# gooofy/zerovox

Hardware: AMD Instinct MI355X
Metric: audio samples/sec + RTF, 128-phoneme zero-shot synth @22.05kHz, 1/2/4/8 GPU (higher is better)
Workload: dtype f16+bf16

## Files before the change

zerovox_amd/csrc/gemm.hip:

```cpp
#include "mfma_util.h"
#include "zvx_kernels.h"

#include <cstring>
#include <type_traits>

#ifndef ZVX_GEMM_PART
#define ZVX_GEMM_PART 0
#endif
#define ZVX_PART_MAIN (ZVX_GEMM_PART != 2)
#define ZVX_PART_RESFUSE (ZVX_GEMM_PART != 1)
#if ZVX_GEMM_PART == 2
extern thread_local bool zvx_gemm_dry_run;
#else
thread_local hipEvent_t zvx_gemm_ev_start = nullptr, zvx_gemm_ev_stop = nullptr;
thread_local bool zvx_gemm_dry_run = false;
#endif
#define g_dry_run zvx_gemm_dry_run

#define ZVX_LAUNCH(...) do { if (!g_dry_run) ZVX_DISPATCH(__VA_ARGS__); } while (0)

namespace zvx {


#define PITCH 80
#define KBYTES 64

__device__ __forceinline__ float bf16_to_f32(unsigned short h) { return __uint_as_float(((unsigned)h) << 16); }
__device__ __forceinline__ unsigned short f32_to_bf16(float f) {
    unsigned u = __float_as_uint(f);
    u += 0x7fffu + ((u >> 16) & 1u);
    return (unsigned short)(u >> 16);
}

template <int DT>
__device__ __forceinline__ void load4(const void* base, long idx, float v[4]) {
    if (DT == DT_F32) {
        float4 t = *(const float4*)((const float*)base + idx);
        v[0] = t.x; v[1] = t.y; v[2] = t.z; v[3] = t.w;
    } else {
        uint2 t = *(const uint2*)((const unsigned short*)base + idx);
        v[0] = __uint_as_float(t.x << 16); v[1] = __uint_as_float(t.x & 0xffff0000u);
        v[2] = __uint_as_float(t.y << 16); v[3] = __uint_as_float(t.y & 0xffff0000u);
    }
}
__device__ __forceinline__ void load4_dyn(const void* base, int dt, long idx, float v[4]) {
    if (dt == DT_F32) load4<DT_F32>(base, idx, v);
    else if (dt == DT_F16) {
        const uint2 t = *(const uint2*)((const unsigned short*)base + idx);
        const f32x2 a = unpack_f16x2(t.x), b = unpack_f16x2(t.y);
        v[0] = a.x; v[1] = a.y; v[2] = b.x; v[3] = b.y;
    } else load4<DT_BF16>(base, idx, v);
}
__device__ __forceinline__ void store4_dyn(void* base, int dt, long idx, const float v[4]) {
    if (dt == DT_F32) {
        *(float4*)((float*)base + idx) = make_float4(v[0], v[1], v[2], v[3]);
    } else if (dt == DT_F16) {
        uint2 t;
        t.x = pack_f16x2_sat(v[0], v[1]); t.y = pack_f16x2_sat(v[2], v[3]);
        *(uint2*)((unsigned short*)base + idx) = t;
    } else {
        uint2 t;
        t.x = (unsigned)f32_to_bf16(v[0]) | ((unsigned)f32_to_bf16(v[1]) << 16);
        t.y = (unsigned)f32_to_bf16(v[2]) | ((unsigned)f32_to_bf16(v[3]) << 16);
        *(uint2*)((unsigned short*)base + idx) = t;
    }
}

template <int TM, int TN>
__device__ __forceinline__ void epilogue(const GemmArgs& a, f32x16 (&acc)[TN][TM], int b, int h, int row_base, int col_base,
                                         int out_len, bool two_d, int lane) {
    const long ooff = (long)b * a.o_bs + (long)h * a.o_hs;
    const long roff = (long)b * a.r_bs + (long)h * a.r_hs;
    const long aoff = (long)b * a.a_bs;
#pragma unroll
    for (int j = 0; j < TM; j++) {
        const int r = row_base + j * 32 + (lane & 31);
        bool rok = r < a.M;
        if (two_d) rok = rok && (r % a.wout) < out_len; else rok = rok && r < out_len;
        if (!rok) continue;
        const float brow = (a.bias_mode == 2) ? a.bias[r] : 0.f;
#pragma unroll
        for (int i = 0; i < TN; i++) {
#pragma unroll
            for (int g = 0; g < 4; g++) {
                const int n = col_base + i * 32 + 8 * g + 4 * (lane >> 5);
                if (n >= a.N) continue;
                float v[4];
#pragma unroll
                for (int e = 0; e < 4; e++) v[e] = acc[i][j][4 * g + e] * a.alpha + brow;
                if (a.bias_mode == 1) {
                    const float4 bb = *(const float4*)(a.bias + n);
                    v[0] += bb.x; v[1] += bb.y; v[2] += bb.z; v[3] += bb.w;
                }
                if (a.res_mode) {
                    float rr[4];
                    load4_dyn(a.res, a.res_dtype, roff + (long)r * a.ldr + n, rr);
                    if (a.res_mode == 2) {
#pragma unroll
                        for (int e = 0; e < 4; e++) rr[e] = rr[e] >= 0.f ? rr[e] : rr[e] * a.res_inv_slope;
                    }
#pragma unroll
                    for (int e = 0; e < 4; e++) v[e] += rr[e];
                }
                if (a.accum_mode) {
                    const long ai = aoff + (long)r * a.lda + n;
                    if (a.accum_mode & 1) {
                        float t[4];
                        load4_dyn(a.accum, a.accum_dtype, ai, t);
                        v[0] += t[0]; v[1] += t[1]; v[2] += t[2]; v[3] += t[3];
                    }
                    if (a.accum_mode & 2) store4_dyn(a.accum, a.accum_dtype, ai, v);
                }
                if (a.out) {
#pragma unroll
                    for (int e = 0; e < 4; e++) {
                        float t = v[e] * a.out_scale;
                        if (a.act == ACT_RELU) t = fmaxf(t, 0.f);
                        else if (a.act == ACT_LRELU) t = t >= 0.f ? t : t * a.slope;
                        v[e] = t;
                    }
                    if (a.post_scale) {
                        const float4 ps = *(const float4*)(a.post_scale + n), pt = *(const float4*)(a.post_shift + n);
                        v[0] = v[0] * ps.x + pt.x; v[1] = v[1] * ps.y + pt.y;
                        v[2] = v[2] * ps.z + pt.z; v[3] = v[3] * ps.w + pt.w;
                    }
                    store4_dyn(a.out, a.out_dtype, ooff + (long)r * a.ldo + n, v);
                }
            }
        }
    }
}

template <int DT, int BM, int BN, int WM, int WN>
__global__ __launch_bounds__(256) void gemm_kernel(const GemmArgs a) {
    constexpr int ES = (DT == DT_F32) ? 4 : 2;
    constexpr int EPC = 16 / ES;
    constexpr int BKE = KBYTES / ES;
    constexpr int TM = BM / WM / 32, TN = BN / WN / 32;
    constexpr int XCH = BM * 4 / 256;
    constexpr int WCH = (BN * 4 + 255) / 256;
    static_assert(WM * WN == 4, "4 waves");

    __shared__ __attribute__((aligned(16))) unsigned char lds[2][(BM + BN) * PITCH];
// ... 24 lines not shown
    const unsigned char* Wp = (const unsigned char*)a.W + ((long)b * a.w_bs + (long)h * a.w_hs) * ES;

    int xu[XCH], xv[XCH];
    const int kc = tid & 3;
#pragma unroll
    for (int i = 0; i < XCH; i++) {
        const int r = m0 + (tid >> 2) + i * 64;
        if (two_d) { xu[i] = (r / a.wout) * a.stride; xv[i] = (r % a.wout) * a.stride; }
        else { xu[i] = 0; xv[i] = r; }
    }

    const int kchunks = (Kb + BKE - 1) / BKE;
    const int S = a.ntaps * kchunks;

    uint4 xreg[XCH], wreg[WCH];

    auto load_regs = [&](int s) {
        const int tap = s / kchunks;
        const int k = (s - tap * kchunks) * BKE + kc * EPC;
        const bool kok = k < Kb;
        const int du = a.du[tap], dv = a.dv[tap];
#pragma unroll
        for (int i = 0; i < XCH; i++) {
            const int iu = xu[i] + du, iv = xv[i] + dv;
            const bool ok = kok && iu >= 0 && iu < a.hin && iv >= 0 && iv < in_len;
            uint4 v = make_uint4(0, 0, 0, 0);
            if (ok) v = *(const uint4*)(Xp + ((long)(iu * a.win + iv) * a.ldx + k) * ES);
            xreg[i] = v;
        }
#pragma unroll
        for (int i = 0; i < WCH; i++) {
            const int c = tid + i * 256;
            const int n = n0 + (c >> 2);
            uint4 v = make_uint4(0, 0, 0, 0);
            if ((BN * 4 >= 256 * (i + 1) || c < BN * 4) && kok && n < a.N)
                v = *(const uint4*)(Wp + ((long)tap * a.w_ts + (long)n * a.ldw + k) * ES);
            wreg[i] = v;
        }
    };
    auto store_lds = [&](int buf) {
        unsigned char* base = lds[buf];
#pragma unroll
        for (int i = 0; i < XCH; i++)
            *(uint4*)(base + ((tid >> 2) + i * 64) * PITCH + kc * 16) = xreg[i];
#pragma unroll
        for (int i = 0; i < WCH; i++) {
            const int c = tid + i * 256;
            if (BN * 4 >= 256 * (i + 1) || c < BN * 4)
                *(uint4*)(base + (BM + (c >> 2)) * PITCH + kc * 16) = wreg[i];
        }
    };

    f32x16 acc[TN][TM];
#pragma unroll
    for (int i = 0; i < TN; i++)
#pragma unroll
        for (int j = 0; j < TM; j++)
#pragma unroll
            for (int e = 0; e < 16; e++) acc[i][j][e] = 0.f;

    const int xrow = wr * (BM / WM) + (lane & 31);
    const int wrow = BM + wc * (BN / WN) + (lane & 31);
    const int koff = (lane >> 5) * 16;

    if (S > 0) {
        load_regs(0);
        store_lds(0);
    }
    __syncthreads();
    for (int s = 0; s < S; s++) {
        if (s + 1 < S) load_regs(s + 1);
        const unsigned char* base = lds[s & 1];
#pragma unroll
        for (int sub = 0; sub < 2; sub++) {
            uint4 xf[TM], wf[TN];
#pragma unroll
            for (int j = 0; j < TM; j++) xf[j] = *(const uint4*)(base + (xrow + j * 32) * PITCH + sub * 32 + koff);
#pragma unroll
            for (int i = 0; i < TN; i++) wf[i] = *(const uint4*)(base + (wrow + i * 32) * PITCH + sub * 32 + koff);
#pragma unroll
            for (int i = 0; i < TN; i++)
#pragma unroll
                for (int j = 0; j < TM; j++) {
                    if (DT == DT_BF16) {
                        acc[i][j] = __builtin_amdgcn_mfma_f32_32x32x16_bf16(
                            __builtin_bit_cast(bf16x8, wf[i]), __builtin_bit_cast(bf16x8, xf[j]), acc[i][j], 0, 0, 0);
                    } else if (DT == DT_F16) {
                        acc[i][j] = __builtin_amdgcn_mfma_f32_32x32x16_f16(
                            __builtin_bit_cast(f16x8, wf[i]), __builtin_bit_cast(f16x8, xf[j]), acc[i][j], 0, 0, 0);
                    } else {
                        acc[i][j] = __builtin_amdgcn_mfma_f32_32x32x2f32(__uint_as_float(wf[i].x), __uint_as_float(xf[j].x), acc[i][j], 0, 0, 0);
                        acc[i][j] = __builtin_amdgcn_mfma_f32_32x32x2f32(__uint_as_float(wf[i].y), __uint_as_float(xf[j].y), acc[i][j], 0, 0, 0);
                        acc[i][j] = __builtin_amdgcn_mfma_f32_32x32x2f32(__uint_as_float(wf[i].z), __uint_as_float(xf[j].z), acc[i][j], 0, 0, 0);
                        acc[i][j] = __builtin_amdgcn_mfma_f32_32x32x2f32(__uint_as_float(wf[i].w), __uint_as_float(xf[j].w), acc[i][j], 0, 0, 0);
                    }
                }
        }
        if (s + 1 < S) store_lds((s + 1) & 1);
        __syncthreads();
    }

    epilogue<TM, TN>(a, acc, b, h, m0 + wr * (BM / WM), n0 + wc * (BN / WN), out_len, two_d, lane);
}

__device__ __forceinline__ unsigned pack_f16x2(float lo, float hi) { return pack_f16x2_sat(lo, hi); }
__device__ __forceinline__ unsigned pack16x2(float lo, float hi, bool f16) { return f16 ? pack_f16x2_sat(lo, hi) : pack_bf16x2(lo, hi); }
__device__ __forceinline__ f32x2 unpack16x2(unsigned u, bool f16) { return f16 ? unpack_f16x2(u) : unpack_bf16x2(u); }

#define ZVX_EPI(res, am, out) ((res) | ((am) << 1) | ((out) << 3))
#define ZVX_EPI_DEC(res) (16 | 8 | (res))
#define ZVX_EPI_FLIP (ZVX_EPI(0, 0, 1) | 32)

template <int TM, int TN, int RES_LDS = 0, int EPI = -1, bool H16 = false>
__device__ __forceinline__ void epilogue_rows(const GemmArgs& a, f32x16 (&acc)[TN][TM], int b, int row_base, int col_base,
                                              int out_len, int lane, unsigned char* stage ,
                                              const unsigned char* res_lds = nullptr ,
                                              int res_pitch = 0) {
    constexpr int NW = TN * 32;
    constexpr int EP = NW * 4 + 16;
    constexpr int LPR = NW / 8;
    constexpr int RPP = 64 / LPR;
    constexpr int NP = 32 / RPP;
    constexpr bool CT = EPI >= 0;
    constexpr bool DEC = CT && (EPI & 16) != 0;
    constexpr bool BURST = !(CT && !DEC && ((EPI >> 1) & 1));
    const long ooff = (long)b * a.o_bs, roff = (long)b * a.r_bs, aoff = (long)b * a.a_bs;
    const int c8 = lane % LPR;
    const int n = col_base + c8 * 8;
    const bool nok = n < a.N;
    const float alpha = CT ? 1.f : a.alpha, oscale = a.out_scale, rinv = a.res_inv_slope;
    const int act = DEC ? ACT_NONE : (CT ? ACT_LRELU : a.act);
    const float slope = CT ? (a.act == ACT_LRELU ? a.slope : 1.f) : a.slope;
    const int res_mode = RES_LDS ? 2 : (DEC ? (EPI & 1) : (CT ? ((EPI & 1) ? 2 : 0) : a.res_mode));
    const int accum_mode = DEC ? 0 : (CT ? (EPI >> 1) & 3 : a.accum_mode), bias_mode = (CT && !DEC) ? 1 : a.bias_mode;
    const bool has_out = CT ? (EPI >> 3) & 1 : a.out != nullptr, out_bf16 = CT || a.out_dtype != DT_F32, has_post = !CT && a.post_scale != nullptr;
    const bool out_f16 = CT ? H16 : a.out_dtype == DT_F16, res_f16 = (CT || RES_LDS) ? H16 : a.res_dtype == DT_F16, acc_f16 = CT ? H16 : ((TN == 1 || TM <= 2) && a.accum_dtype == DT_F16);
    const bool acc_bf16 = CT || a.accum_dtype == DT_BF16 || acc_f16, res_bf16 = CT || RES_LDS || a.res_dtype != DT_F32;
#define pk2(lo, hi, f16) ((CT && H16) ? pack_f16x2_raw(lo, hi) : pack16x2(lo, hi, f16))
    f32x2 bcol[4];
#pragma unroll
    for (int e = 0; e < 4; e++) bcol[e] = (f32x2){0.f, 0.f};
    if (bias_mode == 1 && nok) {
        const float4 b0 = *(const float4*)(a.bias + n), b1 = *(const float4*)(a.bias + n + 4);
        bcol[0] = (f32x2){b0.x, b0.y}; bcol[1] = (f32x2){b0.z, b0.w}; bcol[2] = (f32x2){b1.x, b1.y}; bcol[3] = (f32x2){b1.z, b1.w};
    }
    u32x4 pk[TM][NP];
    const bool res_glb = !RES_LDS && res_mode && res_bf16;
    uint4 rnext[NP];
    auto res_prefetch = [&](int j) {
#pragma unroll
        for (int p = 0; p < NP; p++) {
            const int r = row_base + j * 32 + p * RPP + lane / LPR;
            const bool okp = r < a.M && r < out_len && nok;
            rnext[p] = *(const uint4*)((const unsigned short*)a.res + (okp ? roff + (long)r * a.ldr + n : 0));
        }
    };
    if (res_glb) res_prefetch(0);
#pragma unroll
    for (int j = 0; j < TM; j++) {
#pragma unroll
        for (int i = 0; i < TN; i++)
#pragma unroll
            for (int g = 0; g < 4; g++)
                *(float4*)(stage + (lane & 31) * EP + (i * 32 + 8 * g + 4 * (lane >> 5)) * 4) =
                    make_float4(acc[i][j][4 * g], acc[i][j][4 * g + 1], acc[i][j][4 * g + 2], acc[i][j][4 * g + 3]);
        f32x2 v[NP][4];
        uint4 rraw[NP];
        float4 aa0[NP], aa1[NP];
        uint4 aab[NP];
        bool ok[NP];
        if (res_glb) {
#pragma unroll
            for (int p = 0; p < NP; p++) rraw[p] = rnext[p];
            if (j + 1 < TM) res_prefetch(j + 1);
        }
#pragma unroll
        for (int p = 0; p < NP; p++) {
            const int rl = p * RPP + lane / LPR;
            const int r = row_base + j * 32 + rl;
            ok[p] = r < a.M && r < out_len && nok;
            const float4 v0 = *(const float4*)(stage + rl * EP + c8 * 32), v1 = *(const float4*)(stage + rl * EP + c8 * 32 + 16);
            v[p][0] = (f32x2){v0.x, v0.y}; v[p][1] = (f32x2){v0.z, v0.w}; v[p][2] = (f32x2){v1.x, v1.y}; v[p][3] = (f32x2){v1.z, v1.w};
            if (RES_LDS == 1) rraw[p] = *(const uint4*)(res_lds + (j * 32 + rl) * res_pitch + (col_base + c8 * 8) * 2);
            if (accum_mode & 1) {
                const long ai = ok[p] ? aoff + (long)r * a.lda + n : 0;
                if (acc_bf16) aab[p] = *(const uint4*)((const unsigned short*)a.accum + ai);
                else { const float* ap = (const float*)a.accum + ai; aa0[p] = *(const float4*)ap; aa1[p] = *(const float4*)(ap + 4); }
// ... 70 lines not shown
                    t[2] = t[2] * (f32x2){s1.x, s1.y} + (f32x2){h1.x, h1.y}; t[3] = t[3] * (f32x2){s1.z, s1.w} + (f32x2){h1.z, h1.w};
                }
                if (out_bf16) {
                    const u32x4 o = (u32x4){pk2(t[0].x, t[0].y, out_f16), pk2(t[1].x, t[1].y, out_f16), pk2(t[2].x, t[2].y, out_f16), pk2(t[3].x, t[3].y, out_f16)};
                    if (BURST) pk[j][p] = o;
                    else if (ok[p]) *(u32x4*)((unsigned short*)a.out + ooff + (long)r * a.ldo + n) = o;
                } else if (ok[p]) {
                    if (!CT && a.out_split3) {
                        unsigned short* op = (unsigned short*)a.out + ooff + (long)r * a.ldo + n;
                        u32x4 hv, lv;
#pragma unroll
                        for (int e = 0; e < 4; e++) {
                            if (a.out_split3 == 2) {
                                const unsigned hp = pack_f16x2(t[e].x, t[e].y);
                                const f32x2 rem = (t[e] - unpack_f16x2(hp)) * 2048.f;
                                hv[e] = hp; lv[e] = pack_f16x2(rem.x, rem.y);
                            } else {
                                const unsigned hp = pack_bf16x2(t[e].x, t[e].y);
                                const f32x2 rem = t[e] - unpack_bf16x2(hp);
                                hv[e] = hp; lv[e] = pack_bf16x2(rem.x, rem.y);
                            }
                        }
                        *(u32x4*)op = hv; *(u32x4*)(op + a.N) = hv; *(u32x4*)(op + 2 * a.N) = lv;
                    } else {
                        float* op = (float*)a.out + ooff + (long)r * a.ldo + n;
                        *(float4*)op = make_float4(t[0].x, t[0].y, t[1].x, t[1].y);
                        *(float4*)(op + 4) = make_float4(t[2].x, t[2].y, t[3].x, t[3].y);
                    }
                }
            }
        }
    }
    if (has_out && out_bf16 && BURST) {
        unsigned short* obase = (unsigned short*)a.out + ooff + n;
        const int ldo = a.ldo;
#pragma unroll
        for (int j = 0; j < TM; j++)
#pragma unroll
            for (int p = 0; p < NP; p++) {
                const int r = row_base + j * 32 + p * RPP + lane / LPR;
                if (r < a.M && r < out_len && nok) *(u32x4*)(obase + (long)r * ldo) = pk[j][p];
            }
    }
#undef pk2
}

template <int TM, int TN, bool F16 = false>
__device__ __forceinline__ void epilogue_direct(const GemmArgs& a, f32x16 (&acc)[TN][TM], int b, int row_base, int col_base,
                                                int out_len, int lane, unsigned char* stage ) {
    constexpr int NW = TN * 32, EP = NW * 2 + 16, LPR = NW / 8, RPP = 64 / LPR, NP = 32 / RPP;
    const float slope = a.act == ACT_LRELU ? a.slope : 1.f;
    const int h4 = 4 * (lane >> 5), c8 = lane % LPR, n = col_base + c8 * 8;
    const bool nok = n < a.N;
    float4 bb[TN][4];
#pragma unroll
    for (int i = 0; i < TN; i++)
#pragma unroll
        for (int g = 0; g < 4; g++) {
            const int co = col_base + i * 32 + 8 * g + h4;
            bb[i][g] = co < a.N ? *(const float4*)(a.bias + co) : make_float4(0.f, 0.f, 0.f, 0.f);
        }
    unsigned short* obase = (unsigned short*)a.out + (long)b * a.o_bs + n;
    u32x4 o[TM][NP];
#pragma unroll
    for (int j = 0; j < TM; j++) {
#pragma unroll
        for (int i = 0; i < TN; i++)
#pragma unroll
            for (int g = 0; g < 4; g++) {
                const f32x2 v01 = lrelu2((f32x2){acc[i][j][4 * g], acc[i][j][4 * g + 1]} + (f32x2){bb[i][g].x, bb[i][g].y}, slope);
                const f32x2 v23 = lrelu2((f32x2){acc[i][j][4 * g + 2], acc[i][j][4 * g + 3]} + (f32x2){bb[i][g].z, bb[i][g].w}, slope);
                uint2 pk;
                pk.x = pack16x2(v01.x, v01.y, F16);
                pk.y = pack16x2(v23.x, v23.y, F16);
                *(uint2*)(stage + (lane & 31) * EP + (i * 32 + 8 * g + h4) * 2) = pk;
            }
#pragma unroll
        for (int p = 0; p < NP; p++) o[j][p] = *(const u32x4*)(stage + (p * RPP + lane / LPR) * EP + c8 * 16);
    }
#pragma unroll
    for (int j = 0; j < TM; j++)
#pragma unroll
        for (int p = 0; p < NP; p++) {
            const int r = row_base + j * 32 + p * RPP + lane / LPR;
            if (r < a.M && r < out_len && nok) *(u32x4*)(obase + (long)r * a.ldo) = o[j][p];
        }
}

#if ZVX_PART_MAIN
#define SLAB_KC 64
#define SLAB_PITCH 144

__global__ void k_pack_w(const unsigned short* w, int ntaps, int N, int K, unsigned short* out, int nkc, long total_frag_lanes) {
    long idx = (long)blockIdx.x * blockDim.x + threadIdx.x;
    if (idx >= total_frag_lanes) return;
    const int lane = idx & 63; long t = idx >> 6;
    const int k16 = t & 3; t >>= 2;
    const int tap = t % ntaps; t /= ntaps;
    const int kc = t % nkc; const int nt = t / nkc;
    const int n = nt * 32 + (lane & 31);
    const int k0 = kc * SLAB_KC + k16 * 16 + 8 * (lane >> 5);
    unsigned short v[8];
#pragma unroll
    for (int e = 0; e < 8; e++) {
        const int k = k0 + e;
        v[e] = (n < N && k < K) ? w[((long)tap * N + n) * K + k] : (unsigned short)0;
    }
    uint4 o;
    o.x = v[0] | ((unsigned)v[1] << 16); o.y = v[2] | ((unsigned)v[3] << 16);
    o.z = v[4] | ((unsigned)v[5] << 16); o.w = v[6] | ((unsigned)v[7] << 16);
    *(uint4*)(out + idx * 8) = o;
}

size_t packed_weight_elems(int ntaps, int N, int K) {
    const int nkc = (K + SLAB_KC - 1) / SLAB_KC, nt = (N + 31) / 32;
    return (size_t)nt * nkc * ntaps * 4 * 64 * 8;
}
void launch_pack_weights(const void* w_bf16, int ntaps, int N, int K, void* out, hipStream_t s) {
    const int nkc = (K + SLAB_KC - 1) / SLAB_KC, nt = (N + 31) / 32;
    const long total = (long)nt * nkc * ntaps * 4 * 64;
    hipLaunchKernelGGL(k_pack_w, dim3((unsigned)((total + 255) / 256)), dim3(256), 0, s, (const unsigned short*)w_bf16, ntaps, N, K,
                       (unsigned short*)out, nkc, total);
}

// ... 10 lines not shown
    constexpr int NIT = ((BM + MAXH) * 8 + 255) / 256;
    static_assert(WM * WN == 4, "4 waves");
    extern __shared__ __attribute__((aligned(16))) unsigned char slab[];
    if (F16 && EPI >= 0 && EPI != ZVX_EPI(0, 0, 1) && EPI != ZVX_EPI_FLIP) f16_saturate_mode();

    const int tid = threadIdx.x, lane = tid & 63, wave = __builtin_amdgcn_readfirstlane(tid >> 6);
    const int wr = wave % WM, wc = wave / WM;
    const int ntn = (a.N + BN - 1) / BN;
    int wg, b;
    if (a.xcd_flat) {
        const int nx = gridDim.x, nwg = nx * gridDim.y, id = blockIdx.y * nx + blockIdx.x, q = nwg >> 3, r = nwg & 7, xcd = id & 7;
        const int w = (xcd < r ? xcd * (q + 1) : r * (q + 1) + (xcd - r) * q) + (id >> 3);
        b = w / nx; wg = w - b * nx;
    } else {
        const int nwg = gridDim.x, id = blockIdx.x, q = nwg >> 3, r = nwg & 7, xcd = id & 7;
        wg = (xcd < r ? xcd * (q + 1) : r * (q + 1) + (xcd - r) * q) + (id >> 3);
        b = blockIdx.y;
    }
    const int nt = wg % ntn, mt = wg / ntn;
    const int m0 = mt * BM, n0 = nt * BN;
    const bool bflat = a.bflat != 0;
    const int out_len = bflat ? a.M : (a.out_len ? a.out_len[b] : a.M);
    const int in_len = bflat ? 0 : (a.in_len ? a.in_len[b] : a.in_len_static);
    if (m0 >= out_len || m0 >= a.M) return;
    if (bflat) {
        const int b0 = m0 / a.bflat, t0 = m0 - b0 * a.bflat;
        if (t0 >= a.out_len[b0] && t0 + BM <= a.bflat) return;
    }

    const int HL = a.halo_l, SR = BM + a.halo_l + a.halo_r;
    const int nkc = (a.K + SLAB_KC - 1) / SLAB_KC, n16 = a.K >> 4, ntaps = a.ntaps;
    const unsigned short* Xp = (const unsigned short*)a.X + (long)b * a.x_bs;
    const int nkc2 = (!FULLK && a.K2 > 0) ? (a.K2 + SLAB_KC - 1) / SLAB_KC : 0, n16_2 = a.K2 >> 4;
    const unsigned short* Xp2 = (const unsigned short*)a.X2 + (long)b * a.x2_bs;
    const int in_rows = ((MAXH > 64 || bflat) && a.flat_win) ? a.flat_rows : in_len;
    unsigned rowmask = 0xffffffffu;
    if (bflat) {
        rowmask = 0;
#pragma unroll
        for (int it = 0; it < NIT; it++) {
            const int g = m0 - HL + ((tid + it * 256) >> 3);
            if (g >= 0 && g < in_rows) { const int bb = g / a.bflat; if (g - bb * a.bflat < a.in_len[bb]) rowmask |= 1u << it; }
        }
    } else if (MAXH > 64 && a.flat_win) {
        rowmask = 0;
#pragma unroll
        for (int it = 0; it < NIT; it++) {
            const int g = m0 - HL + ((tid + it * 256) >> 3);
            if (g >= 0 && g < in_rows && (g % a.flat_win) < in_len) rowmask |= 1u << it;
        }
    }

    f32x16 acc[TN][TM];
#pragma unroll
    for (int i = 0; i < TN; i++)
#pragma unroll
        for (int j = 0; j < TM; j++)
#pragma unroll
            for (int e = 0; e < 16; e++) acc[i][j][e] = 0.f;

    constexpr bool WREG = R == 0;
    constexpr int F = BN / 32, CNT = F >= 4 ? F / 4 : 1, WD = 4, D = WREG ? WD : R - 1, WAITN = WREG ? (WD - 1) * TN : (D - 2) * CNT;
    const int nt32_total = (a.N + 31) >> 5;
    const int nsteps = a.ntaps * 4, gtotal = nkc * nsteps + nkc2 * 4;
    const uint4* wsrc[CNT];
#pragma unroll
    for (int j = 0; j < CNT; j++) {
        const int f = wave * CNT + j, t32 = (n0 >> 5) + f;
        wsrc[j] = (const uint4*)a.Wp + (long)(t32 < nt32_total ? t32 : 0) * gtotal * 64 + lane;
    }
    const int xrow0 = HL + wr * (BM / WM) + (lane & 31);
    const int koff = (lane >> 5) * 16;
    unsigned char* ring = slab + ((SR * SLAB_PITCH + 1023) & ~1023);
    const unsigned lds_base = (unsigned)(size_t)(__attribute__((address_space(3))) unsigned char*)slab;
    const int dvreg = a.dv[lane & (ZVX_MAX_TAPS - 1)];
    const bool loader = wave * CNT < F;
    const unsigned char* wq[TN];
#pragma unroll
    for (int i = 0; i < TN; i++) {
        const int t32 = (n0 >> 5) + wc * TN + i;
        wq[i] = (const unsigned char*)a.Wp + (long)(t32 < nt32_total ? t32 : 0) * gtotal * 1024;
    }
    const bool wave_dead = __builtin_amdgcn_readfirstlane((int)(n0 + wc * TN * 32 >= a.N)) != 0;
    const unsigned lane16 = lane * 16;
    u32x4 wreg[WREG ? WD : 1][TN] = {};
    auto wload = [&](int gs, int slot) {
        const long off = (long)(gs < gtotal ? gs : gtotal - 1) * 1024;
#pragma unroll
        for (int i = 0; i < TN; i++)
            asm volatile("global_load_dwordx4 %0, %1, %2" : "+v"(wreg[WREG ? slot : 0][i]) : "v"(lane16), "s"(wq[i] + off) : "memory");
    };
    auto dma = [&](int gs) {
        if (WREG || !loader) return;
        const int slot = gs & (R - 1);
        const long off = (long)(gs < gtotal ? gs : gtotal - 1) * 64;
#pragma unroll
        for (int j = 0; j < CNT; j++)
            __builtin_amdgcn_global_load_lds((const __attribute__((address_space(1))) void*)(wsrc[j] + off),
                                             (__attribute__((address_space(3))) void*)(ring + (slot * F + wave * CNT + j) * 1024), 16, 0, 0);
    };
    if (WREG) { wload(0, 0); wload(1, 1); wload(2, 2); wload(3, 3); }
    else {
#pragma unroll
        for (int s0 = 0; s0 < D; s0++) dma(s0);
    }

    for (int kc = 0; kc < nkc + nkc2; kc++) {
        const bool src2 = !FULLK && kc >= nkc;
        const unsigned short* const Xs = src2 ? Xp2 : Xp;
        const int ldxs = src2 ? a.ldx2 : a.ldx, Ks = src2 ? a.K2 : a.K, kbase = (src2 ? kc - nkc : kc) * SLAB_KC;
        {
            constexpr int FCH = NIT > 10 ? (NIT + 1) / 2 : NIT;
#pragma unroll
            for (int h0 = 0; h0 < NIT; h0 += FCH) {
                uint4 sv[FCH];
#pragma unroll
                for (int i = 0; i < FCH; i++) {
                    const int it = h0 + i;
                    const int c = tid + it * 256;
                    const int row = c >> 3, q = c & 7;
                    const int g = m0 - HL + row, k = kbase + q * 8;
                    sv[i] = make_uint4(0, 0, 0, 0);
                    if (it < NIT && c < SR * 8 && g >= 0 && g < in_rows && k < Ks && ((rowmask >> it) & 1)) sv[i] = *(const uint4*)(Xs + (long)g * ldxs + k);
                }
                if (kc && h0 == 0) __syncthreads();
#pragma unroll
                for (int i = 0; i < FCH; i++) {
                    const int c = tid + (h0 + i) * 256;
                    if (h0 + i < NIT && c < SR * 8) *(uint4*)(slab + (c >> 3) * SLAB_PITCH + (c & 7) * 16) = sv[i];
                }
            }
        }
        __syncthreads();
        int nk16 = 4;
        if (!FULLK) { nk16 = src2 ? n16_2 - (kc - nkc) * 4 : n16 - kc * 4; if (nk16 > 4) nk16 = 4; if (wave_dead) nk16 = 0; }
        const int ntaps_kc = src2 ? 1 : ntaps;

        uint4 xA[TM], wA[TN], xB[TM], wB[TN];
        const unsigned ring_rd = lds_base + (unsigned)(size_t)(ring - slab) + lane * 16 + wc * TN * 1024;
        const int gs0 = src2 ? nkc * nsteps + (kc - nkc) * 4 : kc * nsteps;
        auto rd = [&](uint4 (&xf)[TM], uint4 (&wf)[TN], int gs, unsigned rowoff, int kk) {
            if (!WREG) {
                const unsigned wa = ring_rd + (gs & ((WREG ? 1 : R) - 1)) * (F * 1024);
#pragma unroll
                for (int i = 0; i < TN; i++)
                    asm volatile("ds_read_b128 %0, %1 offset:%2" : "=v"(wf[i]) : "v"(wa), "n"(i * 1024));
            }
#pragma unroll
            for (int j = 0; j < TM; j++)
                asm volatile("ds_read_b128 %0, %1" : "=v"(xf[j]) : "v"(lds_base + rowoff + j * 32 * SLAB_PITCH + kk * 32));
        };
        auto mma = [&](uint4 (&xf)[TM], uint4 (&wf)[TN]) {
#pragma unroll
            for (int i = 0; i < TN; i++)
#pragma unroll
                for (int j = 0; j < TM; j++)
                    acc[i][j] = F16 ? __builtin_amdgcn_mfma_f32_32x32x16_f16(__builtin_bit_cast(f16x8, wf[i]), __builtin_bit_cast(f16x8, xf[j]), acc[i][j], 0, 0, 0)
                                    : __builtin_amdgcn_mfma_f32_32x32x16_bf16(__builtin_bit_cast(bf16x8, wf[i]),
                                                                       __builtin_bit_cast(bf16x8, xf[j]), acc[i][j], 0, 0, 0);
        };
        auto mma_r = [&](uint4 (&xf)[TM], int slot) {
#pragma unroll
            for (int i = 0; i < TN; i++)
#pragma unroll
                for (int j = 0; j < TM; j++)
                    acc[i][j] = F16 ? __builtin_amdgcn_mfma_f32_32x32x16_f16(__builtin_bit_cast(f16x8, wreg[WREG ? slot : 0][i]), __builtin_bit_cast(f16x8, xf[j]), acc[i][j], 0, 0, 0)
                                    : __builtin_amdgcn_mfma_f32_32x32x16_bf16(__builtin_bit_cast(bf16x8, wreg[WREG ? slot : 0][i]),
                                                                       __builtin_bit_cast(bf16x8, xf[j]), acc[i][j], 0, 0, 0);
        };
        auto rowoff_of = [&](int tap) {
            const int d = src2 ? 0 : __builtin_amdgcn_readlane(dvreg, tap < ntaps ? tap : ntaps - 1);
            return (unsigned)((xrow0 + d) * SLAB_PITCH + koff);
        };
        unsigned rowoff = rowoff_of(0);
        rd(xA, wA, gs0, rowoff, 0);
        for (int tap = 0; tap < ntaps_kc; tap++) {
            const unsigned rowoff_next = rowoff_of(tap + 1);
#pragma unroll
            for (int kk = 0; kk < 4; kk++) {
                const int gs = gs0 + tap * 4 + kk;
                if (WREG) asm volatile("s_waitcnt vmcnt(%0)" :: "n"(WAITN) : "memory");
                else asm volatile("s_waitcnt vmcnt(%0)\n\ts_barrier" :: "n"(WAITN) : "memory");
                dma(gs + D);
                if (kk & 1) rd(xA, wA, gs + 1, kk == 3 ? rowoff_next : rowoff, (kk + 1) & 3);
                else        rd(xB, wB, gs + 1, rowoff, kk + 1);
                asm volatile("s_waitcnt lgkmcnt(%0)" :: "n"(WREG ? TM : TM + TN) : "memory");
// ... 1 lines not shown
                if (FULLK || kk < nk16) {
                    if (WREG) { if (kk & 1) mma_r(xB, kk); else mma_r(xA, kk); }
                    else { if (kk & 1) mma(xB, wB); else mma(xA, wA); }
                }
                __builtin_amdgcn_sched_barrier(0);
                if (WREG) wload(gs + WD, kk);
            }
            rowoff = rowoff_next;
        }
        asm volatile("s_waitcnt lgkmcnt(0)" ::: "memory");
    }
    if (WREG) {
#pragma unroll
        for (int sl = 0; sl < (WREG ? WD : 1); sl++)
#pragma unroll
            for (int i = 0; i < TN; i++) asm volatile("s_waitcnt vmcnt(0)" : "+v"(wreg[sl][i]) :: "memory");
    } else {
        asm volatile("s_waitcnt vmcnt(0)" ::: "memory");
    }
    __syncthreads();
    if (EPI == ZVX_EPI_FLIP)
        epilogue_direct<TM, TN, !F16>(a, acc, b, m0 + wr * (BM / WM), n0 + wc * (BN / WN), out_len, lane, slab + wave * (32 * (TN * 64 + 16)));
    else if (EPI == ZVX_EPI(0, 0, 1))
        epilogue_direct<TM, TN, F16>(a, acc, b, m0 + wr * (BM / WM), n0 + wc * (BN / WN), out_len, lane, slab + wave * (32 * (TN * 64 + 16)));
    else
        epilogue_rows<TM, TN, 0, EPI, (F16 && EPI >= 0)>(a, acc, b, m0 + wr * (BM / WM), n0 + wc * (BN / WN), out_len, lane, slab + wave * (32 * (TN * 32 * 4 + 16)));
}

template <int C, int NT, int BM, int WM, int WN, int MINW, int MAXH = 64, bool F16 = false>
__global__ __launch_bounds__(256, MINW) void convreg_kernel(const GemmArgs a) {
    constexpr int TM = BM / WM / 32;
    constexpr int KS = C / 16;
    constexpr int PITCH_ = C * 2 + 16;
    constexpr int CPR = C / 8;
    constexpr int NIT = ((BM + MAXH) * CPR + 255) / 256;
    constexpr int FCH = NIT > 12 ? 8 : NIT;
    static_assert(WM * WN == 4 && WN * 32 == C, "wave layout");
    extern __shared__ __attribute__((aligned(16))) unsigned char slab[];

    const int tid = threadIdx.x, lane = tid & 63, wave = tid >> 6;
    const int wr = wave % WM, wc = wave / WM;
    int wg;
    {
        const int nwg = gridDim.x, id = blockIdx.x, q = nwg >> 3, r = nwg & 7, xcd = id & 7;
        wg = (xcd < r ? xcd * (q + 1) : r * (q + 1) + (xcd - r) * q) + (id >> 3);
    }
    const int m0 = wg * BM, b = blockIdx.y;
    const int out_len = a.out_len ? a.out_len[b] : a.M;
    const int in_len = a.in_len ? a.in_len[b] : a.in_len_static;
    if (m0 >= out_len || m0 >= a.M) return;
    const int HL = a.halo_l, SR = BM + a.halo_l + a.halo_r;
    const unsigned short* Xp = (const unsigned short*)a.X + (long)b * a.x_bs;

    uint4 w[NT][KS];
    {
        const uint4* Wq = (const uint4*)a.Wp + ((long)wc * NT * 4) * 64 + lane;
#pragma unroll
        for (int t = 0; t < NT; t++)
#pragma unroll
            for (int kk = 0; kk < KS; kk++) w[t][kk] = Wq[(t * 4 + kk) * 64];
    }
    {
        const bool flat = MAXH > 64 && a.flat_win;
        const int in_rows = flat ? a.flat_rows : in_len;
#pragma unroll
        for (int h0 = 0; h0 < NIT; h0 += FCH) {
            uint4 sv[FCH];
#pragma unroll
            for (int i = 0; i < FCH; i++) {
                const int c = tid + (h0 + i) * 256;
                const int row = c / CPR, q = c % CPR;
                const int g = m0 - HL + row;
                sv[i] = make_uint4(0, 0, 0, 0);
                if (h0 + i < NIT && c < SR * CPR && g >= 0 && g < in_rows && (!flat || (g % a.flat_win) < in_len)) sv[i] = *(const uint4*)(Xp + (long)g * a.ldx + q * 8);
            }
#pragma unroll
            for (int i = 0; i < FCH; i++) {
                const int c = tid + (h0 + i) * 256;
                if (h0 + i < NIT && c < SR * CPR) *(uint4*)(slab + (c / CPR) * PITCH_ + (c % CPR) * 16) = sv[i];
            }
        }
    }
    __syncthreads();

    f32x16 acc[1][TM];
#pragma unroll
    for (int j = 0; j < TM; j++)
#pragma unroll
        for (int e = 0; e < 16; e++) acc[0][j][e] = 0.f;
    const int xrow0 = HL + wr * (BM / WM) + (lane & 31);
    const int koff = (lane >> 5) * 16;
#pragma unroll
    for (int t = 0; t < NT; t++) {
        const unsigned char* rowp = slab + (xrow0 + a.dv[t]) * PITCH_ + koff;
#pragma unroll
        for (int kk = 0; kk < KS; kk++)
#pragma unroll
            for (int j = 0; j < TM; j++) {
                const uint4 xf = *(const uint4*)(rowp + j * 32 * PITCH_ + kk * 32);
                acc[0][j] = mfma16<F16>(w[t][kk], xf, acc[0][j]);
            }
    }
    __syncthreads();
    epilogue_rows<TM, 1>(a, acc, b, m0 + wr * (BM / WM), wc * 32, out_len, lane, slab + wave * (32 * (32 * 4 + 16)));
}

typedef __attribute__((ext_vector_type(2))) unsigned u32x2_t;
__device__ __forceinline__ void store_block_mfma_layout(unsigned short* row_ptr , const uint2 (&pk)[4], int lane, bool ok) {
#pragma unroll
    for (int pr = 0; pr < 2; pr++) {
        const u32x2_t sx = __builtin_amdgcn_permlane32_swap(pk[2 * pr].x, pk[2 * pr + 1].x, false, false);
        const u32x2_t sy = __builtin_amdgcn_permlane32_swap(pk[2 * pr].y, pk[2 * pr + 1].y, false, false);
        if (ok) *(u32x4*)(row_ptr + 8 * (2 * pr + (lane >> 5))) = (u32x4){sx.x, sy.x, sx.y, sy.y};
    }
}

template <int C, int BM, int WM, int WN, int MAXH, int MODE, int WGPC, bool POOL = false>
__global__ __launch_bounds__(WM * WN * 64, WM * WN * WGPC / 4) void conv2d_persist_kernel(const GemmArgs a, const int ntm, const int ntiles) {
    constexpr int NTHR = WM * WN * 64;
    constexpr int NT = 9, TM = BM / WM / 32, KS = C / 16, PITCH_ = C * 2 + 16, CPR = C / 8, RSTEP = NTHR / CPR;
    constexpr int NIT = ((BM + MAXH) * CPR + NTHR - 1) / NTHR;
    constexpr bool EC_LDS = NTHR > 256;
    static_assert(WN * 32 == C && BM % (WM * 32) == 0, "wave layout");
    extern __shared__ __attribute__((aligned(16))) unsigned char slab[];

    const int tid = threadIdx.x, lane = tid & 63, wave = __builtin_amdgcn_readfirstlane(tid >> 6);
    const int wr = wave % WM, wc = wave / WM;
    const int G = gridDim.x, xcd = blockIdx.x & 7, slot = blockIdx.x >> 3;
    auto tile_of = [&](int r) {
        const int base = r * G, n = ntiles - base < G ? ntiles - base : G;
        if (n <= 0) return ntiles;
        const int per = (n + 7) >> 3, t = xcd * per + slot;
        return (slot < per && t < n) ? base + t : ntiles;
    };
    const int HL = a.halo_l, SR = BM + a.halo_l + a.halo_r, win = a.flat_win, in_rows = a.flat_rows;

    uint4 w[NT][KS];
    {
        const uint4* Wq = (const uint4*)a.Wp + ((long)wc * NT * 4) * 64 + lane;
#pragma unroll
        for (int t = 0; t < NT; t++)
#pragma unroll
// ... 341 lines not shown

    const int tid = threadIdx.x, lane = tid & 63, wave = tid >> 6;
    const int wr = wave % WM, wc = wave / WM;
    const int BMO = BM - 2 * H2;
    const int H1 = a.halo_l;
    const int SR = BM + 2 * H1;
    unsigned char* t1 = slab + ((SR * PITCH_ + 15) & ~15);

    constexpr bool TWO_SETS = (NT * KS <= 24);
    uint4 w[NT][KS];
    uint4 w2[TWO_SETS ? NT : 1][TWO_SETS ? KS : 1];
    const uint4* W1q = (const uint4*)a.Wp2 + ((long)wc * NT * 4) * 64 + lane;
    const uint4* W2q = (const uint4*)a.Wp + ((long)wc * NT * 4) * 64 + lane;
#pragma unroll
    for (int t = 0; t < NT; t++)
#pragma unroll
        for (int kk = 0; kk < KS; kk++) {
            w[t][kk] = W1q[(t * 4 + kk) * 64];
            if (TWO_SETS) w2[t][kk] = W2q[(t * 4 + kk) * 64];
        }
    const int koff = (lane >> 5) * 16;
    const int wrow = wr * (BM / WM);
    int tile;
    {
        const int nwg = gridDim.x, id = blockIdx.x, q = nwg >> 3, r = nwg & 7, xcd = id & 7;
        tile = (xcd < r ? xcd * (q + 1) : r * (q + 1) + (xcd - r) * q) + (id >> 3);
    }
    {
        const int b = tile / ntm, m0 = (tile - b * ntm) * BMO;
        const int out_len = a.out_len ? a.out_len[b] : a.M;
        const int in_len = a.in_len ? a.in_len[b] : a.in_len_static;
        if (tile >= ntiles || m0 >= out_len || m0 >= a.M) return;
        const unsigned short* Xp = (const unsigned short*)a.X + (long)b * a.x_bs;
        {
            uint4 sv[NIT];
            const int tq = tid;
#pragma unroll
            for (int it = 0; it < NIT; it++) {
                const int c = tq + it * 256;
                const int row = c / CPR, q = c % CPR;
                const int g = m0 - H2 - H1 + row;
                sv[it] = make_uint4(0, 0, 0, 0);
                if (c < SR * CPR && g >= 0 && g < in_len) sv[it] = *(const uint4*)(Xp + (long)g * a.ldx + q * 8);
            }
#pragma unroll
            for (int it = 0; it < NIT; it++) {
                const int c = tq + it * 256;
                if (c < SR * CPR) *(uint4*)(slab + (c / CPR) * PITCH_ + (c % CPR) * 16) = sv[it];
            }
        }
        __syncthreads();

        f32x16 acc[1][TM];
#pragma unroll
        for (int j = 0; j < TM; j++)
#pragma unroll
            for (int e = 0; e < 16; e++) acc[0][j][e] = 0.f;
#pragma unroll
        for (int t = 0; t < NT; t++) {
            const unsigned char* rowp = slab + (wrow + (lane & 31) + H1 + a.dv1[t]) * PITCH_ + koff;
#pragma unroll
            for (int kk = 0; kk < KS; kk++)
#pragma unroll
                for (int j = 0; j < TM; j++) {
                    const uint4 xf = *(const uint4*)(rowp + j * 32 * PITCH_ + kk * 32);
                    acc[0][j] = mfma16<F16>(w[t][kk], xf, acc[0][j]);
                }
            if (!TWO_SETS) {
#pragma unroll
                for (int kk = 0; kk < KS; kk++) w[t][kk] = W2q[(t * 4 + kk) * 64];
            }
        }
#pragma unroll
        for (int j = 0; j < TM; j++) {
            const int i = wrow + j * 32 + (lane & 31);
            const int g = m0 - H2 + i;
            const bool inside = g >= 0 && g < in_len;
#pragma unroll
            for (int q = 0; q < 4; q++) {
                const int co = wc * 32 + 8 * q + 4 * (lane >> 5);
                const float4 bb = *(const float4*)(a.bias1 + co);
                const uint2 xr = *(const uint2*)(slab + (i + H1) * PITCH_ + co * 2);
                const f32x2 r01 = inv_lrelu2(F16 ? unpack_f16x2(xr.x) : unpack_bf16x2(xr.x), a.res_inv_slope);
                const f32x2 r23 = inv_lrelu2(F16 ? unpack_f16x2(xr.y) : unpack_bf16x2(xr.y), a.res_inv_slope);
                f32x2 v01 = (f32x2){acc[0][j][4 * q] + bb.x, acc[0][j][4 * q + 1] + bb.y} + r01;
                f32x2 v23 = (f32x2){acc[0][j][4 * q + 2] + bb.z, acc[0][j][4 * q + 3] + bb.w} + r23;
                v01 = lrelu2(v01, a.slope1); v23 = lrelu2(v23, a.slope1);
                if (!inside) { v01 = (f32x2){0.f, 0.f}; v23 = (f32x2){0.f, 0.f}; }
                uint2 pk;
                if (F16) { pk.x = pack_f16x2_sat(v01.x, v01.y); pk.y = pack_f16x2_sat(v23.x, v23.y); }
                else { pk.x = pack_bf16x2(v01.x, v01.y); pk.y = pack_bf16x2(v23.x, v23.y); }
                *(uint2*)(t1 + i * PITCH_ + co * 2) = pk;
            }
        }
        __syncthreads();
#pragma unroll
        for (int j = 0; j < TM; j++)
#pragma unroll
            for (int e = 0; e < 16; e++) acc[0][j][e] = 0.f;
#pragma unroll
        for (int t = 0; t < NT; t++) {
            const unsigned char* rowp = t1 + (wrow + (lane & 31) + H2 + a.dv[t]) * PITCH_ + koff;
#pragma unroll
            for (int kk = 0; kk < KS; kk++)
#pragma unroll
                for (int j = 0; j < TM; j++) {
                    const uint4 xf = *(const uint4*)(rowp + j * 32 * PITCH_ + kk * 32);
                    acc[0][j] = mfma16<F16>(TWO_SETS ? w2[TWO_SETS ? t : 0][TWO_SETS ? kk : 0] : w[t][kk], xf, acc[0][j]);
                }
        }
        const int lim = (m0 + BMO < out_len) ? m0 + BMO : out_len;
        epilogue_rows<TM, 1, 1, -1, F16>(a, acc, b, m0 + wrow, wc * 32, lim, lane, slab + wave * (32 * (32 * 4 + 16)),
                                   t1 + (wrow + H2) * PITCH_, PITCH_);
    }
}

template <int C, int NT, int BM, int WM, int WN, int MINW>
static bool launch_rb2fuse_c(const GemmArgs& a, int h2, hipStream_t stream) {
    const int bmo = BM - 2 * h2;
    if (bmo < 32 || a.halo_l > 16) return false;
    const size_t pitch = C * 2 + 16;
    const size_t sb = (((size_t)(BM + 2 * a.halo_l) * pitch + 15) & ~(size_t)15);
    if (sb < (size_t)4 * 32 * (32 * 4 + 16)) return false;
    const size_t lds = sb + (size_t)(BM + 2 * h2) * pitch;
    if (lds > 160 * 1024) return false;
    const int ntm = (a.M + bmo - 1) / bmo, ntiles = ntm * a.nbatch;
    const dim3 grid(ntiles);
    if (a.dtype == DT_F16) { auto kfn = rb2fuse_kernel<C, NT, BM, WM, WN, MINW, true>; if (!lds_opt_in((const void*)kfn)) return false; ZVX_LAUNCH(kfn, grid, dim3(256), lds, stream, a, h2, ntm, ntiles); }
    else { auto kfn = rb2fuse_kernel<C, NT, BM, WM, WN, MINW, false>; if (!lds_opt_in((const void*)kfn)) return false; ZVX_LAUNCH(kfn, grid, dim3(256), lds, stream, a, h2, ntm, ntiles); }
    return true;
}

int launch_rb2fuse(GemmArgs a, hipStream_t stream) {
    if (a.dtype == DT_F32 || !a.Wp || !a.Wp2 || a.N != a.K || a.nheads != 1 || a.wout > 0 || a.bflat || a.K2) return -1;
    if (!(a.ntaps == 3 || a.ntaps == 5 || a.ntaps == 7) || !(a.N == 32 || a.N == 64)) return -1;
    const int h = (a.ntaps - 1) / 2, d1 = a.dv1[1] - a.dv1[0], d2 = a.dv[1] - a.dv[0];
    if (d1 < 1 || d2 < 1) return -1;
    for (int t = 0; t < a.ntaps; t++) if (a.dv1[t] != (t - h) * d1 || a.dv[t] != (t - h) * d2) return -1;
    if (a.alpha != 1.f || a.bias_mode != 1 || !a.bias || !a.bias1 || a.post_scale || a.res_mode != 2 || a.res != a.X || a.res_dtype != a.dtype || a.ldo % 8 ||
        (a.out && a.out_dtype != a.dtype) || (a.accum && (a.lda % 8 || a.accum_dtype != a.dtype)) || a.in_len != a.out_len || a.ldx != a.N) return -1;
    a.halo_l = a.halo_r = h * d1;
    a.fused = 2;
    if (a.N == 32) {
        if (a.ntaps == 3 && launch_rb2fuse_c<32, 3, 256, 4, 1, 2>(a, h * d2, stream)) return 30;
        if (a.ntaps == 5 && launch_rb2fuse_c<32, 5, 256, 4, 1, 2>(a, h * d2, stream)) return 30;
        if (a.ntaps == 7 && launch_rb2fuse_c<32, 7, 256, 4, 1, 2>(a, h * d2, stream)) return 30;
    } else {
        if (a.ntaps == 3 && launch_rb2fuse_c<64, 3, 256, 2, 2, 2>(a, h * d2, stream)) return 31;
        if (a.ntaps == 5 && launch_rb2fuse_c<64, 5, 256, 2, 2, 2>(a, h * d2, stream)) return 31;
    }
    return -1;
}

template <int C, int NT, int AM, bool HAS_OUT, int TM, bool F16 = false>
__global__ __launch_bounds__(512) __attribute__((amdgpu_waves_per_eu(2, 2))) void resfuse_persist_kernel(const GemmArgs a, int ntm, int ntiles) {
    if (F16) f16_saturate_mode();
    constexpr int KS = C >= 16 ? C / 16 : 1, CPR = C / 8, NTL = C >= 32 ? C / 32 : 1, RG = 4 / NTL;
    constexpr int QN = C >= 32 ? 4 : C / 8;
    constexpr int BM1 = 32 * TM * RG;
    constexpr int H2 = (NT - 1) / 2, BMO = BM1 - 2 * H2;
    constexpr int P = C * 2 + 16, CPP = CPR + 1;
    constexpr int NW = NT * KS;
    constexpr bool LEAN = NW > 36 || (F16 && NW >= 28 && TM == 2 && (AM & 1) && HAS_OUT);
    constexpr int NRES = LEAN ? (NW < 36 ? NW : 36) : NW;
    typedef __attribute__((ext_vector_type(4))) int i32x4;
    extern __shared__ __attribute__((aligned(16))) unsigned char lds[];

    const int tid = threadIdx.x, lane = tid & 63, wave = __builtin_amdgcn_readfirstlane(tid >> 6);
    const int role = wave >> 2, w4 = wave & 3;
    const int wc = w4 % NTL, wr = w4 / NTL, wrow = wr * 32 * TM;
    const int H1 = a.halo_l, SR = BM1 + 2 * H1;
    const int dil = a.dv1[1] - a.dv1[0];
    const float slope1 = a.slope1;
    const int SB = (SR * P + 1023) & ~1023;
    const int TB = ((BM1 + 2 * H2) * P + 15) & ~15;
    unsigned char* const t1base = lds + 4 * SB;
    unsigned char* const stage = t1base + 2 * TB + w4 * (32 * 80);
    float* const bias1_l = (float*)(t1base + 2 * TB + 4 * (32 * 80));
    float* const bias2_l = bias1_l + C;
    int* const lens_l = (int*)(bias2_l + C);
    const unsigned lds_addr0 = (unsigned)(size_t)(__attribute__((address_space(3))) unsigned char*)lds;
    const int G = gridDim.x;
    if (C < 32) {
        for (int i = tid * 16; i < 4 * SB + 2 * TB; i += 512 * 16) *(uint4*)(lds + i) = make_uint4(0, 0, 0, 0);
        __syncthreads();
    }
    if (tid < C) { bias1_l[tid] = a.bias1[tid]; bias2_l[tid] = a.bias[tid]; }
    if (a.nbatch <= 128 && tid < a.nbatch) { lens_l[tid] = a.out_len ? a.out_len[tid] : a.M; lens_l[128 + tid] = a.in_len ? a.in_len[tid] : a.in_len_static; }

    constexpr int NKC = (C + 63) / 64;
    const uint4* const Wq = (const uint4*)(role ? a.Wp : a.Wp2) + ((long)wc * NKC * NT * 4) * 64 + lane;
    auto wfrag = [](int t, int kk) { return (((kk >> 2) * NT + t) * 4 + (kk & 3)) * 64; };
    uint4 w[NRES];
#pragma unroll
    for (int i = 0; i < NRES; i++) w[i] = Wq[wfrag(i / KS, i % KS)];

    constexpr bool BIAS_REG = NW <= 22;
    const int h4 = 4 * (lane >> 5);
    float4 bq[4];
    if (BIAS_REG) {
#pragma unroll
        for (int q = 0; q < 4; q++) bq[q] = q < QN ? *(const float4*)((role ? a.bias : a.bias1) + wc * 32 + 8 * q + h4) : make_float4(0.f, 0.f, 0.f, 0.f);
    }
#pragma unroll
    for (int i = 0; i < NRES; i++) asm volatile("" :: "v"(w[i].x));
    if (BIAS_REG) {
#pragma unroll
        for (int q = 0; q < 4; q++) asm volatile("" :: "v"(bq[q].x));
    }
    __syncthreads();
    struct Tile { int t, b, mt, m0, in_len, out_len; };
    const bool use_tab = a.nbatch <= 128;
    auto sload = [&](const int* p) { int v; asm volatile("s_load_dword %0, %1, 0x0\n\ts_waitcnt lgkmcnt(0)" : "=s"(v) : "s"(p) : "memory"); return v; };
    auto len_of = [&](const int* g, int which, int b, int dflt) {
        if (!g) return dflt;
        return use_tab ? __builtin_amdgcn_readfirstlane(lens_l[which * 128 + b]) : sload(g + b);
    };
    const int gq = G / ntm, gr = G % ntm;
    auto load_tile = [&](int t, int b, int mt) {
        Tile q; q.t = -1; q.b = q.mt = q.m0 = q.in_len = q.out_len = 0;
        for (; t < ntiles; t += G, b += gq, mt += gr) {
            if (mt >= ntm) { mt -= ntm; b++; }
            const int m0 = mt * BMO, ol = len_of(a.out_len, 0, b, a.M);
            if (m0 < ol) { q.t = t; q.b = b; q.mt = mt; q.m0 = m0; q.out_len = ol; q.in_len = len_of(a.in_len, 1, b, a.in_len_static); break; }
        }
        q.t = __builtin_amdgcn_readfirstlane(q.t); q.b = __builtin_amdgcn_readfirstlane(q.b); q.mt = __builtin_amdgcn_readfirstlane(q.mt);
        q.m0 = __builtin_amdgcn_readfirstlane(q.m0);
        q.in_len = __builtin_amdgcn_readfirstlane(q.in_len); q.out_len = __builtin_amdgcn_readfirstlane(q.out_len);
        return q;
    };
    auto next_tile = [&](const Tile& q) {
        int b = q.b + gq, mt = q.mt + gr;
        return load_tile(q.t + G, b, mt);
    };
    constexpr int MAXP = C == 128 ? 10 : 8;
    constexpr bool VREL_REG = NW <= 22;
    const int npieces = SB >> 10;
    auto vrel_of = [&](int n) {
        const int cp = (w4 + 4 * n) * 64 + lane, row = cp / CPP, qs = cp % CPP;
        return qs == CPR ? -(1 << 30) : (row * a.ldx + (qs << 3)) * 2;
    };
    int vrel[VREL_REG ? MAXP : 1];
    if (VREL_REG) {
#pragma unroll
        for (int n = 0; n < MAXP; n++) vrel[n] = vrel_of(n);
    }
    auto dma_slab = [&](const Tile& q, int buf) {
        const int g0 = q.m0 - H2 - H1;
        const unsigned long long pa = (unsigned long long)((const unsigned short*)a.X + (long)q.b * a.x_bs + (long)g0 * a.ldx);
        const i32x4 rs = {__builtin_amdgcn_readfirstlane((int)(unsigned)pa), __builtin_amdgcn_readfirstlane((int)((pa >> 32) & 0xffff)),
                          __builtin_amdgcn_readfirstlane((q.in_len - g0) * a.ldx * 2), 0x00020000};
        const int thr = -g0 * a.ldx * 2;
        const unsigned la0 = lds_addr0 + buf * SB + w4 * 1024;
#pragma unroll
        for (int n = 0; n < MAXP; n++) {
            if (w4 + 4 * n < npieces) {
                const int vr = VREL_REG ? vrel[VREL_REG ? n : 0] : vrel_of(n);
                const int voff = vr < thr ? -16 : vr;
                const unsigned la = __builtin_amdgcn_readfirstlane(la0 + n * 4096);
                asm volatile("s_mov_b32 m0, %0\n\tbuffer_load_dwordx4 %1, %2, 0 offen lds" :: "s"(la), "v"(voff), "s"(rs) : "memory", "m0");
            }
        }
    };

    Tile qA, qB, qC, qD;
    qA = load_tile(ntiles, 0, 0); qB = qA;
    qC = load_tile(blockIdx.x, blockIdx.x / ntm, blockIdx.x % ntm);
    qD = qC.t >= 0 ? next_tile(qC) : qA;
    if (role == 0 && qC.t >= 0) dma_slab(qC, 0);
    asm volatile("s_waitcnt vmcnt(0) lgkmcnt(0)\n\ts_barrier" ::: "memory");
    const int koff = (lane >> 5) * 16;
    f32x16 acc[1][TM];
    for (int ph = 0; qA.t >= 0 || qB.t >= 0 || qC.t >= 0; ph++) {
        const Tile qE = qD.t >= 0 ? next_tile(qD) : qD;
        if (role == 0) {
            if (qD.t >= 0) dma_slab(qD, (ph + 1) & 3);
            if (qB.t >= 0) {
                unsigned char* t1 = t1base + ((ph - 1) & 1) * TB;
#pragma unroll
                for (int j = 0; j < TM; j++) {
                    const int i = wrow + j * 32 + (lane & 31);
                    const int g = qB.m0 - H2 + i;
                    const bool inside = g >= 0 && g < qB.in_len;
#pragma unroll
                    for (int q = 0; q < QN; q++) {
                        const int co = wc * 32 + 8 * q + h4;
                        const float4 bb = BIAS_REG ? bq[q] : *(const float4*)(bias1_l + co);
                        const f32x2 v01 = lrelu2((f32x2){acc[0][j][4 * q], acc[0][j][4 * q + 1]} + (f32x2){bb.x, bb.y}, slope1);
                        const f32x2 v23 = lrelu2((f32x2){acc[0][j][4 * q + 2], acc[0][j][4 * q + 3]} + (f32x2){bb.z, bb.w}, slope1);
                        uint2 pk;
                        pk.x = inside ? pack16<F16>(v01.x, v01.y) : 0u;
                        pk.y = inside ? pack16<F16>(v23.x, v23.y) : 0u;
                        *(uint2*)(t1 + i * P + co * 2) = pk;
                    }
                }
            }
            if (qC.t >= 0) {
#pragma unroll
                for (int j = 0; j < TM; j++)
#pragma unroll
                    for (int e = 0; e < 16; e++) acc[0][j][e] = 0.f;
                const unsigned char* rowp0 = lds + (ph & 3) * SB + (wrow + (lane & 31) + H1 - H2 * dil) * P + koff;
#pragma unroll
                for (int t = 0; t < NT; t++) {
                    const unsigned char* rowp = rowp0 + t * dil * P;
#pragma unroll
                    for (int kk = 0; kk < KS; kk++) {
                        const uint4 wf = (t * KS + kk < NRES) ? w[t * KS + kk < NRES ? t * KS + kk : 0] : Wq[wfrag(t, kk)];
#pragma unroll
                        for (int j = 0; j < TM; j++) {
                            const uint4 xf = *(const uint4*)(rowp + j * 32 * P + kk * 32);
                            acc[0][j] = mfma16<F16>(wf, xf, acc[0][j]);
                        }
                    }
                }
            }
            asm volatile("s_waitcnt vmcnt(0)" ::: "memory");
        } else if (qA.t >= 0) {
#pragma unroll
            for (int j = 0; j < TM; j++)
#pragma unroll
                for (int e = 0; e < 16; e++) acc[0][j][e] = 0.f;
            const unsigned char* rowp = t1base + (ph & 1) * TB + (wrow + (lane & 31)) * P + koff;
#pragma unroll
            for (int t = 0; t < NT; t++)
#pragma unroll
                for (int kk = 0; kk < KS; kk++) {
                    const uint4 wf = (t * KS + kk < NRES) ? w[t * KS + kk < NRES ? t * KS + kk : 0] : Wq[wfrag(t, kk)];
#pragma unroll
                    for (int j = 0; j < TM; j++) {
                        const uint4 xf = *(const uint4*)(rowp + (t + j * 32) * P + kk * 32);
                        acc[0][j] = mfma16<F16>(wf, xf, acc[0][j]);
                    }
                }
            const int lim_rows = (qA.m0 + BMO < qA.out_len) ? qA.m0 + BMO : qA.out_len;
            const int lim = (C >= 32 || (lane & 3) < CPR) ? lim_rows : -(1 << 30);
            {
                const float rinv = a.res_inv_slope, oscale = a.out_scale, slope = a.act == ACT_LRELU ? a.slope : 1.f;
                const unsigned char* resp = lds + ((ph + 2) & 3) * SB + (wrow + H2 + H1 + (lane & 31)) * P + (wc * 32 + h4) * 2;
                const long rm_off = wc * 32 + (lane & 3) * 8;
                unsigned short* accp = (unsigned short*)a.accum + (long)qA.b * a.a_bs + rm_off;
                unsigned short* outp = (unsigned short*)a.out + (long)qA.b * a.o_bs + rm_off;
                float4 bb[LEAN ? 1 : 4];
                if (!LEAN) {
#pragma unroll
                    for (int q = 0; q < QN; q++) bb[LEAN ? 0 : q] = BIAS_REG ? bq[q] : *(const float4*)(bias2_l + wc * 32 + 8 * q + h4);
                }
                constexpr bool XS_EARLY = NW < 28 || TM == 1;
                uint4 xs[TM][2];
                if ((AM & 1) && XS_EARLY) {
#pragma unroll
                    for (int j = 0; j < TM; j++)
#pragma unroll
                        for (int h = 0; h < 2; h++) {
                            const int gr = qA.m0 + wrow + j * 32 + h * 16 + (lane >> 2);
                            xs[j][h] = *(const uint4*)(accp + (gr < lim ? (long)gr * a.lda : 0));
                        }
                }
#pragma unroll
                for (int j = 0; j < TM; j++) {
                    if ((AM & 1) && !XS_EARLY) {
#pragma unroll
                        for (int h = 0; h < 2; h++) {
                            const int gr = qA.m0 + wrow + j * 32 + h * 16 + (lane >> 2);
                            xs[j][h] = *(const uint4*)(accp + (gr < lim ? (long)gr * a.lda : 0));
                        }
                    }
                    uint2 rrj[LEAN ? 1 : 4];
                    if (!LEAN) {
#pragma unroll
                        for (int q = 0; q < QN; q++) rrj[LEAN ? 0 : q] = *(const uint2*)(resp + j * 32 * P + q * 16);
                    }
                    uint2 pk[LEAN ? 1 : 4];
#pragma unroll
                    for (int q = 0; q < QN; q++) {
                        const float4 bq_ = LEAN ? *(const float4*)(bias2_l + wc * 32 + 8 * q + h4) : bb[LEAN ? 0 : q];
                        const uint2 rq_ = LEAN ? *(const uint2*)(resp + j * 32 * P + q * 16) : rrj[LEAN ? 0 : q];
                        f32x2 v01 = (f32x2){acc[0][j][4 * q], acc[0][j][4 * q + 1]} + (f32x2){bq_.x, bq_.y} + inv_lrelu2(unpack16<F16>(rq_.x), rinv);
                        f32x2 v23 = (f32x2){acc[0][j][4 * q + 2], acc[0][j][4 * q + 3]} + (f32x2){bq_.z, bq_.w} + inv_lrelu2(unpack16<F16>(rq_.y), rinv);
                        if (!AM) { v01 = lrelu2(v01, slope); v23 = lrelu2(v23, slope); }
                        uint2 pq;
                        pq.x = pack16<F16>(v01.x, v01.y);
                        pq.y = pack16<F16>(v23.x, v23.y);
                        if (LEAN) *(uint2*)(stage + (lane & 31) * 80 + (8 * q + h4) * 2) = pq;
                        else pk[LEAN ? 0 : q] = pq;
                    }
                    if (!LEAN) {
#pragma unroll
                        for (int q = 0; q < QN; q++) *(uint2*)(stage + (lane & 31) * 80 + (8 * q + h4) * 2) = pk[LEAN ? 0 : q];
                    }
                    uint4 o[2];
#pragma unroll
                    for (int h = 0; h < 2; h++) o[h] = *(const uint4*)(stage + (h * 16 + (lane >> 2)) * 80 + (lane & 3) * 16);
#pragma unroll
                    for (int h = 0; h < 2; h++) {
                        const int gr = qA.m0 + wrow + j * 32 + h * 16 + (lane >> 2);
                        if (AM) {
                            f32x2 t[4] = {unpack16<F16>(o[h].x), unpack16<F16>(o[h].y), unpack16<F16>(o[h].z), unpack16<F16>(o[h].w)};
                            if (AM & 1) {
                                t[0] += unpack16<F16>(xs[j][h].x); t[1] += unpack16<F16>(xs[j][h].y);
                                t[2] += unpack16<F16>(xs[j][h].z); t[3] += unpack16<F16>(xs[j][h].w);
                            }
                            if ((AM & 2) && gr < lim)
                                *(u32x4*)(accp + (long)gr * a.lda) = (u32x4){pack16<F16>(t[0].x, t[0].y), pack16<F16>(t[1].x, t[1].y),
                                                                            pack16<F16>(t[2].x, t[2].y), pack16<F16>(t[3].x, t[3].y)};
                            if (HAS_OUT) {
#pragma unroll
                                for (int e = 0; e < 4; e++) t[e] = lrelu2(t[e] * oscale, slope);
                                o[h] = make_uint4(pack16<F16>(t[0].x, t[0].y), pack16<F16>(t[1].x, t[1].y), pack16<F16>(t[2].x, t[2].y), pack16<F16>(t[3].x, t[3].y));
                            }
                        }
                        if (HAS_OUT && gr < lim) *(uint4*)(outp + (long)gr * a.ldo) = o[h];
                    }
                }
            }
        }
        asm volatile("s_waitcnt lgkmcnt(0)\n\ts_barrier" ::: "memory");
        qA = qB; qB = qC; qC = qD; qD = qE;
    }
}

template <int C, int TM = 2>
static bool launch_resfuse_persist_c(const GemmArgs& a, hipStream_t stream) {
    constexpr int BM1 = 32 * TM * (4 / (C >= 32 ? C / 32 : 1));
    const int h2 = (a.ntaps - 1) / 2, bmo = BM1 - 2 * h2;
    const int ntm = (a.M + bmo - 1) / bmo, ntiles = ntm * a.nbatch;
    const int ncu = persistent_cus();
    dim3 grid(ntiles < ncu ? ntiles : ncu);
    for (int t = 0; t < a.ntaps; t++)
        if (a.dv[t] != t - h2 || a.dv1[t] != (t - h2) * (a.dv1[1] - a.dv1[0])) return false;
    const size_t sb = ((size_t)(BM1 + 2 * a.halo_l) * (C * 2 + 16) + 1023) & ~(size_t)1023;
    const size_t tb = ((size_t)(BM1 + 2 * h2) * (C * 2 + 16) + 15) & ~(size_t)15;
// ... 236 lines not shown
    const int ntn = (a.N + bn - 1) / bn;
    if (a.bflat) {
        const long slots = 2L * ncu;
        const long wg_utt = (long)ntn * ((a.M + bm - 1) / bm) * a.nbatch, wg_flat = (long)ntn * (((long)a.nbatch * a.bflat + bm - 1) / bm);
        if ((wg_flat + slots - 1) / slots < (wg_utt + slots - 1) / slots) { a.flat_win = a.bflat; a.flat_rows = a.nbatch * a.bflat; a.M = a.flat_rows; a.nbatch = 1; }
        else a.bflat = 0;
    }
    if (best == 1 && bflat_hint && a.M > 256 && hl + hr <= 64) {
        const long slots = 2L * ncu;
        const long t256 = (long)ntn * ((a.M + 255) / 256) * a.nbatch, t128 = (long)ntn * ((a.M + 127) / 128) * a.nbatch;
        const long eff256 = 2 * ((t256 + slots - 1) / slots), eff128 = (t128 + slots - 1) / slots;
        if (eff128 < eff256) {
            dim3 g128(ntn * ((a.M + 127) / 128), a.nbatch);
            size_t lds128 = ((size_t)(128 + hl + hr) * SLAB_PITCH + 1023) & ~(size_t)1023;
            const size_t stage128 = (size_t)4 * 32 * (2 * 128 + 16);
            if (lds128 < stage128) lds128 = stage128;
            switch (gemm_epi_mode_of(a)) {
                case ZVX_EPI(0, 0, 1): launch_slab_variant<128, 128, 2, 2, 2, 0, ZVX_EPI(0, 0, 1)>(a, g128, lds128, stream); break;
                case ZVX_EPI_DEC(0): launch_slab_variant<128, 128, 2, 2, 2, 0, ZVX_EPI_DEC(0)>(a, g128, lds128, stream); break;
                case ZVX_EPI_DEC(1): launch_slab_variant<128, 128, 2, 2, 2, 0, ZVX_EPI_DEC(1)>(a, g128, lds128, stream); break;
                default: launch_slab_variant<128, 128, 2, 2, 2, 0>(a, g128, lds128, stream);
            }
            return 22;
        }
    }
    const int ntm = (a.M + bm - 1) / bm;
    dim3 grid(ntn * ntm, a.nbatch);
    const int tn = (bn >= 128) ? 2 : 1;
    if (a.accum_mode && a.accum && a.accum_dtype == DT_F16 && tn == 2 && !(best == 1 && gemm_epi_mode_of(a) >= 0)) return -6;
    size_t lds = (((size_t)(bm + hl + hr) * SLAB_PITCH + 1023) & ~(size_t)1023) + (size_t)ring_slots * (bn / 32) * 1024;
    const size_t stage = (size_t)4 * 32 * (tn * 128 + 16);
    if (lds < stage) lds = stage;
    switch (best) {
        case 0: launch_slab_variant<128, 256, 1, 4, 2, 0>(a, grid, lds, stream); break;
        case 1: switch (gemm_epi_mode_of(a)) {
                    case ZVX_EPI(0, 0, 1): launch_slab_variant<256, 128, 2, 2, 2, 0, ZVX_EPI(0, 0, 1)>(a, grid, lds, stream); break;
                    case ZVX_EPI_FLIP: launch_slab_variant<256, 128, 2, 2, 2, 0, ZVX_EPI_FLIP>(a, grid, lds, stream); break;
                    case ZVX_EPI(1, 0, 1): launch_slab_variant<256, 128, 2, 2, 2, 0, ZVX_EPI(1, 0, 1)>(a, grid, lds, stream); break;
                    case ZVX_EPI(1, 2, 0): launch_slab_variant<256, 128, 2, 2, 2, 0, ZVX_EPI(1, 2, 0)>(a, grid, lds, stream); break;
                    case ZVX_EPI(1, 3, 0): launch_slab_variant<256, 128, 2, 2, 2, 0, ZVX_EPI(1, 3, 0)>(a, grid, lds, stream); break;
                    case ZVX_EPI(1, 1, 1): launch_slab_variant<256, 128, 2, 2, 2, 0, ZVX_EPI(1, 1, 1)>(a, grid, lds, stream); break;
                    case ZVX_EPI_DEC(0): launch_slab_variant<256, 128, 2, 2, 2, 0, ZVX_EPI_DEC(0)>(a, grid, lds, stream); break;
                    case ZVX_EPI_DEC(1): launch_slab_variant<256, 128, 2, 2, 2, 0, ZVX_EPI_DEC(1)>(a, grid, lds, stream); break;
                    default: launch_slab_variant<256, 128, 2, 2, 2, 0>(a, grid, lds, stream);
                }
                break;
        case 2: launch_slab_variant<256, 64, 2, 2, 2, 8>(a, grid, lds, stream); break;
        case 3: launch_slab_variant<256, 32, 4, 1, 2, 8>(a, grid, lds, stream); break;
    }
    return 6 + best;
}


int launch_gemm(const GemmArgs& a, hipStream_t stream) {
    if (a.N <= 0 || a.M <= 0 || a.nbatch <= 0) return -1;
    if (a.ds_out) return launch_conv2d_s2(a, stream) ? 28 : -7;
    if (a.stride == 2 && a.wout > 0 && a.ntaps == 9 && a.K == 64 && a.Wp && launch_conv2d_s2(a, stream)) return 29;
    if (a.ntaps < 1 || a.ntaps > ZVX_MAX_TAPS) return -2;
    if (a.out_split3 && (a.out_dtype != DT_F32 || a.N % 8 || a.flat_win || a.wout > 0)) return -2;
    if (a.N % 4 && (a.bias_mode == 1 || a.res_mode || a.accum_mode || a.post_scale || a.ldo < ((a.N + 3) & ~3))) return -2;
    if (a.Wp && a.dtype == DT_BF16 && a.wout > 0 && a.stride == 1 && a.ntaps == 9 && a.wout == a.win && a.M == a.hin * a.win && a.nheads == 1 && a.w_bs == 0 &&
        !a.k_len && a.K % 16 == 0 && a.N % 32 == 0 && a.ldo % 8 == 0 && a.ldx == a.K && !a.res_mode && !a.accum_mode && a.bias_mode != 2 && a.win <= 271) {
        bool ok9 = true;
        for (int t = 0; t < 9; t++) ok9 = ok9 && a.du[t] == t / 3 - 1 && a.dv[t] == t % 3 - 1;
        if (ok9 && (a.N == a.K ? (a.N == 32 || a.N == 64 || (a.N % 128 == 0 && 2 * (a.win + 1) <= 160)) : false)) {
            GemmArgs f = a;
            f.flat_win = a.win; f.flat_rows = a.hin * a.win;
            for (int t = 0; t < 9; t++) { f.dv[t] = a.du[t] * a.win + a.dv[t]; f.du[t] = 0; }
            f.wout = 0; f.out_len = nullptr;
            const int id = launch_convslab(f, stream);
            if (id >= 0) return id;
        }
    }
    if (a.Wp && a.dtype != DT_F32 && a.wout <= 0 && a.nheads == 1 && a.w_bs == 0 && !a.k_len && a.K % 16 == 0 && a.N % 8 == 0 && a.ldo % 8 == 0) {
        int lo = 0, hi = 0;
        for (int i = 0; i < a.ntaps; i++) { if (a.dv[i] < lo) lo = a.dv[i]; if (a.dv[i] > hi) hi = a.dv[i]; }
        if (hi - lo <= 64 && hi >= 0 && lo <= 0) return launch_convslab(a, stream);
        if (hi - lo <= 96 && hi >= 0 && lo <= 0 && a.ntaps == 7 && a.N == a.K && (a.N == 32 || a.N == 64 || a.N == 128) && !a.K2 && !a.out_split3 && !a.bflat) {
            const int id = launch_convslab(a, stream);
            if (id >= 0) return id;
        }
    }
    if (a.out_split3 || a.K2) return -2;
    static const int bns[3] = {128, 64, 32};
    static const double eff[3] = {1.0, 0.75, 0.45};
    int best = 0; double best_cost = -1;
    for (int i = 0; i < 3; i++) {
        const double cost = (double)((a.N + bns[i] - 1) / bns[i]) * bns[i] / eff[i];
        if (best_cost < 0 || cost < best_cost - 1e-9) { best_cost = cost; best = i; }
    }
    int bn = bns[best], bm = (bn == 128) ? 128 : 256;
    int ntn = (a.N + bn - 1) / bn, ntm = (a.M + bm - 1) / bm;
    if ((long)ntn * ntm * a.nbatch * a.nheads < 512 && a.N >= 64) {
        bm = bn = 64; ntn = (a.N + 63) / 64; ntm = (a.M + 63) / 64;
        dim3 grid(ntn * ntm, a.nbatch * a.nheads), block(256);
        if (a.dtype == DT_BF16) { ZVX_LAUNCH((gemm_kernel<DT_BF16, 64, 64, 2, 2>), grid, block, 0, stream, a); return 18; }
        if (a.dtype == DT_F16) { ZVX_LAUNCH((gemm_kernel<DT_F16, 64, 64, 2, 2>), grid, block, 0, stream, a); return 18; }
        ZVX_LAUNCH((gemm_kernel<DT_F32, 64, 64, 2, 2>), grid, block, 0, stream, a);
        return 19;
    }
    dim3 grid(ntn * ntm, a.nbatch * a.nheads), block(256);
    const int base = (a.dtype != DT_F32) ? 0 : 3;
    const int id = base + best;
    if (a.dtype == DT_F16) {
        switch (id) {
            case 0: ZVX_LAUNCH((gemm_kernel<DT_F16, 128, 128, 2, 2>), grid, block, 0, stream, a); break;
            case 1: ZVX_LAUNCH((gemm_kernel<DT_F16, 256, 64, 4, 1>), grid, block, 0, stream, a); break;
            case 2: ZVX_LAUNCH((gemm_kernel<DT_F16, 256, 32, 4, 1>), grid, block, 0, stream, a); break;
// ... 24 lines not shown
```

zerovox_amd/csrc/pairstream.hip:

```cpp
#include "mfma_util.h"
#include "zvx_kernels.h"

#include <algorithm>
#include <type_traits>

namespace zvx {

#define PS_R 128
#define PS_WD 8
#define PS_XP 256
#define PS_TP 272
#define PS_NDMA 8

#ifndef PS_EXP
#define PS_EXP 0
#endif
#ifndef PS_PD
#define PS_PD 2
#endif
#ifndef PS_PRIO
#define PS_PRIO 1
#endif
#ifndef PS_RES_LDS
#define PS_RES_LDS 1
#endif
#ifndef PS_RPF
#define PS_RPF 2
#endif
#ifndef PS_DMA_TAIL
#define PS_DMA_TAIL 1
#endif
#ifdef PS_PROFILE
#define PS_STAMP(k) do { const unsigned long long t_ = __builtin_readcyclecounter(); tacc[k] += t_ - tlast; tlast = t_; } while (0)
#else
#define PS_STAMP(k) do {} while (0)
#endif

template <int ROLE, int NT, int AM, bool HAS_OUT, bool H16>
__device__ __forceinline__ void ps_role(const PairArgs& a, unsigned char* lds, const int lane, const int ct) {
    constexpr int R = PS_R, H2 = (NT - 1) / 2, NS = 8 * NT, WD = PS_WD;
    constexpr int EPI = (ROLE == 0 && !PS_DMA_TAIL) ? (PS_NDMA + NT - 2) / (NT - 1) : 0;
    static_assert(ROLE == 1 || PS_DMA_TAIL || EPI * (NT - 1) >= PS_NDMA, "DMA slots");
    const int l32 = lane & 31, hi = lane >> 5;
    const int dil = a.dil, H1 = dil * H2, DX = a.DX, DT = a.DT, G0 = a.G0;
    const unsigned tbase = (unsigned)DX * PS_XP;
    const float* const bias_l = (const float*)(lds + tbase + (unsigned)DT * PS_TP) + ROLE * 128;
    const unsigned scratch_l = tbase + (unsigned)DT * PS_TP + 1024;

    const unsigned char* const wq = (const unsigned char*)(ROLE ? a.W2 : a.W1) + (long)ct * NS * 1024;
    const unsigned lane16 = lane * 16;
    u32x4 wreg[WD] = {};
    auto wload = [&](int off, int slot) __attribute__((always_inline)) {
        asm volatile("global_load_dwordx4 %0, %1, %2" : "+v"(wreg[slot]) : "v"(lane16), "s"(wq + off) : "memory");
    };
#pragma unroll
    for (int i = 0; i < WD; i++) wload(i * 1024, i);

    const float slope1 = a.slope1, rinv = a.res_inv_slope, oscale = a.out_scale, oslope = a.slope;
    f32x16 acc[4];
#ifdef PS_PROFILE
    unsigned long long tacc[4] = {0, 0, 0, 0}, tlast = __builtin_readcyclecounter();
#endif

    const int nsegs = a.nseg * a.nbatch;
    for (int seg = blockIdx.x; seg < nsegs; seg += gridDim.x) {
        const int b = seg / a.nseg, sj = seg - b * a.nseg;
        int len = a.len ? a.len[b] : a.M;
        len = __builtin_amdgcn_readfirstlane(len);
        const int seg0 = sj * a.S;
        if (seg0 >= len) continue;
        const int seg_end = min(seg0 + a.S, len);
        const int nb = (seg_end - seg0 + 2 * H2 + R - 1) / R;
        const int c1_0 = seg0 - H2;
        const int xrow0 = c1_0 - H1;
        const unsigned short* const Xb = (const unsigned short*)a.X + (long)b * a.x_bs;

        auto dma_rsrc = [&](int grow, bool real) __attribute__((always_inline)) {
            const unsigned long long pa = (unsigned long long)(Xb + (long)grow * a.ldx);
            int nrec = real ? (len - grow) * a.ldx * 2 : 0; if (nrec < 0) nrec = 0;
            return (i32x4){__builtin_amdgcn_readfirstlane((int)(unsigned)pa), __builtin_amdgcn_readfirstlane((int)((pa >> 32) & 0xffff)),
                           __builtin_amdgcn_readfirstlane(nrec), 0x00020000};
        };
        auto dma_piece = [&](const i32x4& rsrc, int grow, int pos, int pc, bool real) __attribute__((always_inline)) {
            int lv = lane;
            asm volatile("" : "+v"(lv));
            const int rr = lv >> 4, sl = lv & 15;
            int p = pos + 4 * pc; if (p >= DX) p -= DX;
            const int key = (p + rr) & 15;
            int voff = ((4 * pc + rr) * a.ldx + ((sl ^ key) << 3)) * 2;
            if (grow + 4 * pc + rr < 0) voff = -16;
            const unsigned la = __builtin_amdgcn_readfirstlane(real ? (unsigned)p * PS_XP : scratch_l);
            asm volatile("s_mov_b32 m0, %0\n\ts_nop 0\n\tbuffer_load_dwordx4 %1, %2, 0 offen lds" :: "s"(la), "v"(voff), "s"(rsrc) : "memory", "m0");
        };

        int x_rd = 0;
        int x_wr = G0;
        int gx = xrow0 + G0;
        int t_wr = 0;
        int t_rd = DT - 2 * H2;
        int g1 = c1_0;
        int g2 = seg0 - 2 * H2;
        if (ROLE == 0) {
            const i32x4 rs0 = dma_rsrc(xrow0, true);
            for (int pc = ct; pc < G0 / 4; pc += 4) dma_piece(rs0, xrow0, 0, pc, true);
            asm volatile("s_waitcnt vmcnt(0)" ::: "memory");
        }
        asm volatile("s_waitcnt lgkmcnt(0)\n\ts_barrier" ::: "memory");

        auto main_loop = [&](bool dma_real) __attribute__((always_inline)) {
#pragma unroll
            for (int j = 0; j < 4; j++)
#pragma unroll
                for (int e = 0; e < 16; e++) acc[j][e] = 0.f;
            unsigned bs[4], nbs[4], pn = 0, hkn = 0;
            auto bases_common = [&](int u) __attribute__((always_inline)) {
                const int kc = u >= NT ? 1 : 0, tap = u - kc * NT;
                if (ROLE == 0) {
                    pn = x_rd + l32 + tap * dil; pn = min(pn, pn - (unsigned)DX);
                    hkn = (((pn ^ hi) & 15u) << 4) ^ ((unsigned)kc << 7);
                } else {
                    pn = t_rd + l32 + tap; pn = min(pn, pn - (unsigned)DT);
                    hkn = tbase + hi * 16 + kc * 128;
                }
            };
            auto bases_tile = [&](int j, unsigned (&o)[4]) __attribute__((always_inline)) {
                unsigned pj = pn + 32 * j;
                if (ROLE == 0) { pj = min(pj, pj - (unsigned)DX); o[j] = (pj << 8) + hkn; }
                else { pj = min(pj, pj - (unsigned)DT); o[j] = pj * PS_TP + hkn; }
            };
            auto rd1 = [&](uint4& xf, unsigned o, int kk) __attribute__((always_inline)) {
                if (PS_EXP & 2) { asm volatile("" : "=v"(xf)); return; }
                if (PS_EXP & 64) {
                    uint4 dummy;
                    if (ROLE == 0) asm volatile("ds_read_b128 %0, %1" : "=v"(dummy) : "v"(o ^ (unsigned)(kk << 5)));
                    else asm volatile("ds_read_b128 %0, %1" : "=v"(dummy) : "v"(o + kk * 32));
                    asm volatile("" : "=v"(xf));
                    return;
                }
                if (ROLE == 0) asm volatile("ds_read_b128 %0, %1" : "=v"(xf) : "v"(o ^ (unsigned)(kk << 5)));
                else {
                    switch (kk) {
                        case 0: asm volatile("ds_read_b128 %0, %1" : "=v"(xf) : "v"(o)); break;
                        case 1: asm volatile("ds_read_b128 %0, %1 offset:32" : "=v"(xf) : "v"(o)); break;
                        case 2: asm volatile("ds_read_b128 %0, %1 offset:64" : "=v"(xf) : "v"(o)); break;
                        default: asm volatile("ds_read_b128 %0, %1 offset:96" : "=v"(xf) : "v"(o)); break;
                    }
                }
            };
            constexpr int PD = PS_PD;
            static_assert(PD == 1 || PD == 2, "prefetch distance");
            uint4 xs[4][4];
            const i32x4 rsd = PS_DMA_TAIL ? (i32x4){0, 0, 0, 0} : dma_rsrc(gx, dma_real);
            bases_common(0);
#pragma unroll
            for (int j = 0; j < 4; j++) bases_tile(j, bs);
            asm volatile("s_waitcnt lgkmcnt(0)" ::: "memory");
            __builtin_amdgcn_sched_barrier(0);
#pragma unroll
            for (int i = 0; i < PD; i++)
#pragma unroll
                for (int j = 0; j < 4; j++) rd1(xs[i][j], bs[j], i);
            for (int u2 = 0; u2 < NT; u2++) {
                const int next_off = (u2 + 1 == NT ? 0 : (u2 + 1) * (WD * 1024));
#pragma unroll
                for (int h = 0; h < 2; h++) {
                    const int u = 2 * u2 + h;
                    int un = u + 1; if (un == 2 * NT) un = 0;
#pragma unroll
                    for (int kk = 0; kk < 4; kk++) {
                        const int i = h * 4 + kk;
                        asm volatile("s_waitcnt vmcnt(%0) lgkmcnt(%1)" :: "n"(WD - 1 + EPI), "n"(4 * (PD - 1)) : "memory");
                        __builtin_amdgcn_sched_barrier(0);
#pragma unroll
                        for (int j = 0; j < 4; j++) {
                            if (PS_EXP & 32) asm volatile("" : "+v"(acc[j]) : "v"(wreg[i]), "v"(xs[i & 3][j]));
                            else acc[j] = mfma16<H16>(wreg[i], xs[i & 3][j], acc[j]);
                            __builtin_amdgcn_sched_barrier(0);
                            if (kk + PD < 4) rd1(xs[(i + PD) & 3][j], bs[j], kk + PD); else rd1(xs[(i + PD) & 3][j], nbs[j], kk + PD - 4);
                            if (kk == 0 && j == 3) bases_common(un);
                            if (kk == 1) bases_tile(j, nbs);
                            if (j == 3) {
                                if (!(PS_EXP & 1)) wload(next_off + i * 1024, i);
                                if (ROLE == 0 && !PS_DMA_TAIL && !(PS_EXP & 8)) {
#pragma unroll
                                    for (int e = 0; e < EPI; e++)
                                        if (i == (7 * e + 3) / EPI) {
                                            const int pidx = u2 * EPI + e;
                                            dma_piece(rsd, gx, x_wr, ct * PS_NDMA + (pidx < PS_NDMA ? pidx : 0), dma_real && pidx < PS_NDMA);
                                        }
                                }
                            }
                            __builtin_amdgcn_sched_barrier(0);
                        }
                    }
#pragma unroll
                    for (int j = 0; j < 4; j++) bs[j] = nbs[j];
                }
            }
            asm volatile("s_waitcnt lgkmcnt(0)" ::: "memory");
            __builtin_amdgcn_sched_barrier(0);
        };

        auto epilogue_T = [&]() __attribute__((always_inline)) {
            int lv = lane;
            asm volatile("" : "+v"(lv));
            const int l32 = lv & 31, hi = lv >> 5;
            float4 bq[4];
#pragma unroll
            for (int q = 0; q < 4; q++) bq[q] = *(const float4*)(bias_l + ct * 32 + 8 * q + 4 * hi);
#pragma unroll
            for (int j = 0; j < 4; j++) {
                const int g = g1 + 32 * j + l32;
                const bool inside = g >= 0 && g < len;
                unsigned wp = t_wr + 32 * j + l32; wp = min(wp, wp - (unsigned)DT);
                unsigned char* const dst = lds + tbase + wp * PS_TP + (ct * 32 + 4 * hi) * 2;
#pragma unroll
                for (int q = 0; q < 4; q++) {
                    const f32x2 v01 = lrelu2((f32x2){acc[j][4 * q], acc[j][4 * q + 1]} + (f32x2){bq[q].x, bq[q].y}, slope1);
                    const f32x2 v23 = lrelu2((f32x2){acc[j][4 * q + 2], acc[j][4 * q + 3]} + (f32x2){bq[q].z, bq[q].w}, slope1);
                    uint2 pk;
                    pk.x = inside ? pack16<H16>(v01.x, v01.y) : 0u;
                    pk.y = inside ? pack16<H16>(v23.x, v23.y) : 0u;
                    if (!(PS_EXP & 16)) *(uint2*)(dst + q * 16) = pk;
                    else asm volatile("" :: "v"(pk.x), "v"(pk.y), "v"(dst));
                }
            }
        };

        int off[4];
        u32x4 rx[4][2], sx[4][2];
        uint2 rcur[4][4], rnext[4][4];
        auto residual_reads = [&](int blk) __attribute__((always_inline)) {
            int lv = lane;
            asm volatile("" : "+v"(lv));
            unsigned p0 = (unsigned)((long)blk * R % DX) + H1 - H2 + (lv & 31);
            p0 = min(p0, p0 - (unsigned)DX);
#pragma unroll
            for (int j = 0; j < 4; j++) {
                unsigned pj = p0 + 32 * j; pj = min(pj, pj - (unsigned)DX);
                const unsigned char* row = lds + pj * PS_XP + (lv >> 5) * 8;
#pragma unroll
                for (int q = 0; q < 4; q++) rnext[j][q] = *(const uint2*)(row + (((ct * 4 + q) ^ (pj & 15u)) << 4));
            }
        };
        auto res_rsrc = [&](const void* base, long bs_) __attribute__((always_inline)) {
            return __builtin_amdgcn_make_buffer_rsrc((void*)((unsigned short*)base + (long)b * bs_), 0, len * a.ldx * 2, 0x00020000);
        };
        auto epilogue_loads = [&](int gb) __attribute__((always_inline)) {
            int lv = lane;
            asm volatile("" : "+v"(lv));
            const int cA = ct * 32 + 8 * (lv >> 5);
            const __amdgpu_buffer_rsrc_t rsX = res_rsrc(a.X, a.x_bs), rsA = res_rsrc(a.accum, a.a_bs);
#pragma unroll
            for (int j = 0; j < 4; j++) {
                const int g = gb + 32 * j + (lv & 31);
                off[j] = (g >= seg0 && g < seg_end && !(PS_EXP & 4)) ? (g * a.ldx + cA) * 2 : (int)0x80000000;
                if (!PS_RES_LDS) {
                    rx[j][0] = __builtin_amdgcn_raw_buffer_load_b128(rsX, off[j], 0, 0);
                    rx[j][1] = __builtin_amdgcn_raw_buffer_load_b128(rsX, off[j] + 32, 0, 0);
                }
            }
            if (AM & 1) {
#pragma unroll
                for (int j = 0; j < 4; j++) {
                    sx[j][0] = __builtin_amdgcn_raw_buffer_load_b128(rsA, off[j], 0, 0);
                    sx[j][1] = __builtin_amdgcn_raw_buffer_load_b128(rsA, off[j] + 32, 0, 0);
                }
            }
        };
        auto epilogue_out = [&]() __attribute__((always_inline)) {
            int lv = lane;
            asm volatile("" : "+v"(lv));
            float4 bq[4];
#pragma unroll
            for (int q = 0; q < 4; q++) bq[q] = *(const float4*)(bias_l + ct * 32 + 8 * q + 4 * (lv >> 5));
            const __amdgpu_buffer_rsrc_t rsA = res_rsrc(a.accum, a.a_bs), rsO = res_rsrc(a.out, a.o_bs);
#pragma unroll
            for (int j = 0; j < 4; j++) {
                float v[16];
#pragma unroll
                for (int q = 0; q < 4; q++) {
                    v[4 * q] = acc[j][4 * q] + bq[q].x; v[4 * q + 1] = acc[j][4 * q + 1] + bq[q].y;
                    v[4 * q + 2] = acc[j][4 * q + 2] + bq[q].z; v[4 * q + 3] = acc[j][4 * q + 3] + bq[q].w;
                    if (PS_RES_LDS) {
                        const f32x2 r01 = inv_lrelu2(unpack16<H16>(rcur[j][q].x), rinv), r23 = inv_lrelu2(unpack16<H16>(rcur[j][q].y), rinv);
                        v[4 * q] += r01.x; v[4 * q + 1] += r01.y; v[4 * q + 2] += r23.x; v[4 * q + 3] += r23.y;
                    }
                }
#pragma unroll
                for (int pr = 0; pr < 2; pr++) {
                    float w8[8];
#pragma unroll
                    for (int e = 0; e < 4; e++) {
                        const auto r = __builtin_amdgcn_permlane32_swap(__float_as_uint(v[8 * pr + e]), __float_as_uint(v[8 * pr + 4 + e]), false, false);
                        w8[e] = __uint_as_float(r[0]); w8[4 + e] = __uint_as_float(r[1]);
                    }
                    f32x2 t[4] = {(f32x2){w8[0], w8[1]}, (f32x2){w8[2], w8[3]}, (f32x2){w8[4], w8[5]}, (f32x2){w8[6], w8[7]}};
                    if (!PS_RES_LDS) {
                        const u32x4 rr = rx[j][pr];
                        t[0] += inv_lrelu2(unpack16<H16>(rr.x), rinv); t[1] += inv_lrelu2(unpack16<H16>(rr.y), rinv);
                        t[2] += inv_lrelu2(unpack16<H16>(rr.z), rinv); t[3] += inv_lrelu2(unpack16<H16>(rr.w), rinv);
                    }
                    if (AM & 1) {
                        const u32x4 ss = sx[j][pr];
                        t[0] += unpack16<H16>(ss.x); t[1] += unpack16<H16>(ss.y); t[2] += unpack16<H16>(ss.z); t[3] += unpack16<H16>(ss.w);
                    }
                    if (AM & 2)
                        __builtin_amdgcn_raw_buffer_store_b128((u32x4){pack16<H16>(t[0].x, t[0].y), pack16<H16>(t[1].x, t[1].y), pack16<H16>(t[2].x, t[2].y), pack16<H16>(t[3].x, t[3].y)},
                                                               rsA, off[j] + 32 * pr, 0, 0);
                    if (HAS_OUT) {
                        if (AM) {
#pragma unroll
                            for (int e = 0; e < 4; e++) t[e] *= oscale;
                        }
#pragma unroll
                        for (int e = 0; e < 4; e++) t[e] = lrelu2(t[e], oslope);
                        __builtin_amdgcn_raw_buffer_store_b128((u32x4){pack16<H16>(t[0].x, t[0].y), pack16<H16>(t[1].x, t[1].y), pack16<H16>(t[2].x, t[2].y), pack16<H16>(t[3].x, t[3].y)},
                                                               rsO, off[j] + 32 * pr, 0, 0);
                    }
                }
            }
        };

        for (int s = 0; s <= nb + 1; s++) {
            if (ROLE == 0) {
                if (s < nb) {
                    main_loop(s + 1 < nb);
                    if (PS_DMA_TAIL && !(PS_EXP & 8) && s + 1 < nb) {
                        const i32x4 rsd = dma_rsrc(gx, true);
#pragma unroll
                        for (int pc = 0; pc < PS_NDMA; pc++) dma_piece(rsd, gx, x_wr, ct * PS_NDMA + pc, true);
                    }
                    PS_STAMP(0);
                    gx += R; x_wr += R; if (x_wr >= DX) x_wr -= DX;
                    if (PS_PRIO & 2) __builtin_amdgcn_s_setprio(2);
                    epilogue_T();
// ... 99 lines not shown
```

zerovox_amd/csrc/resstream.hip:

```cpp
#include "mfma_util.h"
#include "zvx_kernels.h"

#include <algorithm>
#include <type_traits>

namespace zvx {

#define RS_RD 64
#define RS_PF 2

template <int I, int N, class F>
__device__ __forceinline__ void static_for(F&& f) {
    if constexpr (I < N) { f(std::integral_constant<int, I>{}); static_for<I + 1, N>(f); }
}

template <int I, int PD, int KS, int DIL, int P>
__device__ __forceinline__ void rs_read(uint4 (&xf)[PD + 1], unsigned base) {
    asm volatile("ds_read_b128 %0, %1 offset:%2" : "=v"(xf[I % (PD + 1)]) : "v"(base), "n"((I / KS) * DIL * P + (I % KS) * 32));
}
template <int I, int PD, int KS, int DIL, int P>
__device__ __forceinline__ void rs_prefetch(uint4 (&xf)[PD + 1], unsigned base) {
    if constexpr (I < PD) { rs_read<I, PD, KS, DIL, P>(xf, base); rs_prefetch<I + 1, PD, KS, DIL, P>(xf, base); }
}
template <int I, int NW, int PD, int KS, int DIL, int P, bool H16>
__device__ __forceinline__ void rs_mma_steps(uint4 (&xf)[PD + 1], const uint4 (&w)[NW], unsigned base, f32x16& acc) {
    if constexpr (I < NW) {
        if constexpr (I + PD < NW) rs_read<I + PD, PD, KS, DIL, P>(xf, base);
        asm volatile("s_waitcnt lgkmcnt(%0)" :: "n"(NW - 1 - I >= PD ? PD : NW - 1 - I) : "memory");
        __builtin_amdgcn_sched_barrier(0);
        acc = mfma16<H16>(w[I], xf[I % (PD + 1)], acc);
        __builtin_amdgcn_sched_barrier(0);
        rs_mma_steps<I + 1, NW, PD, KS, DIL, P, H16>(xf, w, base, acc);
    }
}

template <int NR, int WPR>
__device__ __forceinline__ void role_of_wave(int w, int& role, int& sub) {
    if (NR == 6 && WPR == 2) { role = (int)((0x404023235151ull >> (4 * w)) & 15); sub = (w >> 1) & 1; }
    else if (NR == 4 && WPR == 2) { role = (int)((0x23013210u >> (4 * w)) & 15); sub = w >= 4; }
    else if (NR == 2 && WPR == 4) { role = (int)((0x01011010u >> (4 * w)) & 15); sub = w >> 1; }
    else { role = w % NR; sub = w / NR; }
}

template <int NR, int WPR>
__device__ __forceinline__ int prio_of_wave(int w) {
    if (NR == 6 && WPR == 2) return 3 - (w >> 2);
    return w < 4 ? 2 : 1;
}

template <int C, int NT, int NPAIR, int RSPLIT, int DP>
struct RsGeom {
    static constexpr int R = 32 * RSPLIT, H2 = (NT - 1) / 2;
    static constexpr int dil(int p) { return (DP >> (4 * p)) & 15; }
    static constexpr int h0 = dil(0) * H2;
    static constexpr int dT = 2 * R + 2 * H2;
    static constexpr int dX0 = (((RS_PF + 2) * R + RS_RD + h0 + H2 + 2 * h0) + RS_RD - 1) / RS_RD * RS_RD;
    static constexpr int dX(int p) {
        return p == 0 ? 0 : (2 * R + 2 * dil(p) * H2 > 3 * R + dil(p) * H2 + H2 ? 2 * R + 2 * dil(p) * H2 : 3 * R + dil(p) * H2 + H2);
    }
};

template <int C, int NT, int NPAIR, int RSPLIT, int AM, bool HAS_OUT, int DP, bool H16, int ROLE>
__device__ __forceinline__ void rs_role(const StreamArgs& a, unsigned char* const lds, const int lane, const int sub, const int wave) {
    using G = RsGeom<C, NT, NPAIR, RSPLIT, DP>;
    constexpr int NR = 2 * NPAIR, NTL = C / 32, WPR = NTL * RSPLIT;
    constexpr int R = 32 * RSPLIT, KS = C / 16, P = 2 * C + 16, CPP = C / 8 + 1, H2 = (NT - 1) / 2, NW = NT * KS;
    constexpr int PPB = CPP;
    constexpr int PPW = (PPB + WPR - 1) / WPR;
    constexpr int NKC = (C + 63) / 64;
    constexpr int role = ROLE, pair = ROLE >> 1, kind = ROLE & 1;
    const int ct = sub % NTL, rs = sub / NTL;
    const int l32 = lane & 31, koff = (lane >> 5) * 16, h4 = 4 * (lane >> 5);
    constexpr bool is_final = ROLE == NR - 1;

    int my_h = 0, my_H = 0, Hsum = 0;
#pragma unroll
    for (int r = 0; r < NR; r++) {
        const int h = (r & 1) ? H2 : G::dil(r >> 1) * H2;
        Hsum += h;
        if (r <= role) my_H += h;
        if (r == role) my_h = h;
    }
    const int h0 = G::dil(0) * H2;
    const int my_dil = kind ? 1 : G::dil(pair);
    const int NB0 = (Hsum + R - 1) / R;
    int offX = 0, offT = 0, dXp = G::dX0, offXn = 0, dXn = 0;
    {
        int cur = G::dX0 * P;
#pragma unroll
        for (int p = 0; p < NPAIR; p++) {
            if (p == pair) offT = cur;
            cur += G::dT * P;
            if (p + 1 < NPAIR) {
                if (p + 1 == pair) { offX = cur; dXp = G::dX(p + 1); }
                if (p == pair) { offXn = cur; dXn = G::dX(p + 1); }
                cur += G::dX(p + 1) * P;
            }
        }
        offXn = __builtin_amdgcn_readfirstlane(offXn); offX = __builtin_amdgcn_readfirstlane(offX); offT = __builtin_amdgcn_readfirstlane(offT);
        dXp = __builtin_amdgcn_readfirstlane(dXp); dXn = __builtin_amdgcn_readfirstlane(dXn);
    }
    int ring_end = G::dX0 * P + NPAIR * G::dT * P;
#pragma unroll
    for (int p = 1; p < NPAIR; p++) ring_end += G::dX(p) * P;
    unsigned char* const stw = lds + ring_end + sub * (32 * 80);
    const int in_off = kind ? offT : offX, Din = kind ? G::dT : dXp;
    const int out_off = kind ? offXn : offT, Dout = kind ? dXn : G::dT;
    const int res_off = offX, Dres = dXp;

    const void* wbase = nullptr;
    const float* bsrc = nullptr;
#pragma unroll
    for (int p = 0; p < NPAIR; p++)
        if (p == pair) { wbase = kind ? a.W2[p] : a.W1[p]; bsrc = kind ? a.b2[p] : a.b1[p]; }
    const uint4* const Wq = (const uint4*)wbase + ((long)ct * NKC * NT * 4) * 64 + lane;
    uint4 w[NW];
#pragma unroll
    for (int i = 0; i < NW; i++) { const int t = i / KS, kk = i % KS; w[i] = Wq[(((kk >> 2) * NT + t) * 4 + (kk & 3)) * 64]; }
    float* const bias_l = (float*)(lds + ring_end + WPR * (32 * 80));
    if (rs == 0 && lane < 32) bias_l[role * C + ct * 32 + lane] = bsrc[ct * 32 + lane];
    __syncthreads();
#pragma unroll
    for (int i = 0; i < NW; i++) asm volatile("" :: "v"(w[i].x));

    const unsigned lds_addr0 = (unsigned)(size_t)(__attribute__((address_space(3))) unsigned char*)lds;
    const int nslots = G::dX0 / RS_RD;
    int dma_off[PPW];
#pragma unroll
    for (int n = 0; n < PPW; n++) {
        const int j = sub + WPR * n < PPB ? sub + WPR * n : PPB - 1;
        const int slot = j * 64 + lane, row = slot / CPP, qs = slot % CPP;
        dma_off[n] = qs == CPP - 1 ? -16 : (row * a.ldx + (qs << 3)) * 2;
    }
    const unsigned lane_in = lds_addr0 + in_off + koff + l32 * P;

    const float slope1 = a.slope1, rinv = a.res_inv_slope, oscale = a.out_scale, oslope = a.slope;

#ifdef RS_PROFILE
    unsigned long long tacc[12] = {0, 0, 0, 0, 0, 0, 0, 0, 0, 0, 0, 0}, tlast = 0;
#define RS_STAMP(k) do { if (a.prof) { const unsigned long long t_ = __builtin_readcyclecounter(); tacc[k] += t_ - tlast; tlast = t_; } } while (0)
#else
#define RS_STAMP(k) do {} while (0)
#endif
    const int nsegs = a.nseg * a.nbatch;
    for (int seg = blockIdx.x; seg < nsegs; seg += gridDim.x) {
        const int b = seg / a.nseg, sj = seg - b * a.nseg;
        int len = a.len ? a.len[b] : a.M;
        len = __builtin_amdgcn_readfirstlane(len);
        const int seg0 = sj * a.S;
        if (seg0 >= len) continue;
        const int seg_end = min(seg0 + a.S, len);
        const int b_last = (seg_end - seg0 + Hsum + R - 1) / R - 1;
        const int nact = b_last + NB0 + 1;
        const int nsteps = nact + NR - 1;
        const int o0 = seg0 - NB0 * R - 2 * h0;
        const unsigned short* const Xb = (const unsigned short*)a.X + (long)b * a.x_bs;

        int rd_pos = role == 0 ? rs * 32 : (Din - 2 * my_h + rs * 32) % Din;
        int wr_pos = rs * 32;
        int rs_pos = pair == 0 ? (h0 - H2 + rs * 32) : ((Dres - (G::dil(pair) * H2 + H2) % Dres + rs * 32) % Dres);
        int g_out0 = seg0 - NB0 * R - my_H + rs * 32;
        f32x16 acc;

        int issued = 0, dslot = 0;
        auto dma_block = [&]() {
            const int g0 = o0 + issued * RS_RD;
            const unsigned long long pa = (unsigned long long)(Xb + (long)g0 * a.ldx);
            int nrec = (len - g0) * a.ldx * 2; if (nrec < 0) nrec = 0;
            const i32x4 rsrc = {__builtin_amdgcn_readfirstlane((int)(unsigned)pa), __builtin_amdgcn_readfirstlane((int)((pa >> 32) & 0xffff)),
                                __builtin_amdgcn_readfirstlane(nrec), 0x00020000};
            const int thr = -g0 * a.ldx * 2;
            const unsigned la0 = lds_addr0 + offX + dslot * (RS_RD * P);
#pragma unroll
            for (int n = 0; n < PPW; n++) {
                const int j = sub + WPR * n < PPB ? sub + WPR * n : PPB - 1;
                const int voff = g0 >= 0 ? dma_off[n] : (dma_off[n] < thr ? -16 : dma_off[n]);
                const unsigned la = __builtin_amdgcn_readfirstlane(la0 + j * 1024);
                asm volatile("s_mov_b32 m0, %0\n\tbuffer_load_dwordx4 %1, %2, 0 offen lds" :: "s"(la), "v"(voff), "s"(rsrc) : "memory", "m0");
            }
            issued++; dslot++; if (dslot == nslots) dslot = 0;
        };
        auto need = [&](int s) { return (2 * h0 + (s + 1) * R - 1) / RS_RD; };
        auto wait_landed = [&](int nblocks) {
            const int out = issued - nblocks;
            if (out <= 0) asm volatile("s_waitcnt vmcnt(0)" ::: "memory");
            else if (out == 1) asm volatile("s_waitcnt vmcnt(%0)" :: "n"(PPW) : "memory");
            else if (out == 2) asm volatile("s_waitcnt vmcnt(%0)" :: "n"(2 * PPW) : "memory");
            else if (out == 3) asm volatile("s_waitcnt vmcnt(%0)" :: "n"(3 * PPW) : "memory");
            else asm volatile("s_waitcnt vmcnt(%0)" :: "n"(4 * PPW) : "memory");
        };
        if (role == 0) {
            const int target = need(RS_PF - 1) + 1;
            while (issued < target) dma_block();
            wait_landed(need(0) + 1);
        }
        asm volatile("s_waitcnt lgkmcnt(0)\n\ts_barrier" ::: "memory");

        bool pend = false; int pend_g0 = 0;
        uint4 xs[2];
        const int nvalid = seg_end - seg0;
        const __amdgpu_buffer_rsrc_t rsA = __builtin_amdgcn_make_buffer_rsrc((void*)((unsigned short*)a.accum + (long)b * a.a_bs + (long)seg0 * a.lda), 0, a.accum ? nvalid * a.lda * 2 : 0, 0x00020000);
        const __amdgpu_buffer_rsrc_t rsO = __builtin_amdgcn_make_buffer_rsrc((void*)((unsigned short*)a.out + (long)b * a.o_bs + (long)seg0 * a.ldo), 0, a.out ? nvalid * a.ldo * 2 : 0, 0x00020000);
        const int lane_col = (ct * 32 + (lane & 3) * 8) * 2, lane_row = (lane >> 2) - seg0;
        auto row_off = [&](int g0, int h, int ld) { return __mul24(g0 + h * 16 + lane_row, ld * 2) + lane_col; };
        auto store_phase = [&]() {
            uint4 o[2];
#pragma unroll
            for (int h = 0; h < 2; h++) o[h] = *(const uint4*)(stw + (h * 16 + (lane >> 2)) * 80 + (lane & 3) * 16);
#ifdef RS_PROFILE
            asm volatile("" :: "v"(o[0].x), "v"(o[1].x));
            RS_STAMP(7);
            asm volatile("s_waitcnt vmcnt(0)" ::: "memory");
            RS_STAMP(8);
#endif
#pragma unroll
            for (int h = 0; h < 2; h++) {
                if (AM & 1 || HAS_OUT) {
                    f32x2 t[4] = {unpack16<H16>(o[h].x), unpack16<H16>(o[h].y), unpack16<H16>(o[h].z), unpack16<H16>(o[h].w)};
                    if (AM & 1) {
                        t[0] += unpack16<H16>(xs[h].x); t[1] += unpack16<H16>(xs[h].y);
                        t[2] += unpack16<H16>(xs[h].z); t[3] += unpack16<H16>(xs[h].w);
                        if (AM & 2) o[h] = make_uint4(pack16<H16>(t[0].x, t[0].y), pack16<H16>(t[1].x, t[1].y), pack16<H16>(t[2].x, t[2].y), pack16<H16>(t[3].x, t[3].y));
                    }
                    if (AM & 2) __builtin_amdgcn_raw_buffer_store_b128(__builtin_bit_cast(u32x4, o[h]), rsA, row_off(pend_g0, h, a.lda), 0, 0);
                    if (HAS_OUT) {
                        if (AM) {
#pragma unroll
                            for (int e = 0; e < 4; e++) t[e] = lrelu2(t[e] * oscale, oslope);
                            o[h] = make_uint4(pack16<H16>(t[0].x, t[0].y), pack16<H16>(t[1].x, t[1].y), pack16<H16>(t[2].x, t[2].y), pack16<H16>(t[3].x, t[3].y));
                        }
                        __builtin_amdgcn_raw_buffer_store_b128(__builtin_bit_cast(u32x4, o[h]), rsO, row_off(pend_g0, h, a.ldo), 0, 0);
                    }
                } else if (AM & 2) {
                    __builtin_amdgcn_raw_buffer_store_b128(__builtin_bit_cast(u32x4, o[h]), rsA, row_off(pend_g0, h, a.lda), 0, 0);
                }
            }
        };

        auto mma_slow = [&]() {
            constexpr int PD = NW <= 6 ? NW : (NW >= 40 ? 4 : 6);
#pragma unroll
            for (int e = 0; e < 16; e++) acc[e] = 0.f;
            const unsigned p0 = rd_pos + l32;
            const unsigned in_addr = lds_addr0 + in_off + koff;
            uint4 xf[PD + 1];
            unsigned ta = 0;
            auto request = [&](int i) {
                if (i % KS == 0) {
                    unsigned pt = p0 + (i / KS) * my_dil;
                    pt = min(pt, pt - (unsigned)Din);
                    ta = in_addr + pt * P;
                }
                switch (i % KS) {
                    case 0: asm volatile("ds_read_b128 %0, %1" : "=v"(xf[i % (PD + 1)]) : "v"(ta)); break;
                    case 1: asm volatile("ds_read_b128 %0, %1 offset:32" : "=v"(xf[i % (PD + 1)]) : "v"(ta)); break;
                    case 2: asm volatile("ds_read_b128 %0, %1 offset:64" : "=v"(xf[i % (PD + 1)]) : "v"(ta)); break;
                    default: asm volatile("ds_read_b128 %0, %1 offset:96" : "=v"(xf[i % (PD + 1)]) : "v"(ta)); break;
                }
            };
            asm volatile("s_waitcnt lgkmcnt(0)" ::: "memory");
            __builtin_amdgcn_sched_barrier(0);
#pragma unroll
            for (int i = 0; i < PD; i++) request(i);
#pragma unroll
            for (int i = 0; i < NW; i++) {
                if (i + PD < NW) request(i + PD);
                const int rem = NW - 1 - i;
                if (rem >= PD) asm volatile("s_waitcnt lgkmcnt(%0)" :: "n"(PD) : "memory");
                else if (rem == 5) asm volatile("s_waitcnt lgkmcnt(5)" ::: "memory");
                else if (rem == 4) asm volatile("s_waitcnt lgkmcnt(4)" ::: "memory");
                else if (rem == 3) asm volatile("s_waitcnt lgkmcnt(3)" ::: "memory");
                else if (rem == 2) asm volatile("s_waitcnt lgkmcnt(2)" ::: "memory");
                else if (rem == 1) asm volatile("s_waitcnt lgkmcnt(1)" ::: "memory");
                else asm volatile("s_waitcnt lgkmcnt(0)" ::: "memory");
                __builtin_amdgcn_sched_barrier(0);
                acc = mfma16<H16>(w[i], xf[i % (PD + 1)], acc);
                __builtin_amdgcn_sched_barrier(0);
            }
        };
        auto mma_fast = [&](auto dil_c) {
            constexpr int DIL = decltype(dil_c)::value;
            constexpr int PD = NW <= 6 ? NW : (NW >= 40 ? 4 : 6);
#pragma unroll
            for (int e = 0; e < 16; e++) acc[e] = 0.f;
            const unsigned base = lane_in + (unsigned)(rd_pos * P);
            uint4 xf[PD + 1];
            asm volatile("s_waitcnt lgkmcnt(0)" ::: "memory");
            __builtin_amdgcn_sched_barrier(0);
            rs_prefetch<0, PD, KS, DIL, P>(xf, base);
            rs_mma_steps<0, NW, PD, KS, DIL, P, H16>(xf, w, base, acc);
        };
        auto mma_block = [&]() {
            constexpr int D0 = DP & 15, D1 = (DP >> 4) & 15, D2 = (DP >> 8) & 15;
            const int span = 32 + (NT - 1) * my_dil;
            if (rd_pos + span > Din) mma_slow();
            else if (kind) mma_fast(std::integral_constant<int, 1>{});
            else if (pair == 0) mma_fast(std::integral_constant<int, D0>{});
            else if (pair == 1) mma_fast(std::integral_constant<int, NPAIR >= 2 ? D1 : D0>{});
            else mma_fast(std::integral_constant<int, NPAIR >= 3 ? D2 : D0>{});
            rd_pos += R; if (rd_pos >= Din) rd_pos -= Din;
        };
        auto epilogue_block = [&](auto kind_c, auto masked_c) {
            constexpr int KIND = decltype(kind_c)::value;
            constexpr bool MASKED = decltype(masked_c)::value;
            const int g = g_out0 + l32;
            const bool inside = g >= 0 && g < len;
            float4 bq[4];
            uint2 rq[4] = {};
            const unsigned ba = lds_addr0 + (unsigned)((unsigned char*)bias_l - lds) + (role * C + ct * 32 + h4) * 4;
            asm volatile("ds_read_b128 %0, %1" : "=v"(bq[0]) : "v"(ba));
            asm volatile("ds_read_b128 %0, %1 offset:32" : "=v"(bq[1]) : "v"(ba));
            asm volatile("ds_read_b128 %0, %1 offset:64" : "=v"(bq[2]) : "v"(ba));
            asm volatile("ds_read_b128 %0, %1 offset:96" : "=v"(bq[3]) : "v"(ba));
            if (KIND >= 1) {
                unsigned rp = rs_pos + l32; rp = min(rp, rp - (unsigned)Dres);
                const unsigned ra = lds_addr0 + res_off + rp * P + (ct * 32 + h4) * 2;
                asm volatile("ds_read_b64 %0, %1" : "=v"(rq[0]) : "v"(ra));
                asm volatile("ds_read_b64 %0, %1 offset:16" : "=v"(rq[1]) : "v"(ra));
                asm volatile("ds_read_b64 %0, %1 offset:32" : "=v"(rq[2]) : "v"(ra));
                asm volatile("ds_read_b64 %0, %1 offset:48" : "=v"(rq[3]) : "v"(ra));
            }
            unsigned char* dst;
            if (KIND <= 1) { unsigned wp = wr_pos + l32; wp = min(wp, wp - (unsigned)Dout); dst = lds + out_off + wp * P + (ct * 32 + h4) * 2; }
            else dst = stw + l32 * 80 + h4 * 2;
            asm volatile("s_waitcnt lgkmcnt(0)" ::: "memory");
            __builtin_amdgcn_sched_barrier(0);
#pragma unroll
            for (int q = 0; q < 4; q++) {
                f32x2 v01 = (f32x2){acc[4 * q], acc[4 * q + 1]} + (f32x2){bq[q].x, bq[q].y};
                f32x2 v23 = (f32x2){acc[4 * q + 2], acc[4 * q + 3]} + (f32x2){bq[q].z, bq[q].w};
                if (KIND >= 1) { v01 += inv_lrelu2(unpack16<H16>(rq[q].x), rinv); v23 += inv_lrelu2(unpack16<H16>(rq[q].y), rinv); }
                if (KIND <= 1) { v01 = lrelu2(v01, slope1); v23 = lrelu2(v23, slope1); }
                else if (!AM) { v01 = lrelu2(v01, oslope); v23 = lrelu2(v23, oslope); }
                uint2 pk;
                pk.x = pack16<H16>(v01.x, v01.y); pk.y = pack16<H16>(v23.x, v23.y);
                if (KIND <= 1 && MASKED && !inside) { pk.x = 0u; pk.y = 0u; }
                *(uint2*)(dst + q * 16) = pk;
            }
            if (KIND == 2) {
                pend = true; pend_g0 = g_out0;
                if (AM & 1) {
#pragma unroll
                    for (int h = 0; h < 2; h++) xs[h] = __builtin_bit_cast(uint4, __builtin_amdgcn_raw_buffer_load_b128(rsA, row_off(g_out0, h, a.lda), 0, 0));
                }
            }
            wr_pos += R; if (wr_pos >= Dout && Dout > 0) wr_pos -= Dout;
            rs_pos += R; if (rs_pos >= Dres) rs_pos -= Dres;
            g_out0 += R;
        };

        for (int s = 0; s < nsteps; s++) {
            RS_STAMP(0);
            const int blk = s - role;
            if (role == 0) {
                const int target = need(s + RS_PF) + 1;
                while (issued < target) dma_block();
            }
            if (is_final && pend) { store_phase(); pend = false; RS_STAMP(9); }
            RS_STAMP(1);
            if (blk >= 0 && blk < nact) {
                mma_block();
                RS_STAMP(2);
                const bool interior = g_out0 >= 0 && g_out0 + 32 <= len;
                if (is_final) epilogue_block(std::integral_constant<int, 2>{}, std::false_type{});
                else if (!kind) { if (interior) epilogue_block(std::integral_constant<int, 0>{}, std::false_type{}); else epilogue_block(std::integral_constant<int, 0>{}, std::true_type{}); }
                else { if (interior) epilogue_block(std::integral_constant<int, 1>{}, std::false_type{}); else epilogue_block(std::integral_constant<int, 1>{}, std::true_type{}); }
            }
            RS_STAMP(3);
            if (role == 0) wait_landed(need(s + 1) + 1);
            RS_STAMP(4);
            asm volatile("s_waitcnt lgkmcnt(0)" ::: "memory");
            RS_STAMP(5);
            asm volatile("s_barrier" ::: "memory");
            RS_STAMP(6);
        }
        if (is_final && pend) store_phase();
        if (role == 0) asm volatile("s_waitcnt vmcnt(0)" ::: "memory");
        asm volatile("s_barrier" ::: "memory");
    }
#ifdef RS_PROFILE
    if (a.prof && blockIdx.x == 0 && lane == 0)
        for (int k = 0; k < 12; k++) a.prof[(wave * 16 + k)] = (long long)tacc[k], a.prof[wave * 16 + 14] = role, a.prof[wave * 16 + 15] = sub;
#endif
// ... 86 lines not shown
```

zerovox_amd/csrc/zvx.hip:

```cpp
#include "../../include/zvx.h"
#include "zvx_kernels.h"
#include "stream_plan.h"

#include <dlfcn.h>
#include <math.h>
#include <cmath>
#include <rccl/rccl.h>
#include <stdarg.h>
#include <stdio.h>
#include <string.h>

#include <algorithm>
#include <map>
#include <sstream>
#include <stdexcept>
#include <string>
#include <vector>

using namespace zvx;

namespace {

struct ZvxError : std::runtime_error {
    int code;
    ZvxError(int c, const std::string& m) : std::runtime_error(m), code(c) {}
};
[[noreturn]] void fail(int code, const char* fmt, ...) {
    char buf[512];
    va_list ap; va_start(ap, fmt); vsnprintf(buf, sizeof buf, fmt, ap); va_end(ap);
    throw ZvxError(code, buf);
}
#define HIPCHK(x) do { hipError_t e_ = (x); if (e_ != hipSuccess) fail(ZVX_E_HIP, "%s failed: %s (%s:%d)", #x, hipGetErrorString(e_), __FILE__, __LINE__); } while (0)

thread_local std::string g_create_error;

struct Tensor {
    char kind = 'p';
    std::vector<int> dims;
    size_t off = 0, numel = 0;
    void* dev = nullptr;
    int dtype = DT_F32;
    const float* host = nullptr;
    float alpha = 1.f;
    int dim(int i) const { return dims.at(i); }
};

struct DevBuf { void* p = nullptr; void* base = nullptr; size_t cap = 0; };

struct GemmEvent { hipEvent_t a, b; int variant; double flops, bytes; long rows; int N, K, taps, res, fused; std::string tag, kname; };

}

struct zvx_ctx {
    int device = 0;
    hipStream_t stream = nullptr;
    hipStream_t main0 = nullptr;
    hipStream_t comm_stream = nullptr;
    hipStream_t voc_aux[2] = {nullptr, nullptr};
    hipEvent_t voc_ev[3] = {nullptr, nullptr, nullptr};
    int voc_overlap_maxb = 1 << 20;
    int voc_overlap_frames = 28672;
    hipStream_t front_stream = nullptr;
    hipEvent_t ev_front_done = nullptr, ev_mel_free = nullptr, ev_main_join = nullptr;
    int front_overlap = 1;
    bool mel_free_pending = false;
    bool front_dirty_main = true;
    struct HostSlot { void* p = nullptr; size_t cap = 0; hipEvent_t ready = nullptr, done = nullptr; bool pending = false; int B = 0, pcm16 = 0; long stride = 0, need = 0; };
    HostSlot host_slot[2];
    int host_next = 0, host_last = -1;
    hipStream_t copy_stream = nullptr;
    bool copy_is_comm = false;
    hipStream_t aux_stream = nullptr;
    hipEvent_t ev_aux[2] = {nullptr, nullptr};
    int va_overlap_maxb = 1 << 20;
    ncclComm_t comm = nullptr;
    int rank = 0, world = 1;
    hipEvent_t ev_compute = nullptr;
    std::map<const void*, hipEvent_t> gather_fence;
    std::string err;
    std::map<std::string, std::string> cfg;
    std::map<std::string, Tensor> tensors;
    std::vector<float> host_blob;
    std::map<std::string, DevBuf> bufs;
    std::map<const void*, const void*> packed;
    std::map<const void*, const void*> pair_packed;
    int dt = DT_BF16;
    int H = 0, emb_dim = 0, punct_dim = 0, n_phone_rows = 0, n_punct_rows = 0, max_txt_len = 0, max_mel_len = 0;
    int enc_layers = 0, enc_heads = 0, ffn_dim = 0, ffn_k0 = 0, ffn_k1 = 0, vp_dim = 0, vp_k = 0, n_bins = 0;
    int dec_layers = 0, dec_heads = 0, dec_scln = 0, n_mels = 0, hop = 0, res_dim = 0, dec_kind = 0, rn_asp = 1;
    std::vector<int> rn_layers, rn_filters, voc_rates, voc_ksizes, voc_rb_k;
    std::vector<std::vector<int>> voc_rb_d;
    int voc_resblock = 1, voc_c0 = 0;
    int B = 0, Tmax = 0, Lmax = 0;
    std::vector<int> T_host, mel_len_host;
    std::vector<int> in_stage;
    bool have_features = false, have_mel = false;
    int profile = 0;
    int profile_only = -1;
    int rs_prof = 0;
    int enc_split = 0;
    const void* fft_xs_ready = nullptr;
    int norm_fuse_maxb = 1 << 20;
// ... 120 lines not shown
        a.pending = true;
        arena_i ^= 1;
    }
    void upload(void* dst, const void* src, size_t bytes) {
        Arena& a = arena[arena_i];
        const size_t need = (bytes + 63) & ~(size_t)63;
        if (!a.p) { HIPCHK(hipHostMalloc((void**)&a.p, ARENA_BYTES, hipHostMallocDefault)); a.cap = ARENA_BYTES; }
        if (a.cur + need > a.cap) {
            HIPCHK(hipMemcpyAsync(dst, src, bytes, hipMemcpyHostToDevice, stream));
            HIPCHK(hipStreamSynchronize(stream));
            return;
        }
        memcpy(a.p + a.cur, src, bytes);
        HIPCHK(hipMemcpyAsync(dst, a.p + a.cur, bytes, hipMemcpyHostToDevice, stream));
        a.cur += need;
    }
    int* upload_ints(const std::string& name, const int* v, size_t n) {
        int* d = ibuf(name, n);
        upload(d, v, n * sizeof(int));
        return d;
    }
    size_t es() const { return dtype_size(dt); }

    hipEvent_t new_event() {
        hipEvent_t e;
        if (!event_pool.empty()) { e = event_pool.back(); event_pool.pop_back(); return e; }
        HIPCHK(hipEventCreate(&e));
        return e;
    }
    void stage_begin(int s) { if (profile) { HIPCHK(hipEventRecord(stage_ev[s][0], stream)); } }
    void stage_end(int s) { if (profile) { HIPCHK(hipEventRecord(stage_ev[s][1], stream)); stage_used[s] = true; } }

    template <typename V, typename L, typename D>
    void profiled(V&& vid, L&& launch, D&& describe) {
        const bool prof = profile >= 2 && (profile_only < 0 || vid() == profile_only);
        if (!prof) { launch(); return; }
        GemmEvent ev{};
        ev.a = new_event(); ev.b = new_event();
        struct Armed { Armed(hipEvent_t a, hipEvent_t b) { profile_events(a, b); } ~Armed() { profile_events(nullptr, nullptr); } };
        ev.variant = [&] { Armed armed(ev.a, ev.b); return launch(); }();
        describe(ev);
        ev.tag = tag;
        pending.push_back(ev);
    }
    void gemm(GemmArgs& a) {
        if (a.flops <= 0) a.flops = 2.0 * (double)a.M * a.nbatch * a.nheads * (double)a.N * ((double)a.K * a.ntaps + (double)a.K2);
        if (!a.Wp && a.dtype != DT_F32) { auto it = packed.find(a.W); if (it != packed.end()) a.Wp = it->second; }
        a.slab_small = slab_small | (spk_s2_fuse ? 0 : 32); a.xcd_flat = slab_flat;
        profiled([&] { return gemm_variant_of(a); }, [&] {
            const int id = a.fused == 2 ? launch_rb2fuse(a, stream) : (a.fused ? launch_resfuse(a, stream) : launch_gemm(a, stream));
            if (id < 0) fail(ZVX_E_INVALID, "launch_gemm rejected shape M=%d N=%d K=%d taps=%d", a.M, a.N, a.K, a.ntaps);
            return id;
        }, [&](GemmEvent& ev) {
            ev.flops = a.flops; ev.rows = (long)a.M * a.nbatch * a.nheads; ev.N = a.N; ev.K = a.K; ev.taps = a.ntaps; ev.res = a.res_mode; ev.fused = a.fused;
            const double esz = dtype_size(a.dtype);
            const double cells = (double)a.M * a.nbatch * a.nheads * a.N;
            ev.bytes = ((double)a.M * a.nbatch * a.nheads) * (double)(a.K + a.K2) * esz + (double)a.N * ((double)a.K * a.ntaps + a.K2) * esz * (a.fused ? 2 : 1) +
                       (a.out ? cells * dtype_size(a.out_dtype) : 0.0) + ((a.res_mode && !a.fused) ? cells * dtype_size(a.res_dtype) : 0.0) +
                       ((a.accum && (a.accum_mode & 1)) ? cells * dtype_size(a.accum_dtype) : 0.0) + ((a.accum && (a.accum_mode & 2)) ? cells * dtype_size(a.accum_dtype) : 0.0);
        });
        if (sat_check && a.nheads == 1) {
            sat_scan(a.out, a.out_dtype, a.o_bs, a.ldo, a.nbatch, a.M, a.out_len, a.N);
            if (a.accum && (a.accum_mode & 2)) sat_scan(a.accum, a.accum_dtype, a.a_bs, a.lda, a.nbatch, a.M, a.out_len, a.N);
        }
    }
    bool run_stream(StreamArgs& a) {
        const int id = launch_resstream(a, this->stream, true);
        if (id < 0) return false;
        profiled([&] { return id; }, [&] {
            const int id2 = launch_resstream(a, this->stream, false);
            if (id2 < 0) fail(ZVX_E_INVALID, "launch_resstream rejected a shape its dry run accepted (C=%d k=%d pairs=%d)", a.C, a.ntaps, a.npair);
            return id2;
        }, [&](GemmEvent& ev) {
            const double rows = (double)a.M * a.nbatch;
            ev.flops = 2.0 * 2.0 * a.npair * rows * a.C * a.C * a.ntaps; ev.rows = (long)rows; ev.N = a.C; ev.K = a.C; ev.taps = a.ntaps;
            ev.res = a.accum_mode; ev.fused = 10 + a.npair;
            ev.bytes = rows * a.C * 2.0 * (1 + (a.out ? 1 : 0) + ((a.accum && (a.accum_mode & 1)) ? 1 : 0) + ((a.accum && (a.accum_mode & 2)) ? 1 : 0));
        });
        return true;
    }
    template <typename F>
    void timed(double flops, double bytes, F&& f, const char* kname = nullptr) {
        const bool prof = profile >= 2 && profile_only < 0;
        GemmEvent ev{};
        if (prof) { ev.a = new_event(); ev.b = new_event(); HIPCHK(hipEventRecord(ev.a, stream)); }
        f();
        if (prof) { HIPCHK(hipEventRecord(ev.b, stream)); ev.variant = -1; ev.flops = flops; ev.bytes = bytes; ev.tag = tag; if (kname) ev.kname = kname; pending.push_back(ev); }
    }
    void resolve_events() {
        if (stats.empty()) {
            stats.resize(gemm_num_variants());
            for (int i = 0; i < gemm_num_variants(); i++) { memset(&stats[i], 0, sizeof stats[i]); snprintf(stats[i].name, 64, "%s", gemm_variant_name(i)); }
        }
        for (auto& e : pending) {
            float ms = 0.f;
            HIPCHK(hipEventElapsedTime(&ms, e.a, e.b));
            if (shape_log && e.variant >= 0) fprintf(stderr, "launch %-24s rows=%-8ld N=%-4d K=%-4d taps=%-2d res=%d fused=%d  %8.3f ms %8.1f TF/s %8.1f GB/s(alg)\n",
                                   gemm_variant_name(e.variant), e.rows, e.N, e.K, e.taps, e.res, e.fused, ms, e.flops / ms / 1e9, e.bytes / ms / 1e6);
            else if (shape_log) fprintf(stderr, "launch %-24s [%s]  %8.3f ms %8.1f GB/s(alg)\n", "(helper)", e.tag.c_str(), ms, e.bytes / ms / 1e6);
            if (e.variant >= 0) { auto& s = stats[e.variant]; s.launches++; s.ms += ms; s.flops += e.flops; s.bytes += e.bytes; }
            auto& ts = tagstats[e.tag];
            if (!ts.name[0]) snprintf(ts.name, 64, "%s", e.tag.c_str());
            ts.launches++; ts.ms += ms; ts.flops += e.flops; ts.bytes += e.bytes;
            if (!e.kname.empty()) {
                auto& ks = namedstats[e.kname];
                if (!ks.name[0]) snprintf(ks.name, 64, "%s", e.kname.c_str());
                ks.launches++; ks.ms += ms; ks.flops += e.flops; ks.bytes += e.bytes;
            }
            event_pool.push_back(e.a); event_pool.push_back(e.b);
        }
        pending.clear();
        for (int s = 0; s < ZVX_T_COUNT; s++)
            if (stage_used[s]) { float ms = 0.f; HIPCHK(hipEventElapsedTime(&ms, stage_ev[s][0], stage_ev[s][1])); stage_ms[s] = ms; stage_used[s] = false; }
    }
    void sync() {
        if (front_stream) HIPCHK(hipStreamSynchronize(front_stream));
        HIPCHK(hipStreamSynchronize(stream));
        if (comm_stream) HIPCHK(hipStreamSynchronize(comm_stream));
        if (copy_stream && !copy_is_comm) HIPCHK(hipStreamSynchronize(copy_stream));
        if (profile) resolve_events();
    }
    void quiesce_side_streams() noexcept {
        if (front_stream) (void)hipStreamSynchronize(front_stream);
        if (aux_stream) (void)hipStreamSynchronize(aux_stream);
        for (int i = 0; i < 2; i++) if (voc_aux[i]) (void)hipStreamSynchronize(voc_aux[i]);
        front_dirty_main = true; mel_free_pending = false;
    }
    void front_setup() {
        if (front_stream) return;
        int least = 0, greatest = 0;
        HIPCHK(hipDeviceGetStreamPriorityRange(&least, &greatest));
        HIPCHK(hipStreamCreateWithPriority(&front_stream, hipStreamNonBlocking, greatest));
        HIPCHK(hipEventCreateWithFlags(&ev_front_done, hipEventDisableTiming));
        HIPCHK(hipEventCreateWithFlags(&ev_mel_free, hipEventDisableTiming));
        HIPCHK(hipEventCreateWithFlags(&ev_main_join, hipEventDisableTiming));
    }
};

struct zvx_stream {
    zvx_ctx* c = nullptr;
    int frames = 0, chunk = 0, cpc = 0, halo = 0, hop = 0, native = 0, out_rate = 0;
    int nchunks = 0, next_chunk = 0, done = 0;
    int Pcap = 0;
    long wstride = 0;
    int64_t total = 0, emitted = 0, delay = 0, max_piece = 0;
    enum { DENOISE = 0, LIMIT = 1, RESAMPLE = 2 };
    struct Stage {
        int kind = DENOISE;
        zvx_plan::ReachPlanner reach;
        zvx_plan::ResamplePlanner rate;
        float* buf[2] = {nullptr, nullptr};
// ... 861 lines not shown
    const int* lens_d;
    void *A, *X0, *T1, *PP[2], *XS;
    bool side_ok;
    void* sideT1[2]; void* sidePP[2][2];
};
struct VocStage {
    int i, Cin, Cout, rows_in, rows;
    const int* len_in; const int* len;
    int dt_in, dt;
    float next_slope;
};

struct RbConv { std::string name; const Tensor* w = nullptr; const void* packed = nullptr; const float* bias = nullptr; };
struct RbWeights { std::string name; std::vector<RbConv> c1, c2; };
RbWeights voc_rb_weights(zvx_ctx* c, const VocCall& v, const VocStage& s, int j) {
    RbWeights w;
    w.name = "voc.rb" + std::to_string(s.i * v.nk + j);
    auto conv = [&](const char* which, int t) {
        RbConv r;
        r.name = w.name + which + std::to_string(t);
        r.w = &voc_weight(c, r.name + "_w", s.dt);
        auto it = c->packed.find(r.w->dev);
        if (it != c->packed.end()) r.packed = it->second;
        r.bias = c->pf(r.name + "_b");
        return r;
    };
    for (int t = 0; t < (int)c->voc_rb_d[j].size(); t++) {
        if (c->voc_resblock == 1) { w.c1.push_back(conv(".c1_", t)); w.c2.push_back(conv(".c2_", t)); }
        else w.c1.push_back(conv(".c_", t));
    }
    return w;
}

struct StageClose { int accum_mode; bool writes_out; };
StageClose stage_close(int j, int nk) {
    if (nk == 1) return {0, true};
    return {j == 0 ? 2 : (j < nk - 1 ? 3 : 1), j == nk - 1};
}
template <typename Args>
void close_stage(Args& a, const StageClose& cl, const VocCall& v, const VocStage& s) {
    a.accum = cl.accum_mode ? v.XS : nullptr; a.accum_mode = cl.accum_mode; a.a_bs = (long)s.rows * s.Cout; a.lda = s.Cout;
    if (cl.writes_out) { a.out = v.A; a.out_scale = 1.0f / v.nk; a.slope = s.next_slope; }
    else a.out = nullptr;
    if constexpr (std::is_same<Args, GemmArgs>::value) { a.accum_dtype = s.dt; if (cl.writes_out) a.act = ACT_LRELU; }
}

void voc_conv_pre(zvx_ctx* c, const VocCall& v, const void* vin, int dt) {
    const int nm = c->n_mels, Pmax = v.Pmax;
    const int* P_d = v.lens_d + v.B;
    GemmArgs a = gemm_base(dt);
    a.X = vin; a.x_bs = (long)Pmax * nm; a.ldx = nm; a.W = voc_weight(c, "voc.pre_w", dt).dev; a.ldw = nm; a.w_ts = (long)c->voc_c0 * nm;
    a.M = Pmax; a.N = c->voc_c0; a.K = nm; a.nbatch = v.B; a.in_len = P_d; a.out_len = P_d;
    set_taps_1d(a, c->t("voc.pre_w").dim(0), 1);
    a.bias = c->pf("voc.pre_b"); a.bias_mode = 1; a.act = ACT_LRELU; a.slope = 0.1f;
    a.out = v.A; a.o_bs = (long)Pmax * c->voc_c0; a.ldo = c->voc_c0;
    c->gemm(a);
}

void voc_upsample(zvx_ctx* c, const VocCall& v, const VocStage& s) {
    const int u = c->voc_rates[s.i], ku = c->voc_ksizes[s.i], B = v.B, Cin = s.Cin, Cout = s.Cout, rows_in = s.rows_in, dt_in = s.dt_in;
    const std::string up = "voc.up" + std::to_string(s.i);
    GemmArgs a = gemm_base(dt_in);
    a.out_dtype = s.dt;
    a.X = v.A; a.x_bs = (long)rows_in * Cin; a.ldx = Cin; a.ldw = Cin;
    a.M = rows_in; a.K = Cin; a.nbatch = B; a.in_len = s.len_in; a.out_len = s.len_in;
    a.bias_mode = 1; a.act = ACT_LRELU; a.slope = 0.1f;
    a.o_bs = (long)rows_in * u * Cout; a.ldo = u * Cout;
    if (dt_in != DT_F32 && c->has(up + "_wlo")) {
        const int hc = (u / 2) * Cout;
        a.N = hc; a.ntaps = 2; a.w_ts = (long)hc * Cin; a.flops = 2.0 * B * (double)rows_in * Cin * Cout * ku / 2;
        a.W = voc_weight(c, up + "_wlo", dt_in).dev; a.dv[0] = -1; a.dv[1] = 0;
        a.bias = c->pf(up + "_b"); a.out = v.X0;
        c->gemm(a);
        a.Wp = nullptr;
        a.W = voc_weight(c, up + "_whi", dt_in).dev; a.dv[0] = 0; a.dv[1] = 1;
        a.bias = c->pf(up + "_b") + hc; a.out = (char*)v.X0 + (size_t)hc * c->es();
        c->gemm(a);
    } else {
        a.W = voc_weight(c, up + "_w", dt_in).dev; a.w_ts = (long)u * Cout * Cin; a.N = u * Cout;
        a.ntaps = 3; a.dv[0] = -1; a.dv[1] = 0; a.dv[2] = 1;
        a.bias = c->pf(up + "_b"); a.out = v.X0;
        a.flops = 2.0 * B * (double)rows_in * Cin * Cout * ku;
        c->gemm(a);
    }
}

const zvx_ctx::NsWeights& voc_narrow_weights(zvx_ctx* c, const VocCall& v, const VocStage& s) {
    const int Cout = s.Cout, nk = v.nk;
    const std::string key = "voc.ns." + std::to_string(s.i) + (s.dt == DT_F16 ? ".h16" : "");
    auto it = c->ns_weights.find(key);
    if (it != c->ns_weights.end()) return it->second;
    zvx_ctx::NsWeights nw;
    int nfrag = 0;
    for (int j = 0; j < nk; j++) for (int q = 0; q < 6; q++) { nw.woff[6 * j + q] = nfrag; nfrag += narrowstage_steps(Cout, c->voc_rb_k[j]); }
    nw.W = c->buf(key + ".w", (size_t)nfrag * 1024);
    nw.bias = c->fbuf(key + ".b", (size_t)6 * nk * Cout);
    for (int j = 0; j < nk; j++) {
        const RbWeights w = voc_rb_weights(c, v, s, j);
        for (int t = 0; t < 3; t++)
            for (int q = 0; q < 2; q++) {
                const RbConv& cv = q ? w.c2[t] : w.c1[t];
                if (cv.w->dims.size() != 3 || cv.w->dim(0) != c->voc_rb_k[j] || cv.w->dim(1) != Cout || cv.w->dim(2) != Cout) fail(ZVX_E_MANIFEST, "weights: '%s' has an unexpected shape", cv.name.c_str());
                const int ci = 6 * j + 2 * t + q;
                launch_pack_narrow(cv.w->dev, c->voc_rb_k[j], Cout, (char*)nw.W + (size_t)nw.woff[ci] * 1024, c->stream);
                HIPCHK(hipMemcpyAsync(nw.bias + (size_t)ci * Cout, cv.bias, (size_t)Cout * 4, hipMemcpyDeviceToDevice, c->stream));
            }
    }
    return c->ns_weights.emplace(key, nw).first->second;
}

bool voc_narrow_stage(zvx_ctx* c, const VocCall& v, const VocStage& s) {
    const int Cout = s.Cout, nk = v.nk, rows = s.rows;
    if (!c->use_stagefuse || c->sat_check || c->voc_resblock != 1 || s.dt == DT_F32 || (Cout != 16 && Cout != 8) || nk < 1 || nk > 3) return false;
    for (int j = 0; j < nk; j++) if (c->voc_rb_d[j].size() != 3) return false;
    const zvx_ctx::NsWeights& nw = voc_narrow_weights(c, v, s);
    StageArgs sa;
    memset(&sa, 0, sizeof sa);
    sa.X = v.X0; sa.x_bs = (long)rows * Cout; sa.ldx = Cout; sa.W = nw.W; sa.bias = nw.bias;
    memcpy(sa.woff, nw.woff, sizeof sa.woff);
    sa.C = Cout; sa.nk = nk;
    for (int j = 0; j < nk; j++) { sa.ks[j] = c->voc_rb_k[j]; for (int t = 0; t < 3; t++) sa.dil[j][t] = c->voc_rb_d[j][t]; }
    sa.out = v.A; sa.o_bs = (long)rows * Cout; sa.ldo = Cout;
    sa.slope1 = 0.1f; sa.res_inv_slope = 10.0f; sa.slope = s.next_slope;
    sa.len = s.len; sa.M = rows; sa.nbatch = v.B; sa.f16 = s.dt == DT_F16;
    if (!launch_narrowstage(sa, c->stream, true)) return false;
    const int vid = Cout == 16 ? 24 : 25;
    c->profiled([&] { return vid; }, [&] {
        if (!launch_narrowstage(sa, c->stream, false)) fail(ZVX_E_INVALID, "launch_narrowstage rejected a stage its dry run accepted (C=%d)", Cout);
        return vid;
    }, [&](GemmEvent& ev) {
        double ksum = 0; for (int j = 0; j < nk; j++) ksum += c->voc_rb_k[j];
        const double rws = (double)rows * v.B;
        ev.flops = 2.0 * rws * Cout * Cout * 6.0 * ksum; ev.rows = (long)rws; ev.N = Cout; ev.K = Cout; ev.taps = (int)ksum; ev.fused = 100 + nk;
        ev.bytes = rws * Cout * 2.0 * 2.0;
    });
    return true;
}

void voc_side_begin(zvx_ctx* c) {
    for (int q = 0; q < 2; q++) if (!c->voc_aux[q]) HIPCHK(hipStreamCreateWithFlags(&c->voc_aux[q], hipStreamNonBlocking));
    for (int q = 0; q < 3; q++) if (!c->voc_ev[q]) HIPCHK(hipEventCreateWithFlags(&c->voc_ev[q], hipEventDisableTiming));
    HIPCHK(hipEventRecord(c->voc_ev[0], c->stream));
}
struct SideHop {
    zvx_ctx* const c; hipStream_t const main_stream, aux; hipEvent_t const done; bool on_aux = false;
    SideHop(zvx_ctx* c_, hipStream_t aux_, hipEvent_t done_) : c(c_), main_stream(c_->stream), aux(aux_), done(done_) {
        if (aux) HIPCHK(hipStreamWaitEvent(aux, c->voc_ev[0], 0));
    }
    ~SideHop() { c->stream = main_stream; }
    void to_aux() { if (aux && !on_aux) { c->stream = aux; on_aux = true; } }
    void to_main() {
        if (on_aux) {
            HIPCHK(hipEventRecord(done, aux));
            c->stream = main_stream; on_aux = false;
            HIPCHK(hipStreamWaitEvent(main_stream, done, 0));
        }
    }
};

void voc_resblock(zvx_ctx* c, const VocCall& v, const VocStage& s, int j) {
    const int B = v.B, rows = s.rows, Cout = s.Cout, dt = s.dt;
    const bool side = v.side_ok && j >= 1;
    SideHop hop(c, side ? c->voc_aux[j - 1] : nullptr, side ? c->voc_ev[j] : nullptr);
    void* const T1s = side ? v.sideT1[j - 1] : v.T1;
    void* const* const PPs = side ? v.sidePP[j - 1] : v.PP;
    const int k = c->voc_rb_k[j];
    const std::vector<int>& dil = c->voc_rb_d[j];
    const int nd = (int)dil.size();
    const RbWeights w = voc_rb_weights(c, v, s, j);
    const StageClose close = stage_close(j, v.nk);
    const void* cur = v.X0;
    int pp = 0;
    int t_first = 0;
    if (c->voc_resblock == 1 && dt != DT_F32 && c->use_resstream && !c->sat_check && nd >= 1 && nd <= 3) {
        bool packed_ok = true;
        for (int t = 0; t < nd; t++) packed_ok = packed_ok && w.c1[t].packed && w.c2[t].packed;
        auto chain = [&](int t0, int np, const void* in, bool closes) {
            StreamArgs sa;
            memset(&sa, 0, sizeof sa);
            sa.X = in; sa.x_bs = (long)rows * Cout; sa.ldx = Cout; sa.C = Cout; sa.ntaps = k; sa.npair = np;
            for (int q = 0; q < np; q++) {
                sa.W1[q] = w.c1[t0 + q].packed; sa.W2[q] = w.c2[t0 + q].packed;
                sa.b1[q] = w.c1[t0 + q].bias; sa.b2[q] = w.c2[t0 + q].bias;
                sa.dil[q] = dil[t0 + q];
            }
            sa.seg_min = c->rs_seg_min; sa.f16 = dt == DT_F16;
            if (c->rs_prof) sa.prof = (long long*)c->buf("rs.prof." + w.name + "." + std::to_string(t0), 16 * 16 * 8);
            sa.slope1 = 0.1f; sa.res_inv_slope = 10.0f; sa.out_scale = 1.f; sa.slope = 0.1f;
            sa.len = s.len; sa.M = rows; sa.nbatch = B; sa.o_bs = (long)rows * Cout; sa.ldo = Cout; sa.a_bs = (long)rows * Cout; sa.lda = Cout;
            if (closes) close_stage(sa, close, v, s);
            else sa.out = PPs[pp];
            return sa;
        };
        if (packed_ok) {
            StreamArgs whole = chain(0, nd, v.X0, true);
            hop.to_main();
            if (c->run_stream(whole)) t_first = nd;
            else if (nd == 3) {
                StreamArgs head = chain(0, 2, v.X0, false);
                StreamArgs probe = chain(2, 1, PPs[pp], true);
                if (launch_resstream(head, c->stream, true) >= 0 && launch_resstream(probe, c->stream, true) >= 0) {
                    hop.to_aux();
                    c->run_stream(head);
                    cur = PPs[pp]; pp ^= 1;
                    StreamArgs tail = chain(2, 1, cur, true);
                    hop.to_main();
                    c->run_stream(tail);
                    t_first = nd;
                }
            }
        }
    }
    auto rb_base = [&] {
        GemmArgs a = gemm_base(dt);
        a.M = rows; a.N = Cout; a.K = Cout; a.nbatch = B; a.in_len = s.len; a.out_len = s.len; a.ldw = Cout; a.w_ts = (long)Cout * Cout;
        a.x_bs = (long)rows * Cout; a.ldx = Cout; a.o_bs = (long)rows * Cout; a.ldo = Cout;
        return a;
    };
    if (c->voc_resblock == 2 && nd == 2 && dt != DT_F32 && c->use_rb2fuse && !c->sat_check && (Cout == 32 || Cout == 64) && w.c1[0].packed && w.c1[1].packed) {
        GemmArgs a = rb_base();
        a.X = v.X0; a.W = w.c1[1].w->dev; a.Wp = w.c1[1].packed; a.Wp2 = w.c1[0].packed;
        a.bias1 = w.c1[0].bias; a.slope1 = 0.1f; a.fused = 2;
        set_taps_1d(a, k, dil[1]);
        for (int q = 0; q < k; q++) a.dv1[q] = (q - (k - 1) / 2) * dil[0];
        a.bias = w.c1[1].bias; a.bias_mode = 1;
        a.res = v.X0; a.r_bs = (long)rows * Cout; a.ldr = Cout; a.res_mode = 2; a.res_inv_slope = 10.0f; a.res_dtype = dt;
        close_stage(a, close, v, s);
        a.flops = 2.0 * 2.0 * B * (double)rows * Cout * Cout * k;
        if (gemm_variant_of(a) >= 0) { hop.to_main(); c->gemm(a); t_first = nd; }
    }
    for (int t = t_first; t < nd; t++) {
        const bool last = (t == nd - 1);
        if (last) hop.to_main(); else hop.to_aux();
        auto rb_tail = [&](GemmArgs& a) {
            a.bias_mode = 1;
            a.res = cur; a.r_bs = (long)rows * Cout; a.ldr = Cout; a.res_mode = 2; a.res_inv_slope = 10.0f; a.res_dtype = dt;
            if (last) close_stage(a, close, v, s);
            else { a.act = ACT_LRELU; a.slope = 0.1f; a.out = PPs[pp]; }
        };
        GemmArgs a = rb_base();
        if (c->voc_resblock == 1) {
            const RbConv& c1 = w.c1[t]; const RbConv& c2 = w.c2[t];
            bool fuse = dt != DT_F32 && !c->sat_check && c1.packed && c2.packed;
            if (fuse) {
                a.X = cur; a.W = c2.w->dev; a.Wp = c2.packed; a.Wp2 = c1.packed;
                a.bias1 = c1.bias; a.slope1 = 0.1f; a.fused = 1;
                a.no_pairstream = c->use_pairstream <= 0 ? 1 : (c->use_pairstream == 3 ? 2 : 0);
                set_taps_1d(a, k, 1);
                for (int q = 0; q < k; q++) a.dv1[q] = (q - (k - 1) / 2) * dil[t];
                a.bias = c2.bias;
                a.flops = 2.0 * 2.0 * B * (double)rows * Cout * Cout * k;
                rb_tail(a);
                const int fv = gemm_variant_of(a);
                fuse = fv >= 0 && !(Cout == 128 && fv != 23);
            }
            if (!fuse) {
                a = rb_base();
                a.X = cur; a.W = c1.w->dev;
                set_taps_1d(a, k, dil[t]);
                a.bias = c1.bias; a.bias_mode = 1; a.act = ACT_LRELU; a.slope = 0.1f;
                a.out = T1s;
                c->gemm(a);
                a = rb_base();
                a.X = T1s; a.W = c2.w->dev;
                set_taps_1d(a, k, 1);
                a.bias = c2.bias;
                rb_tail(a);
            }
        } else {
// ... 2308 lines not shown
```

zerovox_amd/csrc/zvx_kernels.h:

```cpp
#pragma once
#include <hip/hip_runtime.h>
#include <hip/hip_ext.h>
#include <stdint.h>
#include <atomic>
#include <mutex>
#include <set>
#include <utility>

extern thread_local hipEvent_t zvx_gemm_ev_start, zvx_gemm_ev_stop;
#define ZVX_DISPATCH(kernel, grid, block, lds, stream, ...) \
    do { if (zvx_gemm_ev_start) hipExtLaunchKernelGGL(kernel, grid, block, lds, stream, zvx_gemm_ev_start, zvx_gemm_ev_stop, 0, __VA_ARGS__); \
         else hipLaunchKernelGGL(kernel, grid, block, lds, stream, __VA_ARGS__); } while (0)

namespace zvx {

inline void profile_events(hipEvent_t start, hipEvent_t stop) { zvx_gemm_ev_start = start; zvx_gemm_ev_stop = stop; }

typedef unsigned short bf16_t;

enum DType { DT_F32 = 0, DT_BF16 = 1, DT_F16 = 2 };
static inline size_t dtype_size(int dt) { return dt == DT_F32 ? 4 : 2; }
inline int num_cus() {
    static const int n = [] { int dev = 0, v = 0; if (hipGetDevice(&dev) != hipSuccess || hipDeviceGetAttribute(&v, hipDeviceAttributeMultiprocessorCount, dev) != hipSuccess || v <= 0) v = 256; return v; }();
    return n;
}
inline int persistent_cus() { return num_cus(); }

inline bool lds_opt_in(const void* kfn) {
    static std::mutex mu;
    static std::set<std::pair<const void*, int>> done;
    int dev = 0;
    if (hipGetDevice(&dev) != hipSuccess) return false;
    std::lock_guard<std::mutex> lk(mu);
    if (done.count({kfn, dev})) return true;
    if (hipFuncSetAttribute(kfn, hipFuncAttributeMaxDynamicSharedMemorySize, 160 * 1024) != hipSuccess) return false;
    done.insert({kfn, dev});
    return true;
}

enum Act { ACT_NONE = 0, ACT_RELU = 1, ACT_LRELU = 2, ACT_TANH = 3 };

#define ZVX_MAX_TAPS 16

struct GemmArgs {
    const void* X; long x_bs, x_hs; int ldx;
    const void* W; long w_bs, w_hs, w_ts; int ldw;
    const void* Wp;
    int halo_l, halo_r;
    const void* Wp2; const float* bias1; int dv1[ZVX_MAX_TAPS]; int fused; float slope1;
    int no_pairstream;
    int dtype;
    int M, N, K;
    int nbatch, nheads;
    const int* in_len;
    const int* out_len;
    const int* k_len;
    int in_len_static;
    int ntaps; int du[ZVX_MAX_TAPS], dv[ZVX_MAX_TAPS];
    int stride, wout, hin, win;
    int flat_win, flat_rows;
    int bflat;
    const void* X2; long x2_bs; int ldx2, K2;
    int xcd_flat;
    int slab_small;
    int out_split3;
    float alpha;
    const float* bias; int bias_mode;
    const void* res; long r_bs, r_hs; int ldr; int res_dtype; int res_mode;
    float res_inv_slope;
    void* accum; long a_bs; int lda; int accum_mode;
    int accum_dtype;
    float out_scale;
    int act; float slope;
    const float* post_scale; const float* post_shift;
    void* out; long o_bs, o_hs; int ldo; int out_dtype;
    float* se_part; int* se_part_S;
    void* ds_out; const void* ds_Wp; const float* ds_bias;
    double flops;
};

int launch_gemm(const GemmArgs& a, hipStream_t stream);
int gemm_variant_of(const GemmArgs& a);
int gemm_epi_mode_of(const GemmArgs& a);
int launch_resfuse(GemmArgs a, hipStream_t stream);
int launch_rb2fuse(GemmArgs a, hipStream_t stream);
size_t packed_weight_elems(int ntaps, int N, int K);
void launch_pack_pair(const void* packedA, int ntapsA, int KA, const void* packedB, int ntapsB, int KB, int N, void* out, hipStream_t s);
void launch_pack_weights(const void* w_bf16, int ntaps, int N, int K, void* out, hipStream_t s);
const char* gemm_variant_name(int id);
int gemm_num_variants();

struct StreamArgs {
    const void* X; long x_bs; int ldx;
    const void* W1[3]; const void* W2[3];
    const float* b1[3]; const float* b2[3];
    int dil[3];
    int C, ntaps, npair;
    void* out; long o_bs; int ldo;
    void* accum; long a_bs; int lda; int accum_mode;
    float slope1, res_inv_slope, out_scale, slope;
    const int* len; int M, nbatch;
    int S, nseg;
    int dX0, dT, dX[3];
    double flops;
    long long* prof;
    int seg_min;
    int f16;
};
int launch_resstream(StreamArgs a, hipStream_t stream, bool dry_run);

struct PairArgs {
    const void* X; long x_bs; int ldx;
    const void* W1; const void* W2;
    const float* b1; const float* b2;
    int C, ntaps, dil;
    void* out; long o_bs; int ldo;
    void* accum; long a_bs; int lda; int accum_mode;
    float slope1, res_inv_slope, out_scale, slope;
    const int* len; int M, nbatch;
    int force;
    int f16;
    int S, nseg, DX, DT, G0;
    long long* prof;
};
bool launch_pairstream(PairArgs a, hipStream_t stream, bool dry_run);

struct StageArgs {
    const void* X; long x_bs; int ldx;
    const void* W;
    int woff[18];
    const float* bias;
    int C, nk, ks[3], dil[3][3];
    void* out; long o_bs; int ldo;
    float slope1, res_inv_slope, slope;
    const int* len; int M, nbatch;
// ... 218 lines not shown
```

Measured before the change: 345.9 million.

## Seed MFMA accumulators with bias instead of adding bias in epilogues

Adds a bias_acc flag so GEMM and the fused conv kernels initialise their MFMA accumulators with the per-column bias rather than zero, and drop the bias add from their epilogues. The goal is to remove the epilogue bias loads and adds, and the registers that keep bias live through the tile loop. A fallback clears the flag for unsupported configurations. The vocoder pre-conv, upsample and resblock calls enable it. It also changes one NRES register-residency threshold in the stream kernel. The risk is that earlier bias loads raise register pressure or add latency before the MFMA loop.

Result: no change. 345.6 million, median of 2 (-0.1%).

```diff
diff --git a/zerovox_amd/csrc/gemm.hip b/zerovox_amd/csrc/gemm.hip
--- a/zerovox_amd/csrc/gemm.hip
+++ b/zerovox_amd/csrc/gemm.hip
@@ -67,8 +67,36 @@
 }
 
 template <int TM, int TN>
+__device__ __forceinline__ void acc_bias_load(f32x16 (&acc)[TN][TM], const float* bias, int col_base, int N, int lane) {
+#pragma unroll
+    for (int i = 0; i < TN; i++)
+#pragma unroll
+        for (int g = 0; g < 4; g++) {
+            const int co = col_base + i * 32 + 8 * g + 4 * (lane >> 5);
+            const float4 bb = co < N ? *(const float4*)(bias + co) : make_float4(0.f, 0.f, 0.f, 0.f);
+            acc[i][0][4 * g] = bb.x; acc[i][0][4 * g + 1] = bb.y; acc[i][0][4 * g + 2] = bb.z; acc[i][0][4 * g + 3] = bb.w;
+        }
+}
+template <int TM, int TN>
+__device__ __forceinline__ void acc_bias_spread(f32x16 (&acc)[TN][TM]) {
+#pragma unroll
+    for (int i = 0; i < TN; i++)
+#pragma unroll
+        for (int j = 1; j < TM; j++) acc[i][j] = acc[i][0];
+}
+template <int TM, int TN>
+__device__ __forceinline__ void acc_zero(f32x16 (&acc)[TN][TM]) {
+#pragma unroll
+    for (int i = 0; i < TN; i++)
+#pragma unroll
+        for (int j = 0; j < TM; j++)
+#pragma unroll
+            for (int e = 0; e < 16; e++) acc[i][j][e] = 0.f;
+}
+
+template <int TM, int TN>
 __device__ __forceinline__ void epilogue(const GemmArgs& a, f32x16 (&acc)[TN][TM], int b, int h, int row_base, int col_base,
-                                         int out_len, bool two_d, int lane) {
+                                         int out_len, bool two_d, int lane, bool bias_done = false ) {
     const long ooff = (long)b * a.o_bs + (long)h * a.o_hs;
     const long roff = (long)b * a.r_bs + (long)h * a.r_hs;
     const long aoff = (long)b * a.a_bs;
@@ -88,7 +116,7 @@
                 float v[4];
 #pragma unroll
                 for (int e = 0; e < 4; e++) v[e] = acc[i][j][4 * g + e] * a.alpha + brow;
-                if (a.bias_mode == 1) {
+                if (a.bias_mode == 1 && !bias_done) {
                     const float4 bb = *(const float4*)(a.bias + n);
                     v[0] += bb.x; v[1] += bb.y; v[2] += bb.z; v[3] += bb.w;
                 }
@@ -219,12 +247,11 @@
     };
 
     f32x16 acc[TN][TM];
-#pragma unroll
-    for (int i = 0; i < TN; i++)
-#pragma unroll
-        for (int j = 0; j < TM; j++)
-#pragma unroll
-            for (int e = 0; e < 16; e++) acc[i][j][e] = 0.f;
+    const bool bias_done = DT != DT_F32 && a.bias_acc;
+    if (bias_done) {
+        acc_bias_load<TM, TN>(acc, a.bias, n0 + wc * (BN / WN), a.N, lane);
+        acc_bias_spread<TM, TN>(acc);
+    } else acc_zero<TM, TN>(acc);
 
     const int xrow = wr * (BM / WM) + (lane & 31);
     const int wrow = BM + wc * (BN / WN) + (lane & 31);
@@ -267,7 +294,7 @@
         __syncthreads();
     }
 
-    epilogue<TM, TN>(a, acc, b, h, m0 + wr * (BM / WM), n0 + wc * (BN / WN), out_len, two_d, lane);
+    epilogue<TM, TN>(a, acc, b, h, m0 + wr * (BM / WM), n0 + wc * (BN / WN), out_len, two_d, lane, bias_done);
 }
 
 __device__ __forceinline__ unsigned pack_f16x2(float lo, float hi) { return pack_f16x2_sat(lo, hi); }
@@ -299,7 +326,7 @@
     const int act = DEC ? ACT_NONE : (CT ? ACT_LRELU : a.act);
     const float slope = CT ? (a.act == ACT_LRELU ? a.slope : 1.f) : a.slope;
     const int res_mode = RES_LDS ? 2 : (DEC ? (EPI & 1) : (CT ? ((EPI & 1) ? 2 : 0) : a.res_mode));
-    const int accum_mode = DEC ? 0 : (CT ? (EPI >> 1) & 3 : a.accum_mode), bias_mode = (CT && !DEC) ? 1 : a.bias_mode;
+    const int accum_mode = DEC ? 0 : (CT ? (EPI >> 1) & 3 : a.accum_mode), bias_mode = a.bias_acc ? 0 : ((CT && !DEC) ? 1 : a.bias_mode);
     const bool has_out = CT ? (EPI >> 3) & 1 : a.out != nullptr, out_bf16 = CT || a.out_dtype != DT_F32, has_post = !CT && a.post_scale != nullptr;
     const bool out_f16 = CT ? H16 : a.out_dtype == DT_F16, res_f16 = (CT || RES_LDS) ? H16 : a.res_dtype == DT_F16, acc_f16 = CT ? H16 : ((TN == 1 || TM <= 2) && a.accum_dtype == DT_F16);
     const bool acc_bf16 = CT || a.accum_dtype == DT_BF16 || acc_f16, res_bf16 = CT || RES_LDS || a.res_dtype != DT_F32;
@@ -476,13 +503,14 @@
     const float slope = a.act == ACT_LRELU ? a.slope : 1.f;
     const int h4 = 4 * (lane >> 5), c8 = lane % LPR, n = col_base + c8 * 8;
     const bool nok = n < a.N;
+    const bool badd = !a.bias_acc;
     float4 bb[TN][4];
 #pragma unroll
     for (int i = 0; i < TN; i++)
 #pragma unroll
         for (int g = 0; g < 4; g++) {
             const int co = col_base + i * 32 + 8 * g + h4;
-            bb[i][g] = co < a.N ? *(const float4*)(a.bias + co) : make_float4(0.f, 0.f, 0.f, 0.f);
+            bb[i][g] = (badd && co < a.N) ? *(const float4*)(a.bias + co) : make_float4(0.f, 0.f, 0.f, 0.f);
         }
     unsigned short* obase = (unsigned short*)a.out + (long)b * a.o_bs + n;
     u32x4 o[TM][NP];
@@ -492,8 +520,9 @@
         for (int i = 0; i < TN; i++)
 #pragma unroll
             for (int g = 0; g < 4; g++) {
-                const f32x2 v01 = lrelu2((f32x2){acc[i][j][4 * g], acc[i][j][4 * g + 1]} + (f32x2){bb[i][g].x, bb[i][g].y}, slope);
-                const f32x2 v23 = lrelu2((f32x2){acc[i][j][4 * g + 2], acc[i][j][4 * g + 3]} + (f32x2){bb[i][g].z, bb[i][g].w}, slope);
+                f32x2 s01 = (f32x2){acc[i][j][4 * g], acc[i][j][4 * g + 1]}, s23 = (f32x2){acc[i][j][4 * g + 2], acc[i][j][4 * g + 3]};
+                if (badd) { s01 += (f32x2){bb[i][g].x, bb[i][g].y}; s23 += (f32x2){bb[i][g].z, bb[i][g].w}; }
+                const f32x2 v01 = lrelu2(s01, slope), v23 = lrelu2(s23, slope);
                 uint2 pk;
                 pk.x = pack16x2(v01.x, v01.y, F16);
                 pk.y = pack16x2(v23.x, v23.y, F16);
@@ -610,12 +639,9 @@
     }
 
     f32x16 acc[TN][TM];
-#pragma unroll
-    for (int i = 0; i < TN; i++)
-#pragma unroll
-        for (int j = 0; j < TM; j++)
-#pragma unroll
-            for (int e = 0; e < 16; e++) acc[i][j][e] = 0.f;
+    const bool bias_acc = a.bias_acc != 0;
+    if (bias_acc) acc_bias_load<TM, TN>(acc, a.bias, n0 + wc * (BN / WN), a.N, lane);
+    else acc_zero<TM, TN>(acc);
 
     constexpr bool WREG = R == 0;
     constexpr int F = BN / 32, CNT = F >= 4 ? F / 4 : 1, WD = 4, D = WREG ? WD : R - 1, WAITN = WREG ? (WD - 1) * TN : (D - 2) * CNT;
@@ -690,6 +716,7 @@
             }
         }
         __syncthreads();
+        if (bias_acc && kc == 0) acc_bias_spread<TM, TN>(acc);
         int nk16 = 4;
         if (!FULLK) { nk16 = src2 ? n16_2 - (kc - nkc) * 4 : n16 - kc * 4; if (nk16 > 4) nk16 = 4; if (wave_dead) nk16 = 0; }
         const int ntaps_kc = src2 ? 1 : ntaps;
@@ -797,6 +824,10 @@
     const int HL = a.halo_l, SR = BM + a.halo_l + a.halo_r;
     const unsigned short* Xp = (const unsigned short*)a.X + (long)b * a.x_bs;
 
+    f32x16 acc[1][TM];
+    const bool bias_acc = a.bias_acc != 0;
+    if (bias_acc) acc_bias_load<TM, 1>(acc, a.bias, wc * 32, a.N, lane);
+    else acc_zero<TM, 1>(acc);
     uint4 w[NT][KS];
     {
         const uint4* Wq = (const uint4*)a.Wp + ((long)wc * NT * 4) * 64 + lane;
@@ -828,11 +859,7 @@
     }
     __syncthreads();
 
-    f32x16 acc[1][TM];
-#pragma unroll
-    for (int j = 0; j < TM; j++)
-#pragma unroll
-        for (int e = 0; e < 16; e++) acc[0][j][e] = 0.f;
+    if (bias_acc) acc_bias_spread<TM, 1>(acc);
     const int xrow0 = HL + wr * (BM / WM) + (lane & 31);
     const int koff = (lane >> 5) * 16;
 #pragma unroll
@@ -1280,10 +1307,9 @@
         __syncthreads();
 
         f32x16 acc[1][TM];
-#pragma unroll
-        for (int j = 0; j < TM; j++)
-#pragma unroll
-            for (int e = 0; e < 16; e++) acc[0][j][e] = 0.f;
+        const bool bias_acc = a.bias_acc != 0;
+        if (bias_acc) { acc_bias_load<TM, 1>(acc, a.bias1, wc * 32, a.N, lane); acc_bias_spread<TM, 1>(acc); }
+        else acc_zero<TM, 1>(acc);
 #pragma unroll
         for (int t = 0; t < NT; t++) {
             const unsigned char* rowp = slab + (wrow + (lane & 31) + H1 + a.dv1[t]) * PITCH_ + koff;
@@ -1307,12 +1333,13 @@
 #pragma unroll
             for (int q = 0; q < 4; q++) {
                 const int co = wc * 32 + 8 * q + 4 * (lane >> 5);
-                const float4 bb = *(const float4*)(a.bias1 + co);
+                const float4 bb = bias_acc ? make_float4(0.f, 0.f, 0.f, 0.f) : *(const float4*)(a.bias1 + co);
                 const uint2 xr = *(const uint2*)(slab + (i + H1) * PITCH_ + co * 2);
                 const f32x2 r01 = inv_lrelu2(F16 ? unpack_f16x2(xr.x) : unpack_bf16x2(xr.x), a.res_inv_slope);
                 const f32x2 r23 = inv_lrelu2(F16 ? unpack_f16x2(xr.y) : unpack_bf16x2(xr.y), a.res_inv_slope);
-                f32x2 v01 = (f32x2){acc[0][j][4 * q] + bb.x, acc[0][j][4 * q + 1] + bb.y} + r01;
-                f32x2 v23 = (f32x2){acc[0][j][4 * q + 2] + bb.z, acc[0][j][4 * q + 3] + bb.w} + r23;
+                f32x2 v01 = (f32x2){acc[0][j][4 * q], acc[0][j][4 * q + 1]}, v23 = (f32x2){acc[0][j][4 * q + 2], acc[0][j][4 * q + 3]};
+                if (!bias_acc) { v01 += (f32x2){bb.x, bb.y}; v23 += (f32x2){bb.z, bb.w}; }
+                v01 += r01; v23 += r23;
                 v01 = lrelu2(v01, a.slope1); v23 = lrelu2(v23, a.slope1);
                 if (!inside) { v01 = (f32x2){0.f, 0.f}; v23 = (f32x2){0.f, 0.f}; }
                 uint2 pk;
@@ -1322,10 +1349,8 @@
             }
         }
         __syncthreads();
-#pragma unroll
-        for (int j = 0; j < TM; j++)
-#pragma unroll
-            for (int e = 0; e < 16; e++) acc[0][j][e] = 0.f;
+        if (bias_acc) { acc_bias_load<TM, 1>(acc, a.bias, wc * 32, a.N, lane); acc_bias_spread<TM, 1>(acc); }
+        else acc_zero<TM, 1>(acc);
 #pragma unroll
         for (int t = 0; t < NT; t++) {
             const unsigned char* rowp = t1 + (wrow + (lane & 31) + H2 + a.dv[t]) * PITCH_ + koff;
@@ -1390,7 +1415,7 @@
     constexpr int P = C * 2 + 16, CPP = CPR + 1;
     constexpr int NW = NT * KS;
     constexpr bool LEAN = NW > 36 || (F16 && NW >= 28 && TM == 2 && (AM & 1) && HAS_OUT);
-    constexpr int NRES = LEAN ? (NW < 36 ? NW : 36) : NW;
+    constexpr int NRES = LEAN ? (NW < 36 ? NW : 36) : ((NW >= 28 && TM == 2 && AM == 2 && HAS_OUT) ? NW - 2 : NW);
     typedef __attribute__((ext_vector_type(4))) int i32x4;
     extern __shared__ __attribute__((aligned(16))) unsigned char lds[];
 
@@ -1425,17 +1450,17 @@
 
     constexpr bool BIAS_REG = NW <= 22;
     const int h4 = 4 * (lane >> 5);
-    float4 bq[4];
+    f32x16 bacc;
     if (BIAS_REG) {
 #pragma unroll
-        for (int q = 0; q < 4; q++) bq[q] = q < QN ? *(const float4*)((role ? a.bias : a.bias1) + wc * 32 + 8 * q + h4) : make_float4(0.f, 0.f, 0.f, 0.f);
+        for (int q = 0; q < 4; q++) {
+            const float4 t = q < QN ? *(const float4*)((role ? a.bias : a.bias1) + wc * 32 + 8 * q + h4) : make_float4(0.f, 0.f, 0.f, 0.f);
+            bacc[4 * q] = t.x; bacc[4 * q + 1] = t.y; bacc[4 * q + 2] = t.z; bacc[4 * q + 3] = t.w;
+        }
     }
 #pragma unroll
     for (int i = 0; i < NRES; i++) asm volatile("" :: "v"(w[i].x));
-    if (BIAS_REG) {
-#pragma unroll
-        for (int q = 0; q < 4; q++) asm volatile("" :: "v"(bq[q].x));
-    }
+    if (BIAS_REG) asm volatile("" :: "v"(bacc));
     __syncthreads();
     struct Tile { int t, b, mt, m0, in_len, out_len; };
     const bool use_tab = a.nbatch <= 128;
@@ -1499,6 +1524,15 @@
     asm volatile("s_waitcnt vmcnt(0) lgkmcnt(0)\n\ts_barrier" ::: "memory");
     const int koff = (lane >> 5) * 16;
     f32x16 acc[1][TM];
+    auto acc_from_bias = [&](const float* tab) {
+        if (BIAS_REG) return;
+#pragma unroll
+        for (int q = 0; q < 4; q++) {
+            const float4 bb = q < QN ? *(const float4*)(tab + wc * 32 + 8 * q + h4) : make_float4(0.f, 0.f, 0.f, 0.f);
+            bacc[4 * q] = bb.x; bacc[4 * q + 1] = bb.y; bacc[4 * q + 2] = bb.z; bacc[4 * q + 3] = bb.w;
+        }
+        asm volatile("" : "+v"(bacc));
+    };
     for (int ph = 0; qA.t >= 0 || qB.t >= 0 || qC.t >= 0; ph++) {
         const Tile qE = qD.t >= 0 ? next_tile(qD) : qD;
         if (role == 0) {
@@ -1513,9 +1547,8 @@
 #pragma unroll
                     for (int q = 0; q < QN; q++) {
                         const int co = wc * 32 + 8 * q + h4;
-                        const float4 bb = BIAS_REG ? bq[q] : *(const float4*)(bias1_l + co);
-                        const f32x2 v01 = lrelu2((f32x2){acc[0][j][4 * q], acc[0][j][4 * q + 1]} + (f32x2){bb.x, bb.y}, slope1);
-                        const f32x2 v23 = lrelu2((f32x2){acc[0][j][4 * q + 2], acc[0][j][4 * q + 3]} + (f32x2){bb.z, bb.w}, slope1);
+                        const f32x2 v01 = lrelu2((f32x2){acc[0][j][4 * q], acc[0][j][4 * q + 1]}, slope1);
+                        const f32x2 v23 = lrelu2((f32x2){acc[0][j][4 * q + 2], acc[0][j][4 * q + 3]}, slope1);
                         uint2 pk;
                         pk.x = inside ? pack16<F16>(v01.x, v01.y) : 0u;
                         pk.y = inside ? pack16<F16>(v23.x, v23.y) : 0u;
@@ -1524,10 +1557,7 @@
                 }
             }
             if (qC.t >= 0) {
-#pragma unroll
-                for (int j = 0; j < TM; j++)
-#pragma unroll
-                    for (int e = 0; e < 16; e++) acc[0][j][e] = 0.f;
+                acc_from_bias(bias1_l);
                 const unsigned char* rowp0 = lds + (ph & 3) * SB + (wrow + (lane & 31) + H1 - H2 * dil) * P + koff;
 #pragma unroll
                 for (int t = 0; t < NT; t++) {
@@ -1538,17 +1568,14 @@
 #pragma unroll
                         for (int j = 0; j < TM; j++) {
                             const uint4 xf = *(const uint4*)(rowp + j * 32 * P + kk * 32);
-                            acc[0][j] = mfma16<F16>(wf, xf, acc[0][j]);
+                            acc[0][j] = mfma16<F16>(wf, xf, (t == 0 && kk == 0) ? bacc : acc[0][j]);
                         }
                     }
                 }
             }
             asm volatile("s_waitcnt vmcnt(0)" ::: "memory");
         } else if (qA.t >= 0) {
-#pragma unroll
-            for (int j = 0; j < TM; j++)
-#pragma unroll
-                for (int e = 0; e < 16; e++) acc[0][j][e] = 0.f;
+            acc_from_bias(bias2_l);
             const unsigned char* rowp = t1base + (ph & 1) * TB + (wrow + (lane & 31)) * P + koff;
 #pragma unroll
             for (int t = 0; t < NT; t++)
@@ -1558,7 +1585,7 @@
 #pragma unroll
                     for (int j = 0; j < TM; j++) {
                         const uint4 xf = *(const uint4*)(rowp + (t + j * 32) * P + kk * 32);
-                        acc[0][j] = mfma16<F16>(wf, xf, acc[0][j]);
+                        acc[0][j] = mfma16<F16>(wf, xf, (t == 0 && kk == 0) ? bacc : acc[0][j]);
                     }
                 }
             const int lim_rows = (qA.m0 + BMO < qA.out_len) ? qA.m0 + BMO : qA.out_len;
@@ -1569,11 +1596,6 @@
                 const long rm_off = wc * 32 + (lane & 3) * 8;
                 unsigned short* accp = (unsigned short*)a.accum + (long)qA.b * a.a_bs + rm_off;
                 unsigned short* outp = (unsigned short*)a.out + (long)qA.b * a.o_bs + rm_off;
-                float4 bb[LEAN ? 1 : 4];
-                if (!LEAN) {
-#pragma unroll
-                    for (int q = 0; q < QN; q++) bb[LEAN ? 0 : q] = BIAS_REG ? bq[q] : *(const float4*)(bias2_l + wc * 32 + 8 * q + h4);
-                }
                 constexpr bool XS_EARLY = NW < 28 || TM == 1;
                 uint4 xs[TM][2];
                 if ((AM & 1) && XS_EARLY) {
@@ -1602,10 +1624,9 @@
                     uint2 pk[LEAN ? 1 : 4];
 #pragma unroll
                     for (int q = 0; q < QN; q++) {
-                        const float4 bq_ = LEAN ? *(const float4*)(bias2_l + wc * 32 + 8 * q + h4) : bb[LEAN ? 0 : q];
                         const uint2 rq_ = LEAN ? *(const uint2*)(resp + j * 32 * P + q * 16) : rrj[LEAN ? 0 : q];
-                        f32x2 v01 = (f32x2){acc[0][j][4 * q], acc[0][j][4 * q + 1]} + (f32x2){bq_.x, bq_.y} + inv_lrelu2(unpack16<F16>(rq_.x), rinv);
-                        f32x2 v23 = (f32x2){acc[0][j][4 * q + 2], acc[0][j][4 * q + 3]} + (f32x2){bq_.z, bq_.w} + inv_lrelu2(unpack16<F16>(rq_.y), rinv);
+                        f32x2 v01 = (f32x2){acc[0][j][4 * q], acc[0][j][4 * q + 1]} + inv_lrelu2(unpack16<F16>(rq_.x), rinv);
+                        f32x2 v23 = (f32x2){acc[0][j][4 * q + 2], acc[0][j][4 * q + 3]} + inv_lrelu2(unpack16<F16>(rq_.y), rinv);
                         if (!AM) { v01 = lrelu2(v01, slope); v23 = lrelu2(v23, slope); }
                         uint2 pq;
                         pq.x = pack16<F16>(v01.x, v01.y);
@@ -1948,8 +1969,19 @@
 }
 
 
+bool gemm_bias_acc_of(const GemmArgs& a) {
+    if (a.fused) return a.dtype != DT_F32;
+    return a.bias_acc && !(a.dtype == DT_F32 || a.bias_mode != 1 || !a.bias || a.alpha != 1.f || a.wout > 0 || a.ds_out || a.out_split3 || a.se_part ||
+                           a.nheads != 1 || a.k_len || a.N % 4);
+}
+
 int launch_gemm(const GemmArgs& a, hipStream_t stream) {
     if (a.N <= 0 || a.M <= 0 || a.nbatch <= 0) return -1;
+    if (a.bias_acc && !gemm_bias_acc_of(a)) {
+        GemmArgs c = a;
+        c.bias_acc = 0;
+        return launch_gemm(c, stream);
+    }
     if (a.ds_out) return launch_conv2d_s2(a, stream) ? 28 : -7;
     if (a.stride == 2 && a.wout > 0 && a.ntaps == 9 && a.K == 64 && a.Wp && launch_conv2d_s2(a, stream)) return 29;
     if (a.ntaps < 1 || a.ntaps > ZVX_MAX_TAPS) return -2;
diff --git a/zerovox_amd/csrc/pairstream.hip b/zerovox_amd/csrc/pairstream.hip
--- a/zerovox_amd/csrc/pairstream.hip
+++ b/zerovox_amd/csrc/pairstream.hip
@@ -44,7 +44,6 @@
     const int l32 = lane & 31, hi = lane >> 5;
     const int dil = a.dil, H1 = dil * H2, DX = a.DX, DT = a.DT, G0 = a.G0;
     const unsigned tbase = (unsigned)DX * PS_XP;
-    const float* const bias_l = (const float*)(lds + tbase + (unsigned)DT * PS_TP) + ROLE * 128;
     const unsigned scratch_l = tbase + (unsigned)DT * PS_TP + 1024;
 
     const unsigned char* const wq = (const unsigned char*)(ROLE ? a.W2 : a.W1) + (long)ct * NS * 1024;
@@ -108,10 +107,6 @@
         asm volatile("s_waitcnt lgkmcnt(0)\n\ts_barrier" ::: "memory");
 
         auto main_loop = [&](bool dma_real) __attribute__((always_inline)) {
-#pragma unroll
-            for (int j = 0; j < 4; j++)
-#pragma unroll
-                for (int e = 0; e < 16; e++) acc[j][e] = 0.f;
             unsigned bs[4], nbs[4], pn = 0, hkn = 0;
             auto bases_common = [&](int u) __attribute__((always_inline)) {
                 const int kc = u >= NT ? 1 : 0, tap = u - kc * NT;
@@ -156,10 +151,25 @@
             for (int j = 0; j < 4; j++) bases_tile(j, bs);
             asm volatile("s_waitcnt lgkmcnt(0)" ::: "memory");
             __builtin_amdgcn_sched_barrier(0);
+            f32x4 bq0, bq1, bq2, bq3;
+            {
+                const unsigned ba = tbase + (unsigned)DT * PS_TP + (ROLE * 128 + ct * 32 + 4 * hi) * 4;
+                asm volatile("ds_read_b128 %0, %1" : "=v"(bq0) : "v"(ba));
+                asm volatile("ds_read_b128 %0, %1 offset:32" : "=v"(bq1) : "v"(ba));
+                asm volatile("ds_read_b128 %0, %1 offset:64" : "=v"(bq2) : "v"(ba));
+                asm volatile("ds_read_b128 %0, %1 offset:96" : "=v"(bq3) : "v"(ba));
+            }
 #pragma unroll
             for (int i = 0; i < PD; i++)
 #pragma unroll
                 for (int j = 0; j < 4; j++) rd1(xs[i][j], bs[j], i);
+            asm volatile("s_waitcnt lgkmcnt(%0)" :: "n"(4 * PD) : "memory");
+            __builtin_amdgcn_sched_barrier(0);
+            asm volatile("" : "+v"(bq0), "+v"(bq1), "+v"(bq2), "+v"(bq3));
+#pragma unroll
+            for (int j = 0; j < 4; j++)
+                acc[j] = (f32x16){bq0.x, bq0.y, bq0.z, bq0.w, bq1.x, bq1.y, bq1.z, bq1.w, bq2.x, bq2.y, bq2.z, bq2.w, bq3.x, bq3.y, bq3.z, bq3.w};
+            __builtin_amdgcn_sched_barrier(0);
             for (int u2 = 0; u2 < NT; u2++) {
                 const int next_off = (u2 + 1 == NT ? 0 : (u2 + 1) * (WD * 1024));
 #pragma unroll
@@ -205,9 +215,6 @@
             int lv = lane;
             asm volatile("" : "+v"(lv));
             const int l32 = lv & 31, hi = lv >> 5;
-            float4 bq[4];
-#pragma unroll
-            for (int q = 0; q < 4; q++) bq[q] = *(const float4*)(bias_l + ct * 32 + 8 * q + 4 * hi);
 #pragma unroll
             for (int j = 0; j < 4; j++) {
                 const int g = g1 + 32 * j + l32;
@@ -216,8 +223,8 @@
                 unsigned char* const dst = lds + tbase + wp * PS_TP + (ct * 32 + 4 * hi) * 2;
 #pragma unroll
                 for (int q = 0; q < 4; q++) {
-                    const f32x2 v01 = lrelu2((f32x2){acc[j][4 * q], acc[j][4 * q + 1]} + (f32x2){bq[q].x, bq[q].y}, slope1);
-                    const f32x2 v23 = lrelu2((f32x2){acc[j][4 * q + 2], acc[j][4 * q + 3]} + (f32x2){bq[q].z, bq[q].w}, slope1);
+                    const f32x2 v01 = lrelu2((f32x2){acc[j][4 * q], acc[j][4 * q + 1]}, slope1);
+                    const f32x2 v23 = lrelu2((f32x2){acc[j][4 * q + 2], acc[j][4 * q + 3]}, slope1);
                     uint2 pk;
                     pk.x = inside ? pack16<H16>(v01.x, v01.y) : 0u;
                     pk.y = inside ? pack16<H16>(v23.x, v23.y) : 0u;
@@ -271,17 +278,14 @@
         auto epilogue_out = [&]() __attribute__((always_inline)) {
             int lv = lane;
             asm volatile("" : "+v"(lv));
-            float4 bq[4];
-#pragma unroll
-            for (int q = 0; q < 4; q++) bq[q] = *(const float4*)(bias_l + ct * 32 + 8 * q + 4 * (lv >> 5));
             const __amdgpu_buffer_rsrc_t rsA = res_rsrc(a.accum, a.a_bs), rsO = res_rsrc(a.out, a.o_bs);
 #pragma unroll
             for (int j = 0; j < 4; j++) {
                 float v[16];
 #pragma unroll
                 for (int q = 0; q < 4; q++) {
-                    v[4 * q] = acc[j][4 * q] + bq[q].x; v[4 * q + 1] = acc[j][4 * q + 1] + bq[q].y;
-                    v[4 * q + 2] = acc[j][4 * q + 2] + bq[q].z; v[4 * q + 3] = acc[j][4 * q + 3] + bq[q].w;
+                    v[4 * q] = acc[j][4 * q]; v[4 * q + 1] = acc[j][4 * q + 1];
+                    v[4 * q + 2] = acc[j][4 * q + 2]; v[4 * q + 3] = acc[j][4 * q + 3];
                     if (PS_RES_LDS) {
                         const f32x2 r01 = inv_lrelu2(unpack16<H16>(rcur[j][q].x), rinv), r23 = inv_lrelu2(unpack16<H16>(rcur[j][q].y), rinv);
                         v[4 * q] += r01.x; v[4 * q + 1] += r01.y; v[4 * q + 2] += r23.x; v[4 * q + 3] += r23.y;
diff --git a/zerovox_amd/csrc/resstream.hip b/zerovox_amd/csrc/resstream.hip
--- a/zerovox_amd/csrc/resstream.hip
+++ b/zerovox_amd/csrc/resstream.hip
@@ -22,15 +22,27 @@
 __device__ __forceinline__ void rs_prefetch(uint4 (&xf)[PD + 1], unsigned base) {
     if constexpr (I < PD) { rs_read<I, PD, KS, DIL, P>(xf, base); rs_prefetch<I + 1, PD, KS, DIL, P>(xf, base); }
 }
+__device__ __forceinline__ void rs_bias_request(f32x4 (&bq)[4], unsigned ba) {
+    asm volatile("ds_read_b128 %0, %1" : "=v"(bq[0]) : "v"(ba));
+    asm volatile("ds_read_b128 %0, %1 offset:32" : "=v"(bq[1]) : "v"(ba));
+    asm volatile("ds_read_b128 %0, %1 offset:64" : "=v"(bq[2]) : "v"(ba));
+    asm volatile("ds_read_b128 %0, %1 offset:96" : "=v"(bq[3]) : "v"(ba));
+}
+__device__ __forceinline__ void rs_bias_to_acc(f32x4 (&bq)[4], f32x16& acc) {
+    f32x4 b0 = bq[0], b1 = bq[1], b2 = bq[2], b3 = bq[3];
+    asm volatile("" : "+v"(b0), "+v"(b1), "+v"(b2), "+v"(b3));
+    acc = (f32x16){b0.x, b0.y, b0.z, b0.w, b1.x, b1.y, b1.z, b1.w, b2.x, b2.y, b2.z, b2.w, b3.x, b3.y, b3.z, b3.w};
+}
 template <int I, int NW, int PD, int KS, int DIL, int P, bool H16>
-__device__ __forceinline__ void rs_mma_steps(uint4 (&xf)[PD + 1], const uint4 (&w)[NW], unsigned base, f32x16& acc) {
+__device__ __forceinline__ void rs_mma_steps(uint4 (&xf)[PD + 1], const uint4 (&w)[NW], unsigned base, f32x4 (&bq)[4], f32x16& acc) {
     if constexpr (I < NW) {
         if constexpr (I + PD < NW) rs_read<I + PD, PD, KS, DIL, P>(xf, base);
         asm volatile("s_waitcnt lgkmcnt(%0)" :: "n"(NW - 1 - I >= PD ? PD : NW - 1 - I) : "memory");
         __builtin_amdgcn_sched_barrier(0);
+        if constexpr (I == 0) rs_bias_to_acc(bq, acc);
         acc = mfma16<H16>(w[I], xf[I % (PD + 1)], acc);
         __builtin_amdgcn_sched_barrier(0);
-        rs_mma_steps<I + 1, NW, PD, KS, DIL, P, H16>(xf, w, base, acc);
+        rs_mma_steps<I + 1, NW, PD, KS, DIL, P, H16>(xf, w, base, bq, acc);
     }
 }
 
@@ -133,6 +145,7 @@
         dma_off[n] = qs == CPP - 1 ? -16 : (row * a.ldx + (qs << 3)) * 2;
     }
     const unsigned lane_in = lds_addr0 + in_off + koff + l32 * P;
+    const unsigned bias_addr = lds_addr0 + (unsigned)((unsigned char*)bias_l - lds) + (role * C + ct * 32 + h4) * 4;
 
     const float slope1 = a.slope1, rinv = a.res_inv_slope, oscale = a.out_scale, oslope = a.slope;
 
@@ -239,8 +252,7 @@
 
         auto mma_slow = [&]() {
             constexpr int PD = NW <= 6 ? NW : (NW >= 40 ? 4 : 6);
-#pragma unroll
-            for (int e = 0; e < 16; e++) acc[e] = 0.f;
+            f32x4 bq[4];
             const unsigned p0 = rd_pos + l32;
             const unsigned in_addr = lds_addr0 + in_off + koff;
             uint4 xf[PD + 1];
@@ -260,6 +272,7 @@
             };
             asm volatile("s_waitcnt lgkmcnt(0)" ::: "memory");
             __builtin_amdgcn_sched_barrier(0);
+            rs_bias_request(bq, bias_addr);
 #pragma unroll
             for (int i = 0; i < PD; i++) request(i);
 #pragma unroll
@@ -274,6 +287,7 @@
                 else if (rem == 1) asm volatile("s_waitcnt lgkmcnt(1)" ::: "memory");
                 else asm volatile("s_waitcnt lgkmcnt(0)" ::: "memory");
                 __builtin_amdgcn_sched_barrier(0);
+                if (i == 0) rs_bias_to_acc(bq, acc);
                 acc = mfma16<H16>(w[i], xf[i % (PD + 1)], acc);
                 __builtin_amdgcn_sched_barrier(0);
             }
@@ -281,14 +295,14 @@
         auto mma_fast = [&](auto dil_c) {
             constexpr int DIL = decltype(dil_c)::value;
             constexpr int PD = NW <= 6 ? NW : (NW >= 40 ? 4 : 6);
-#pragma unroll
-            for (int e = 0; e < 16; e++) acc[e] = 0.f;
+            f32x4 bq[4];
             const unsigned base = lane_in + (unsigned)(rd_pos * P);
             uint4 xf[PD + 1];
             asm volatile("s_waitcnt lgkmcnt(0)" ::: "memory");
             __builtin_amdgcn_sched_barrier(0);
+            rs_bias_request(bq, bias_addr);
             rs_prefetch<0, PD, KS, DIL, P>(xf, base);
-            rs_mma_steps<0, NW, PD, KS, DIL, P, H16>(xf, w, base, acc);
+            rs_mma_steps<0, NW, PD, KS, DIL, P, H16>(xf, w, base, bq, acc);
         };
         auto mma_block = [&]() {
             constexpr int D0 = DP & 15, D1 = (DP >> 4) & 15, D2 = (DP >> 8) & 15;
@@ -305,13 +319,7 @@
             constexpr bool MASKED = decltype(masked_c)::value;
             const int g = g_out0 + l32;
             const bool inside = g >= 0 && g < len;
-            float4 bq[4];
             uint2 rq[4] = {};
-            const unsigned ba = lds_addr0 + (unsigned)((unsigned char*)bias_l - lds) + (role * C + ct * 32 + h4) * 4;
-            asm volatile("ds_read_b128 %0, %1" : "=v"(bq[0]) : "v"(ba));
-            asm volatile("ds_read_b128 %0, %1 offset:32" : "=v"(bq[1]) : "v"(ba));
-            asm volatile("ds_read_b128 %0, %1 offset:64" : "=v"(bq[2]) : "v"(ba));
-            asm volatile("ds_read_b128 %0, %1 offset:96" : "=v"(bq[3]) : "v"(ba));
             if (KIND >= 1) {
                 unsigned rp = rs_pos + l32; rp = min(rp, rp - (unsigned)Dres);
                 const unsigned ra = lds_addr0 + res_off + rp * P + (ct * 32 + h4) * 2;
@@ -327,8 +335,7 @@
             __builtin_amdgcn_sched_barrier(0);
 #pragma unroll
             for (int q = 0; q < 4; q++) {
-                f32x2 v01 = (f32x2){acc[4 * q], acc[4 * q + 1]} + (f32x2){bq[q].x, bq[q].y};
-                f32x2 v23 = (f32x2){acc[4 * q + 2], acc[4 * q + 3]} + (f32x2){bq[q].z, bq[q].w};
+                f32x2 v01 = (f32x2){acc[4 * q], acc[4 * q + 1]}, v23 = (f32x2){acc[4 * q + 2], acc[4 * q + 3]};
                 if (KIND >= 1) { v01 += inv_lrelu2(unpack16<H16>(rq[q].x), rinv); v23 += inv_lrelu2(unpack16<H16>(rq[q].y), rinv); }
                 if (KIND <= 1) { v01 = lrelu2(v01, slope1); v23 = lrelu2(v23, slope1); }
                 else if (!AM) { v01 = lrelu2(v01, oslope); v23 = lrelu2(v23, oslope); }
diff --git a/zerovox_amd/csrc/zvx.hip b/zerovox_amd/csrc/zvx.hip
--- a/zerovox_amd/csrc/zvx.hip
+++ b/zerovox_amd/csrc/zvx.hip
@@ -47,7 +47,7 @@
 
 struct DevBuf { void* p = nullptr; void* base = nullptr; size_t cap = 0; };
 
-struct GemmEvent { hipEvent_t a, b; int variant; double flops, bytes; long rows; int N, K, taps, res, fused; std::string tag, kname; };
+struct GemmEvent { hipEvent_t a, b; int variant; double flops, bytes; long rows; int N, K, taps, res, fused, bias_acc; std::string tag, kname; };
 
 }
 
@@ -274,7 +274,7 @@
             if (id < 0) fail(ZVX_E_INVALID, "launch_gemm rejected shape M=%d N=%d K=%d taps=%d", a.M, a.N, a.K, a.ntaps);
             return id;
         }, [&](GemmEvent& ev) {
-            ev.flops = a.flops; ev.rows = (long)a.M * a.nbatch * a.nheads; ev.N = a.N; ev.K = a.K; ev.taps = a.ntaps; ev.res = a.res_mode; ev.fused = a.fused;
+            ev.flops = a.flops; ev.rows = (long)a.M * a.nbatch * a.nheads; ev.N = a.N; ev.K = a.K; ev.taps = a.ntaps; ev.res = a.res_mode; ev.fused = a.fused; ev.bias_acc = gemm_bias_acc_of(a);
             const double esz = dtype_size(a.dtype);
             const double cells = (double)a.M * a.nbatch * a.nheads * a.N;
             ev.bytes = ((double)a.M * a.nbatch * a.nheads) * (double)(a.K + a.K2) * esz + (double)a.N * ((double)a.K * a.ntaps + a.K2) * esz * (a.fused ? 2 : 1) +
@@ -296,7 +296,7 @@
         }, [&](GemmEvent& ev) {
             const double rows = (double)a.M * a.nbatch;
             ev.flops = 2.0 * 2.0 * a.npair * rows * a.C * a.C * a.ntaps; ev.rows = (long)rows; ev.N = a.C; ev.K = a.C; ev.taps = a.ntaps;
-            ev.res = a.accum_mode; ev.fused = 10 + a.npair;
+            ev.res = a.accum_mode; ev.fused = 10 + a.npair; ev.bias_acc = 1;
             ev.bytes = rows * a.C * 2.0 * (1 + (a.out ? 1 : 0) + ((a.accum && (a.accum_mode & 1)) ? 1 : 0) + ((a.accum && (a.accum_mode & 2)) ? 1 : 0));
         });
         return true;
@@ -317,8 +317,8 @@
         for (auto& e : pending) {
             float ms = 0.f;
             HIPCHK(hipEventElapsedTime(&ms, e.a, e.b));
-            if (shape_log && e.variant >= 0) fprintf(stderr, "launch %-24s rows=%-8ld N=%-4d K=%-4d taps=%-2d res=%d fused=%d  %8.3f ms %8.1f TF/s %8.1f GB/s(alg)\n",
-                                   gemm_variant_name(e.variant), e.rows, e.N, e.K, e.taps, e.res, e.fused, ms, e.flops / ms / 1e9, e.bytes / ms / 1e6);
+            if (shape_log && e.variant >= 0) fprintf(stderr, "launch %-24s rows=%-8ld N=%-4d K=%-4d taps=%-2d res=%d fused=%d  %8.3f ms %8.1f TF/s %8.1f GB/s(alg) bias_acc=%d\n",
+                                   gemm_variant_name(e.variant), e.rows, e.N, e.K, e.taps, e.res, e.fused, ms, e.flops / ms / 1e9, e.bytes / ms / 1e6, e.bias_acc);
             else if (shape_log) fprintf(stderr, "launch %-24s [%s]  %8.3f ms %8.1f GB/s(alg)\n", "(helper)", e.tag.c_str(), ms, e.bytes / ms / 1e6);
             if (e.variant >= 0) { auto& s = stats[e.variant]; s.launches++; s.ms += ms; s.flops += e.flops; s.bytes += e.bytes; }
             auto& ts = tagstats[e.tag];
@@ -1286,7 +1286,7 @@
     a.X = vin; a.x_bs = (long)Pmax * nm; a.ldx = nm; a.W = voc_weight(c, "voc.pre_w", dt).dev; a.ldw = nm; a.w_ts = (long)c->voc_c0 * nm;
     a.M = Pmax; a.N = c->voc_c0; a.K = nm; a.nbatch = v.B; a.in_len = P_d; a.out_len = P_d;
     set_taps_1d(a, c->t("voc.pre_w").dim(0), 1);
-    a.bias = c->pf("voc.pre_b"); a.bias_mode = 1; a.act = ACT_LRELU; a.slope = 0.1f;
+    a.bias = c->pf("voc.pre_b"); a.bias_mode = 1; a.bias_acc = 1; a.act = ACT_LRELU; a.slope = 0.1f;
     a.out = v.A; a.o_bs = (long)Pmax * c->voc_c0; a.ldo = c->voc_c0;
     c->gemm(a);
 }
@@ -1298,7 +1298,7 @@
     a.out_dtype = s.dt;
     a.X = v.A; a.x_bs = (long)rows_in * Cin; a.ldx = Cin; a.ldw = Cin;
     a.M = rows_in; a.K = Cin; a.nbatch = B; a.in_len = s.len_in; a.out_len = s.len_in;
-    a.bias_mode = 1; a.act = ACT_LRELU; a.slope = 0.1f;
+    a.bias_mode = 1; a.bias_acc = 1; a.act = ACT_LRELU; a.slope = 0.1f;
     a.o_bs = (long)rows_in * u * Cout; a.ldo = u * Cout;
     if (dt_in != DT_F32 && c->has(up + "_wlo")) {
         const int hc = (u / 2) * Cout;
@@ -1365,7 +1365,7 @@
     }, [&](GemmEvent& ev) {
         double ksum = 0; for (int j = 0; j < nk; j++) ksum += c->voc_rb_k[j];
         const double rws = (double)rows * v.B;
-        ev.flops = 2.0 * rws * Cout * Cout * 6.0 * ksum; ev.rows = (long)rws; ev.N = Cout; ev.K = Cout; ev.taps = (int)ksum; ev.fused = 100 + nk;
+        ev.flops = 2.0 * rws * Cout * Cout * 6.0 * ksum; ev.rows = (long)rws; ev.N = Cout; ev.K = Cout; ev.taps = (int)ksum; ev.fused = 100 + nk; ev.bias_acc = 1;
         ev.bytes = rws * Cout * 2.0 * 2.0;
     });
     return true;
@@ -1449,6 +1449,7 @@
         GemmArgs a = gemm_base(dt);
         a.M = rows; a.N = Cout; a.K = Cout; a.nbatch = B; a.in_len = s.len; a.out_len = s.len; a.ldw = Cout; a.w_ts = (long)Cout * Cout;
         a.x_bs = (long)rows * Cout; a.ldx = Cout; a.o_bs = (long)rows * Cout; a.ldo = Cout;
+        a.bias_acc = 1;
         return a;
     };
     if (c->voc_resblock == 2 && nd == 2 && dt != DT_F32 && c->use_rb2fuse && !c->sat_check && (Cout == 32 || Cout == 64) && w.c1[0].packed && w.c1[1].packed) {
diff --git a/zerovox_amd/csrc/zvx_kernels.h b/zerovox_amd/csrc/zvx_kernels.h
--- a/zerovox_amd/csrc/zvx_kernels.h
+++ b/zerovox_amd/csrc/zvx_kernels.h
@@ -66,6 +66,7 @@
     int out_split3;
     float alpha;
     const float* bias; int bias_mode;
+    int bias_acc;
     const void* res; long r_bs, r_hs; int ldr; int res_dtype; int res_mode;
     float res_inv_slope;
     void* accum; long a_bs; int lda; int accum_mode;
@@ -81,6 +82,7 @@
 
 int launch_gemm(const GemmArgs& a, hipStream_t stream);
 int gemm_variant_of(const GemmArgs& a);
+bool gemm_bias_acc_of(const GemmArgs& a);
 int gemm_epi_mode_of(const GemmArgs& a);
 int launch_resfuse(GemmArgs a, hipStream_t stream);
 int launch_rb2fuse(GemmArgs a, hipStream_t stream);
```
